# cvangysel/SERT

Hardware: AMD Instinct MI355X
Metric: training_pairs_per_sec (higher is better)
Workload: dtype f32; 1 GPU; C2 LSE: VectorSpaceLanguageModel (NCE z=10, Adam) V_w=100000 V_e=1000 d=128 window=10 batch=65536; global_batch=65536, per_gpu_batch=65536, parallelism=dp1, id_dtype=uint32, seed=0, instance_weights=1, dataset_instances=4194304, dataset_batches=64

## Files before the change

### include/sert_hip_debug.h

```cpp
#ifndef SERT_HIP_DEBUG_H
#define SERT_HIP_DEBUG_H

#include "sert_hip.h"

#ifdef __cplusplus
extern "C" {
#endif

int sert_debug_update_counts(sert_model* m, int64_t* out, int n);

int sert_debug_poison_scratch(sert_model* m);

int sert_debug_row_lists(const uint32_t* allbits, int world, int rank, int64_t num_batches, int64_t bit_words,
                         int64_t rows_per_rank, int64_t vocab, int64_t batch, int32_t* serve_cnt,
                         int32_t* fetch_cnt, int32_t* serve_rows, int32_t* fetch_rows, int32_t* union_rows,
                         int32_t* ptr, int32_t* ent, int64_t capacity, int64_t* sizes);

int sert_debug_word_index_sum(const void* ids, int id_bytes, int64_t num_batches, int B, int n, int vocab, int row_groups,
                              int dense_heavy, int64_t batch, const float* src, int d, float divisor, float* grad_out,
                              int64_t* stats);

int sert_bench_gemm(int device, int ta, int tb, int epi, int M, int N, int K, int splits,
                    int iters, double* avg_us);

int sert_debug_gemm(int device, int ta, int tb, int epi, int M, int N, int K, const float* A, const float* B,
                    const float* bias, float* C);

int sert_debug_gemm_splitk(int device, int M, int N, int K, int splits, const float* A, const float* B, float* out);

int sert_debug_gemm_longk(int device, int tb, int M, int N, int K, int splits, const float* A, const float* B, float* C);

enum { SERT_MEMBENCH_COPY = 0, SERT_MEMBENCH_READ = 1, SERT_MEMBENCH_GATHER = 2, SERT_MEMBENCH_OPTIMIZER = 3 };
int sert_bench_memory(int device, int kind, size_t bytes, size_t table_bytes, int row_bytes,
                      int window, size_t gap_bytes, int blocks, int iters, double* avg_us);

#ifdef __cplusplus
}
#endif
#endif
```

### sert_amd/_capi.py

```python
import ctypes
import os

import numpy as np

_HERE = os.path.dirname(os.path.abspath(__file__))
LIB_PATH = os.environ.get('SERT_LIB') or os.path.join(_HERE, 'libsert_hip.so')

KIND_LOGLINEAR, KIND_VECTORSPACE, KIND_VECTORSPACE_SOFTMAX = 0, 1, 2
SPLIT_TRAIN, SPLIT_VALIDATE = 0, 1

T_RW, T_RE, T_W, T_B = 0, 1, 2, 3
T_STATE0_RW, T_STATE0_RE, T_STATE0_W, T_STATE0_B = 4, 5, 6, 7
T_STATE1_RW, T_STATE1_RE, T_STATE1_W, T_STATE1_B = 8, 9, 10, 11
T_GRAD_RW, T_GRAD_RE, T_GRAD_W, T_GRAD_B = 12, 13, 14, 15
T_ACT_H, T_ACT_T, T_ACT_DA, T_ACT_DH, T_ACT_ROWLOSS = 16, 17, 18, 19, 20

COMM_ID_BYTES = 128

EXPORTS = [
    'sert_create', 'sert_destroy', 'sert_last_error', 'sert_device_info', 'sert_device_count',
    'sert_set_tensor', 'sert_get_tensor', 'sert_tensor_size', 'sert_set_step', 'sert_get_step',
    'sert_set_eval_draws', 'sert_get_eval_draws', 'sert_negatives_of_step',
    'sert_upload_dataset', 'sert_train_batch', 'sert_hint_next_batch', 'sert_train_batches',
    'sert_eval_batch', 'sert_eval_batches',
    'sert_predict_project', 'sert_predict_tokens', 'sert_score_topk',
    'sert_scorer_create', 'sert_scorer_destroy', 'sert_scorer_topk', 'sert_scorer_scores',
    'sert_host_alloc', 'sert_host_free',
    'sert_comm_unique_id', 'sert_comm_init', 'sert_comm_init_host', 'sert_comm_destroy', 'sert_comm_stats',
    'sert_synchronize', 'sert_timing_enable', 'sert_timing_reset', 'sert_timing_count',
    'sert_timing_name', 'sert_timing_avg_us', 'sert_timing_launches', 'sert_bench_gemm', 'sert_debug_gemm', 'sert_debug_gemm_splitk', 'sert_debug_gemm_longk', 'sert_bench_memory', 'sert_debug_row_lists', 'sert_debug_word_index_sum',
    'sert_debug_update_counts', 'sert_debug_poison_scratch',
    'sert_profile_range_push', 'sert_profile_range_pop',
]


_F32P, _I64P = ctypes.POINTER(ctypes.c_float), ctypes.POINTER(ctypes.c_int64)
ALLTOALL_FN = ctypes.CFUNCTYPE(ctypes.c_int, ctypes.c_void_p, _F32P, _I64P, _I64P, _F32P, _I64P, _I64P)


class SertConfig(ctypes.Structure):
    _fields_ = [
        ('struct_size', ctypes.c_uint32),
        ('kind', ctypes.c_int32),
        ('batch_size', ctypes.c_int32),
        ('global_batch_size', ctypes.c_int32),
        ('window_size', ctypes.c_int32),
        ('vocab_size', ctypes.c_int32),
        ('num_entities', ctypes.c_int32),
        ('word_dim', ctypes.c_int32),
        ('entity_dim', ctypes.c_int32),
        ('num_negatives', ctypes.c_int32),
        ('id_bytes', ctypes.c_int32),
        ('device', ctypes.c_int32),
        ('keep_grads', ctypes.c_int32),
        ('deterministic', ctypes.c_int32),
        ('inference_only', ctypes.c_int32),
        ('lambda_', ctypes.c_float),
        ('lr', ctypes.c_float),
        ('beta1', ctypes.c_float),
        ('beta2', ctypes.c_float),
        ('eps', ctypes.c_float),
        ('seed', ctypes.c_uint64),
    ]


class SertError(RuntimeError):
    pass


_lib = None


def load():
    global _lib
    if _lib is not None:
        return _lib
    if not os.path.exists(LIB_PATH):
        raise SertError(
            'libsert_hip.so not found at %s; build it with '
            '`python -m sert_amd._build` (hipcc --offload-arch=gfx950). '
            'There is no CPU fallback.' % LIB_PATH)
    lib = ctypes.CDLL(LIB_PATH)
    vp, i32, i64, sz = ctypes.c_void_p, ctypes.c_int32, ctypes.c_int64, ctypes.c_size_t
    fp = ctypes.c_void_p
    lib.sert_create.argtypes = [ctypes.POINTER(SertConfig), ctypes.POINTER(vp)]
    lib.sert_destroy.argtypes = [vp]
    lib.sert_last_error.restype = ctypes.c_char_p
    lib.sert_device_info.argtypes = [ctypes.c_int, ctypes.c_char_p, sz]
    lib.sert_device_count.argtypes = []
    lib.sert_set_tensor.argtypes = [vp, ctypes.c_int, fp, sz]
    lib.sert_get_tensor.argtypes = [vp, ctypes.c_int, fp, sz]
    lib.sert_tensor_size.argtypes = [vp, ctypes.c_int]
    lib.sert_tensor_size.restype = sz
    lib.sert_set_step.argtypes = [vp, i64]
    lib.sert_get_step.argtypes = [vp]
    lib.sert_get_step.restype = i64
    lib.sert_set_eval_draws.argtypes = [vp, i64]
    lib.sert_get_eval_draws.argtypes = [vp]
    lib.sert_get_eval_draws.restype = i64
    lib.sert_negatives_of_step.argtypes = [vp, i64, ctypes.c_int, vp]
    lib.sert_upload_dataset.argtypes = [vp, ctypes.c_int, fp, fp, fp, fp, fp, fp, i64]
    lib.sert_train_batch.argtypes = [vp, i64, fp, ctypes.POINTER(ctypes.c_float)]
    lib.sert_train_batches.argtypes = [vp, fp, i64, fp]
    lib.sert_hint_next_batch.argtypes = [vp, i64]
    lib.sert_eval_batch.argtypes = [vp, ctypes.c_int, i64, fp, ctypes.POINTER(ctypes.c_float)]
    lib.sert_eval_batches.argtypes = [vp, ctypes.c_int, ctypes.c_void_p, i64, ctypes.c_void_p]
    lib.sert_predict_project.argtypes = [vp, fp, i64, fp]
    lib.sert_predict_tokens.argtypes = [vp, fp, i64, fp]
    lib.sert_score_topk.argtypes = [ctypes.c_int, fp, i64, i32, fp, i64, i32, fp, fp]
    lib.sert_scorer_create.argtypes = [ctypes.c_int, fp, i64, i32, ctypes.POINTER(vp)]
    lib.sert_scorer_destroy.argtypes = [vp]
    lib.sert_scorer_topk.argtypes = [vp, fp, i64, i32, fp, fp]
    lib.sert_scorer_scores.argtypes = [vp, fp, i64, fp]
    lib.sert_host_alloc.argtypes = [ctypes.POINTER(vp), sz]
# ... 159 lines not shown
        check(self._lib.sert_eval_batch(self._h, split, int(batch_index), _addr(negatives),
                                        ctypes.byref(loss)))
        return np.float32(loss.value)

    def eval_batches(self, split, batch_indices):
        idx = np.ascontiguousarray(batch_indices, dtype=np.int64)
        out = np.empty(idx.shape[0], dtype=np.float32)
        if idx.shape[0]:
            check(self._lib.sert_eval_batches(self._h, split, idx.ctypes.data, idx.shape[0], out.ctypes.data))
        return out

    def predict_project(self, avg):
        avg = np.ascontiguousarray(avg, dtype=np.float32)
        q = avg.shape[0]
        out = np.empty((q, self.cfg.entity_dim), dtype=np.float32)
        check(self._lib.sert_predict_project(self._h, avg.ctypes.data, q, out.ctypes.data))
        return out

    def predict_tokens(self, ids):
        ids = np.ascontiguousarray(ids)
        assert ids.dtype.itemsize == self.cfg.id_bytes
        rows = ids.shape[0]
        out = np.empty((rows, self.cfg.window_size, self.cfg.num_entities), dtype=np.float32)
        check(self._lib.sert_predict_tokens(self._h, ids.ctypes.data, rows, out.ctypes.data))
        return out

    def comm_init(self, unique_id, rank, world):
        assert len(unique_id) == COMM_ID_BYTES
        check(self._lib.sert_comm_init(self._h, unique_id, rank, world))

    def comm_init_host(self, rank, world, alltoall):
        def trampoline(_user, send, soff, scnt, recv, roff, rcnt):
            try:
                so = np.ctypeslib.as_array(soff, shape=(world,))
                sc = np.ctypeslib.as_array(scnt, shape=(world,))
                ro = np.ctypeslib.as_array(roff, shape=(world,))
                rc = np.ctypeslib.as_array(rcnt, shape=(world,))
                ns = int((so + sc).max()) if world else 0
                nr = int((ro + rc).max()) if world else 0
                sbuf = np.ctypeslib.as_array(send, shape=(max(ns, 1),))
                rbuf = np.ctypeslib.as_array(recv, shape=(max(nr, 1),))
                alltoall(sbuf, so, sc, rbuf, ro, rc)
                return 0
            except Exception:
                import traceback
                traceback.print_exc()
                return 1
        self._host_alltoall = ALLTOALL_FN(trampoline)
        check(self._lib.sert_comm_init_host(self._h, rank, world, self._host_alltoall, None))

    def comm_stats(self):
        v = (ctypes.c_double * 8)()
        check(self._lib.sert_comm_stats(self._h, v, 8))
        return {'world': int(v[0]), 'exchange': {0: 'none', 1: 'zero1', 2: 'rows'}[int(v[1])],
                'bytes_per_step': float(v[2]), 'zero1_bytes_per_step': float(v[3]),
                'transport': {0: 'none', 1: 'rccl', 2: 'host'}[int(v[4])], 'steps': int(v[5]),
                'rows_fetched_per_batch': float(v[6]), 'rows_served_per_batch': float(v[7])}

    def synchronize(self):
        check(self._lib.sert_synchronize(self._h))

    def timing_enable(self, on=True):
        check(self._lib.sert_timing_enable(self._h, int(on)))

    def timing_launches(self):
        n = self._lib.sert_timing_count(self._h)
        return {self._lib.sert_timing_name(self._h, i).decode():
                self._lib.sert_timing_launches(self._h, i) for i in range(n)}

    def timing_reset(self):
        check(self._lib.sert_timing_reset(self._h))

    def poison_scratch(self):
        self._lib.sert_debug_poison_scratch.argtypes = [ctypes.c_void_p]
        check(self._lib.sert_debug_poison_scratch(self._h))

    def update_counts(self):
        v = (ctypes.c_int64 * 10)()
        self._lib.sert_debug_update_counts.argtypes = [ctypes.c_void_p, ctypes.POINTER(ctypes.c_int64), ctypes.c_int]
        check(self._lib.sert_debug_update_counts(self._h, v, 10))
        names = ('dense', 'lazy', 'skip_32_1', 'skip_64_1', 'skip_32_3', 'skip_64_2', 'skip_64_3', 'skip_64_4', 'skip_full', 'skip_sparse')
        return dict(zip(names, (int(x) for x in v)))

    def timings(self):
        n = self._lib.sert_timing_count(self._h)
        return {self._lib.sert_timing_name(self._h, i).decode():
                self._lib.sert_timing_avg_us(self._h, i) for i in range(n)}


def comm_unique_id():
    buf = ctypes.create_string_buffer(COMM_ID_BYTES)
    check(load().sert_comm_unique_id(buf))
    return buf.raw


def score_topk(entities, projections, k, device=0):
    e = np.ascontiguousarray(entities, dtype=np.float32)
    p = np.ascontiguousarray(projections, dtype=np.float32)
    assert e.ndim == 2 and p.ndim == 2 and e.shape[1] == p.shape[1]
    q = p.shape[0]
    idx = np.empty((q, k), dtype=np.int32)
    val = np.empty((q, k), dtype=np.float32)
    check(load().sert_score_topk(device, e.ctypes.data, e.shape[0], e.shape[1], p.ctypes.data, q,
                                 k, idx.ctypes.data, val.ctypes.data))
    return idx, val


class PinnedBuffer(object):

    def __init__(self, dtype):
        self.dtype = np.dtype(dtype)
        self._ptr = ctypes.c_void_p()
        self._bytes = 0
        self._lib = load()

    def view(self, shape):
        if os.environ.get('SERT_NO_PINNED'):
            return np.empty(shape, dtype=self.dtype)
        need = int(np.prod(shape)) * self.dtype.itemsize
        if need > self._bytes:
            self.free()
            cap = max(need, 1 << 16)
            check(self._lib.sert_host_alloc(ctypes.byref(self._ptr), cap))
            self._bytes = cap
        raw = (ctypes.c_char * max(need, 1)).from_address(self._ptr.value)
        return np.frombuffer(raw, dtype=self.dtype, count=int(np.prod(shape))).reshape(shape)

    def holds(self, array):
        if not self._ptr.value or not isinstance(array, np.ndarray) or not array.flags['C_CONTIGUOUS']:
            return False
        addr = array.ctypes.data
        return self._ptr.value <= addr and addr + array.nbytes <= self._ptr.value + self._bytes

    def free(self):
        if self._ptr.value:
            self._lib.sert_host_free(self._ptr)
            self._ptr = ctypes.c_void_p()
            self._bytes = 0

    def __del__(self):
        try:
            self.free()
        except Exception:
            pass


class Scorer(object):

    MAX_HOST_SCORES = 1 << 26

    def __init__(self, entities, device=0):
        e = np.ascontiguousarray(entities, dtype=np.float32)
        assert e.ndim == 2
        self.num_entities, self.dim = e.shape
        self._lib = load()
        self._h = ctypes.c_void_p()
        check(self._lib.sert_scorer_create(device, e.ctypes.data, e.shape[0], e.shape[1],
                                           ctypes.byref(self._h)))
        self._pin_q, self._pin_idx, self._pin_val = PinnedBuffer(np.float32), PinnedBuffer(np.int32), PinnedBuffer(np.float32)

    def query_buffer(self, num_queries):
        return self._pin_q.view((num_queries, self.dim))

    def _stage(self, projections):
        p = np.asarray(projections, dtype=np.float32)
        if p.ndim == 1:
# ... 4 lines not shown
        staged = self._pin_q.view(p.shape)
        np.copyto(staged, p)
        return staged

    def topk(self, projections, k):
        p = self._stage(projections)
        q = p.shape[0]
        idx = self._pin_idx.view((q, k))
        val = self._pin_val.view((q, k))
        check(self._lib.sert_scorer_topk(self._h, p.ctypes.data, q, k, idx.ctypes.data,
                                         val.ctypes.data))
        return idx, val

    def scores(self, projections):
        p = np.ascontiguousarray(projections, dtype=np.float32)
        if p.ndim == 1:
            p = p.reshape(1, -1)
        assert p.shape[1] == self.dim
        out = np.empty((p.shape[0], self.num_entities), dtype=np.float32)
        check(self._lib.sert_scorer_scores(self._h, p.ctypes.data, p.shape[0], out.ctypes.data))
        return out

    def rank(self, projections, k=None):
        if k is not None and k <= min(self.num_entities, 1024):
            return self.topk(projections, k)
        p = np.asarray(projections, dtype=np.float32)
        if p.ndim == 1:
            p = p.reshape(1, -1)
        keep = self.num_entities if k is None else min(k, self.num_entities)
        step = max(1, self.MAX_HOST_SCORES // self.num_entities)
        idx = np.empty((p.shape[0], keep), dtype=np.int32)
        val = np.empty((p.shape[0], keep), dtype=np.float32)
        for lo in range(0, p.shape[0], step):
            sc = self.scores(p[lo:lo + step])
            order = np.argsort(-sc, axis=1, kind='stable')[:, :keep]
            idx[lo:lo + step] = order
            val[lo:lo + step] = np.take_along_axis(sc, order, axis=1)
        return idx, val

    def close(self):
        if getattr(self, '_h', None) is not None and self._h:
            self._lib.sert_scorer_destroy(self._h)
            self._h = None
        for b in (getattr(self, '_pin_q', None), getattr(self, '_pin_idx', None), getattr(self, '_pin_val', None)):
            if b is not None:
                b.free()

    def __del__(self):
        try:
            self.close()
        except Exception:
            pass


def bench_gemm(M, N, K, ta=0, tb=0, epi=0, splits=1, iters=20, device=0):
    us = ctypes.c_double()
    check(load().sert_bench_gemm(device, ta, tb, epi, M, N, K, splits, iters, ctypes.byref(us)))
    return us.value


MEMBENCH_COPY, MEMBENCH_READ, MEMBENCH_GATHER, MEMBENCH_OPTIMIZER = 0, 1, 2, 3
SEPARATE_ALLOCATIONS = ctypes.c_size_t(-1).value


def debug_word_index_sum(ids, vocab, src, batch=0, row_groups=1, dense_heavy=False, divisor=1.0, sort_level0=False):
    lib = load()
    ids = np.ascontiguousarray(ids)
    assert ids.ndim == 3 and ids.dtype in (np.uint8, np.uint16, np.uint32), (ids.shape, ids.dtype)
    src = np.ascontiguousarray(src, dtype=np.float32)
    nb, B, n = ids.shape
    assert src.shape[0] == B
    d = src.shape[1]
    out = np.empty((vocab, d), dtype=np.float32)
    stats = np.zeros(8, dtype=np.int64)
    lib.sert_debug_word_index_sum.argtypes = [ctypes.c_void_p, ctypes.c_int, ctypes.c_int64, ctypes.c_int, ctypes.c_int, ctypes.c_int,
                                              ctypes.c_int, ctypes.c_int, ctypes.c_int64, ctypes.c_void_p, ctypes.c_int, ctypes.c_float,
                                              ctypes.c_void_p, ctypes.c_void_p]
    check(lib.sert_debug_word_index_sum(_addr(ids), ids.dtype.itemsize, nb, B, n, int(vocab), int(row_groups), int(bool(dense_heavy)) | (2 if sort_level0 else 0),
                                        int(batch), _addr(src), d, float(divisor), _addr(out), _addr(stats)))
    keys = ('levels', 'items', 'partial_rows', 'final_items', 'dense_words', 'row_groups', 'level0_items', 'distinct_words')
    return out, dict(zip(keys, [int(x) for x in stats]))


def debug_gemm(A, B, ta=0, tb=0, epi=0, bias=None, device=0):
    lib = load()
    A = np.ascontiguousarray(A, dtype=np.float32)
    B = np.ascontiguousarray(B, dtype=np.float32)
    K, M = A.shape if ta else A.shape[::-1]
    N = B.shape[0] if tb else B.shape[1]
    assert (B.shape[1] if tb else B.shape[0]) == K, (A.shape, B.shape)
    C = np.empty((M, N), dtype=np.float32)
    if bias is not None:
        bias = np.ascontiguousarray(bias, dtype=np.float32)
    lib.sert_debug_gemm.argtypes = [ctypes.c_int] * 7 + [ctypes.c_void_p] * 4
    check(lib.sert_debug_gemm(device, int(ta), int(tb), int(epi), M, N, K, _addr(A), _addr(B),
                              _addr(bias) if bias is not None else None, _addr(C)))
    return C


def debug_gemm_splitk(A, B, splits, device=0):
    lib = load()
    A = np.ascontiguousarray(A, dtype=np.float32)
    B = np.ascontiguousarray(B, dtype=np.float32)
    K, M = A.shape
    N = B.shape[1]
    assert B.shape[0] == K
    out = np.empty(M * N + N, dtype=np.float32)
    lib.sert_debug_gemm_splitk.argtypes = [ctypes.c_int] * 5 + [ctypes.c_void_p] * 3
    check(lib.sert_debug_gemm_splitk(device, M, N, K, int(splits), _addr(A), _addr(B), _addr(out)))
    return out[:M * N].reshape(M, N), out[M * N:]


def debug_gemm_longk(A, B, splits, tb=0, device=0):
    lib = load()
    A = np.ascontiguousarray(A, dtype=np.float32)
    B = np.ascontiguousarray(B, dtype=np.float32)
    M, K = A.shape
    N = B.shape[0] if tb else B.shape[1]
    assert (B.shape[1] if tb else B.shape[0]) == K
    out = np.empty((M, N), dtype=np.float32)
    lib.sert_debug_gemm_longk.argtypes = [ctypes.c_int] * 6 + [ctypes.c_void_p] * 3
    check(lib.sert_debug_gemm_longk(device, int(tb), M, N, K, int(splits), _addr(A), _addr(B), _addr(out)))
    return out


def bench_memory(kind, nbytes, table_bytes=0, row_bytes=512, window=10, gap_bytes=0, blocks=0, iters=20, device=0):
    us = ctypes.c_double()
    check(load().sert_bench_memory(device, kind, nbytes, table_bytes, row_bytes, window, gap_bytes, blocks, iters,
                                   ctypes.byref(us)))
    return us.value


def debug_row_lists(allbits, rank, rows_per_rank, vocab, batch):
    allbits = np.ascontiguousarray(allbits, dtype=np.uint32)
    world, nb, bw = allbits.shape
    cap = int(vocab) + 2
    i32 = lambda n: np.zeros(n, dtype=np.int32)
    scnt, fcnt = i32(world), i32(world)
    srows, frows, urows, ptr, ent = (i32(cap * world) for _ in range(5))
    sizes = np.zeros(5, dtype=np.int64)
    check(load().sert_debug_row_lists(allbits.ctypes.data, world, rank, nb, bw, rows_per_rank, vocab, batch,
                                      scnt.ctypes.data, fcnt.ctypes.data, srows.ctypes.data, frows.ctypes.data,
                                      urows.ctypes.data, ptr.ctypes.data, ent.ctypes.data, cap * world, sizes.ctypes.data))
    ns, nf, nu, ne = (int(x) for x in sizes[:4])
    return dict(serve_cnt=scnt, fetch_cnt=fcnt, serve_rows=srows[:ns], fetch_rows=frows[:nf], union_rows=urows[:nu],
                ptr=ptr[:nu + 1], ent=ent[:ne], max_xfer_rows=int(sizes[4]))


class profile_range(object):

    def __init__(self, name):
        self.name = name.encode() if isinstance(name, str) else name

    def __enter__(self):
        check(load().sert_profile_range_push(self.name))
        return self

    def __exit__(self, *exc):
        check(load().sert_profile_range_pop())
```

### sert_amd/csrc/host/api_data_train.inc

```

int sert_upload_dataset(sert_model* m, int split, const void* x, const int32_t* y_int,
                        const int64_t* csr_indptr, const int32_t* csr_indices,
                        const float* csr_data, const float* w, int64_t N) {
    if (!m) SERT_FAIL("null model");
    invalidate_speculation(m);
    m->hint_next = -1;
    if (split != SERT_SPLIT_TRAIN && split != SERT_SPLIT_VALIDATE) SERT_FAIL("bad split");
    if (N < 0) SERT_FAIL("negative instance count");
    if (N > 0 && !x) SERT_FAIL("x is null");
    if (N > 0 && !y_int && !(csr_indptr && csr_indices && csr_data)) SERT_FAIL("no labels given");
    if (is_vs(m) && N > 0 && !y_int) SERT_FAIL("vectorspace requires int labels (models.py:933-934)");
    SERT_HIP(hipSetDevice(m->cfg.device));
    if (N > 0) {
        const size_t toks = (size_t)N * m->cfg.window_size;
        const uint32_t Vw = (uint32_t)m->cfg.vocab_size;
        bool ok = true;
        SERT_ID_DISPATCH(m->cfg.id_bytes, {
            const IdT* xi = (const IdT*)x;
            uint32_t mx = 0;
            for (size_t i = 0; i < toks; ++i) mx = std::max<uint32_t>(mx, (uint32_t)xi[i]);
            ok = mx < Vw;
        });
        if (!ok) SERT_FAIL("token id >= vocab_size in x");
        const int32_t Ve = m->cfg.num_entities;
        if (y_int) {
            for (int64_t i = 0; i < N; ++i)
                if (y_int[i] < 0 || y_int[i] >= Ve) SERT_FAIL("label out of range [0, num_entities) in y");
        } else {
            if (csr_indptr[0] != 0) SERT_FAIL("csr_indptr[0] != 0");
            for (int64_t r = 0; r < N; ++r)
                if (csr_indptr[r + 1] < csr_indptr[r]) SERT_FAIL("csr_indptr is not non-decreasing");
            const int64_t nnz = csr_indptr[N];
            for (int64_t i = 0; i < nnz; ++i)
                if (csr_indices[i] < 0 || csr_indices[i] >= Ve) SERT_FAIL("label column out of range [0, num_entities) in csr_indices");
        }
    }
    DataSplit& d = m->split[split];
    free_split(d);
    d.N = N;
    if (N == 0) return 0;
    hipStream_t s = m->stream;
    const size_t xbytes = (size_t)N * m->cfg.window_size * m->cfg.id_bytes;
    SERT_HIP(hipMalloc(&d.x, xbytes));
    SERT_HIP(hipMemcpyAsync(d.x, x, xbytes, hipMemcpyHostToDevice, s));
    if (y_int) {
        d.max_labels_per_row = 1;
        SERT_TRY(dmalloc(&d.y, (size_t)N));
        SERT_HIP(hipMemcpyAsync(d.y, y_int, N * sizeof(int32_t), hipMemcpyHostToDevice, s));
    } else {
        d.nnz = csr_indptr[N];
        for (int64_t r = 0; r < N; ++r)
            d.max_labels_per_row = std::max<int64_t>(d.max_labels_per_row, csr_indptr[r + 1] - csr_indptr[r]);
        SERT_TRY(dmalloc(&d.csr_indptr, (size_t)N + 1));
        SERT_TRY(dmalloc(&d.csr_indices, (size_t)std::max<int64_t>(1, d.nnz)));
        SERT_TRY(dmalloc(&d.csr_data, (size_t)std::max<int64_t>(1, d.nnz)));
        SERT_HIP(hipMemcpyAsync(d.csr_indptr, csr_indptr, (N + 1) * sizeof(int64_t), hipMemcpyHostToDevice, s));
        if (d.nnz) {
            SERT_HIP(hipMemcpyAsync(d.csr_indices, csr_indices, d.nnz * sizeof(int32_t), hipMemcpyHostToDevice, s));
            SERT_HIP(hipMemcpyAsync(d.csr_data, csr_data, d.nnz * sizeof(float), hipMemcpyHostToDevice, s));
        }
    }
    if (split == SERT_SPLIT_TRAIN) {
        SERT_TRY(dmalloc(&d.w, (size_t)N));
        if (w) {
            SERT_HIP(hipMemcpyAsync(d.w, w, N * sizeof(float), hipMemcpyHostToDevice, s));
        } else {
            std::vector<float> ones((size_t)N, 1.0f);
            SERT_HIP(hipMemcpyAsync(d.w, ones.data(), N * sizeof(float), hipMemcpyHostToDevice, s));
            SERT_HIP(hipStreamSynchronize(s));
        }
    }
    if (split == SERT_SPLIT_TRAIN && !m->cfg.inference_only && !is_vs(m))
        SERT_TRY(dmalloc(&d.labfix, (size_t)std::max<int64_t>(1, y_int ? N : d.nnz)));
    if (split == SERT_SPLIT_TRAIN && !m->cfg.inference_only) {
        const int B = m->cfg.batch_size, n = m->cfg.window_size;
        const int64_t nb = N / B;
        WordIndex wi;
        const bool row_is_pos = !is_vs(m);
        bool vs_heavy = false;
        if (is_vs(m) && m->cfg.word_dim % 4 == 0 && m->cfg.word_dim <= 512) {
            const int d4 = m->cfg.word_dim / 4;
            const bool lpi32 = d4 <= 32 || (d4 > 64 && 64 * cdiv(d4, 64) > 32 * cdiv(d4, 32));
            const bool bundle_on = variant_knob("SERT_SEG_BUNDLE") && atoi(variant_knob("SERT_SEG_BUNDLE")) != 0;
            vs_heavy = knob("SERT_DENSE_HEAVY") ? atoi(knob("SERT_DENSE_HEAVY")) != 0 : (lpi32 && !bundle_on);
        }
        const bool dense_heavy = !variant_knob("SERT_NO_DENSE_HEAVY") && (is_vs(m) ? vs_heavy : (m->cfg.num_entities % 4 == 0));
        int row_groups = 1;
        if (is_vs(m) && m->cfg.word_dim % 4 == 0)
            if (const char* e = variant_knob("SERT_SEG_GROUPS")) row_groups = std::min(std::max(1, atoi(e)), std::max(1, B / 64));
        const bool sort_level0 = is_vs(m) && row_groups == 1 && !(variant_knob("SERT_SEG_BUNDLE") && atoi(variant_knob("SERT_SEG_BUNDLE")) != 0) &&
                                 !variant_knob("SERT_SEG_NO_SORT");
        bool ids_ok = true;
        SERT_ID_DISPATCH(m->cfg.id_bytes,
                         ids_ok = build_word_index<IdT>((const IdT*)x, nb, B, n, m->cfg.vocab_size, row_is_pos, wi,
                                                        !is_vs(m), dense_heavy, row_groups, sort_level0));
        if (!ids_ok) SERT_FAIL("token id >= vocab_size in x");
        if (!is_vs(m) && !wi.slots.empty()) {
            const size_t V = (size_t)m->cfg.num_entities;
            SERT_TRY(dmalloc(&d.idx_uwords, std::max<size_t>(1, wi.uwords.size())));
            SERT_TRY(dmalloc(&d.idx_slots, wi.slots.size()));
            SERT_HIP(hipMemcpyAsync(d.idx_uwords, wi.uwords.data(), wi.uwords.size() * sizeof(int32_t), hipMemcpyHostToDevice, s));
            SERT_HIP(hipMemcpyAsync(d.idx_slots, wi.slots.data(), wi.slots.size() * sizeof(int32_t), hipMemcpyHostToDevice, s));
            SERT_TRY(dmalloc(&d.idx_rows_div, wi.rows_div.size()));
            SERT_HIP(hipMemcpyAsync(d.idx_rows_div, wi.rows_div.data(), wi.rows_div.size() * sizeof(int32_t), hipMemcpyHostToDevice, s));
            SERT_HIP(hipStreamSynchronize(s));
            if ((size_t)wi.max_distinct > m->zu_rows) {
                (void)hipFree(m->Zu); (void)hipFree(m->dZu);
                m->Zu = nullptr; m->dZu = nullptr;
                m->zu_rows = (size_t)wi.max_distinct;
                SERT_TRY(dmalloc(&m->Zu, m->zu_rows * V));
                SERT_TRY(dmalloc(&m->dZu, m->zu_rows * V));
            }
            if ((size_t)wi.max_part_rows + 1 > m->zpart_rows) {
                (void)hipFree(m->zpart);
                m->zpart = nullptr;
                m->zpart_rows = (size_t)wi.max_part_rows + 1;
                SERT_TRY(dmalloc(&m->zpart, m->zpart_rows * V));
            }
        }
        if (!wi.rows.empty()) {
            SERT_TRY(dmalloc(&d.idx_rows, wi.rows.size()));
            SERT_HIP(hipMemcpyAsync(d.idx_rows, wi.rows.data(), wi.rows.size() * sizeof(int32_t), hipMemcpyHostToDevice, s));
            SERT_HIP(hipMalloc((void**)&d.idx_items, std::max<size_t>(1, wi.items.size()) * sizeof(SegItem)));
            SERT_HIP(hipMemcpyAsync(d.idx_items, wi.items.data(), wi.items.size() * sizeof(SegItem), hipMemcpyHostToDevice, s));
            if (!wi.heavy.empty()) {
                SERT_HIP(hipMalloc((void**)&d.idx_heavy, wi.heavy.size() * sizeof(int32_t)));
                SERT_HIP(hipMemcpyAsync(d.idx_heavy, wi.heavy.data(), wi.heavy.size() * sizeof(int32_t), hipMemcpyHostToDevice, s));
            }
            const bool bundle = variant_knob("SERT_SEG_BUNDLE") && atoi(variant_knob("SERT_SEG_BUNDLE")) != 0;
            if (!wi.bundles.empty() && bundle && is_vs(m)) {
                SERT_TRY(dmalloc(&d.idx_bundles, wi.bundles.size()));
                SERT_HIP(hipMemcpyAsync(d.idx_bundles, wi.bundles.data(), wi.bundles.size() * sizeof(int32_t), hipMemcpyHostToDevice, s));
            }
            SERT_HIP(hipStreamSynchronize(s));
        }
        if (!wi.touched_bits.empty()) {
            SERT_TRY(dmalloc(&d.idx_touched_bits, wi.touched_bits.size()));
            SERT_HIP(hipMemcpyAsync(d.idx_touched_bits, wi.touched_bits.data(), wi.touched_bits.size() * sizeof(uint32_t),
                                    hipMemcpyHostToDevice, s));
            SERT_HIP(hipStreamSynchronize(s));
            d.bit_words = wi.bit_words;
        }
        if (is_dp(m)) SERT_TRY(xr_build_lists(m, wi.touched_bits, nb, wi.bit_words));
        if (wi.any_dense) {
            SERT_HIP(hipMalloc((void**)&d.idx_dense_counts, wi.dense_counts.size()));
            SERT_HIP(hipMemcpyAsync(d.idx_dense_counts, wi.dense_counts.data(), wi.dense_counts.size(), hipMemcpyHostToDevice, s));
            std::vector<int32_t> hw((size_t)nb * kHeavyMax, 0);
            for (int64_t b = 0; b < nb; ++b)
                for (int h = 0; h < wi.batches[(size_t)b].dense_cnt; ++h) hw[(size_t)b * kHeavyMax + h] = wi.batches[(size_t)b].dense_word[h];
            if (!wi.dense_tok_slot.empty() && variant_knob("SERT_GATHER_HOT") && atoi(variant_knob("SERT_GATHER_HOT")) != 0) {
                SERT_HIP(hipMalloc((void**)&d.idx_tok_slot, wi.dense_tok_slot.size()));
                SERT_HIP(hipMemcpyAsync(d.idx_tok_slot, wi.dense_tok_slot.data(), wi.dense_tok_slot.size(), hipMemcpyHostToDevice, s));
                d.dense_cnt_of.resize((size_t)nb);
                for (int64_t b = 0; b < nb; ++b) d.dense_cnt_of[(size_t)b] = wi.batches[(size_t)b].dense_cnt;
            }
            SERT_TRY(dmalloc(&d.idx_dense_words, hw.size()));
            SERT_HIP(hipMemcpyAsync(d.idx_dense_words, hw.data(), hw.size() * sizeof(int32_t), hipMemcpyHostToDevice, s));
            SERT_HIP(hipStreamSynchronize(s));
            if (!m->hpart)
                SERT_TRY(dmalloc(&m->hpart, (size_t)std::max(cdiv(B, heavy_rows_fused(B)), cdiv(B, kHeavyRowsPerBlock)) * kHeavyMax *
                                               (size_t)(is_vs(m) ? m->cfg.word_dim : m->cfg.num_entities)));
        } else {
            for (auto& bxx : wi.batches) bxx.dense_cnt = 0;
        }
        d.idx_batches = wi.batches;
        if ((size_t)wi.max_part_rows + 1 > m->wpart_rows) {
            (void)hipFree(m->wpart);
            m->wpart_rows = (size_t)wi.max_part_rows + 1;
            SERT_TRY(dmalloc(&m->wpart, m->wpart_rows * m->cfg.word_dim));
        }
    }
    SERT_HIP(hipStreamSynchronize(s));
    return 0;
}

int sert_train_batch(sert_model* m, int64_t batch_index, const int64_t* negatives, float* loss_out) {
    refresh_gemm_choice();
    if (!m) SERT_FAIL("null model");
    SERT_HIP(hipSetDevice(m->cfg.device));
    static const bool no_spin = variant_knob("SERT_NO_SPIN") != nullptr;
    const int64_t hint = m->hint_next;
    m->hint_next = -1;
    m->lazy_next = hint;
    auto prefetch_next = [&]() -> int {
        const DataSplit& ds = m->split[SERT_SPLIT_TRAIN];
        if (hint < 0 || m->timing.enabled || m->cfg.keep_grads) return 0;
        if ((hint + 1) * (int64_t)m->cfg.batch_size > ds.N) return 0;
        if (can_speculate_step(m)) {
            bool fused = false;
            SERT_TRY(step_forward_backward(m, ds, hint, nullptr, &fused));
            m->spec_fb_batch = hint;
            m->spec_fb_step = m->step;
        } else if (is_vs(m) && !is_fs(m)) {
            if (m->xr_on) SERT_TRY(xr_fetch_params(m, hint));
            SERT_TRY(vs_project(m, ds, hint));
            m->projected_batch = hint;
        } else if (m->xr_on) {
            SERT_TRY(xr_fetch_params(m, hint));
        }
        return 0;
    };
    if (m->timing.enabled || no_spin) {
        SERT_TRY(train_step_async(m, batch_index, negatives, m->d_loss));
        SERT_HIP(hipMemcpyAsync(m->h_loss, m->d_loss, 3 * sizeof(float), hipMemcpyDeviceToHost, m->stream));
        SERT_HIP(hipEventRecord(m->ev_loss, m->stream));
        SERT_TRY(prefetch_next());
        SERT_HIP(hipEventSynchronize(m->ev_loss));
        timing_collect(m);
        if (loss_out) *loss_out = m->h_loss[0];
        return 0;
    }
    SERT_TRY(train_step_async(m, batch_index, negatives, m->h_loss_dev, true));
    SERT_TRY(prefetch_next());
    const unsigned want = m->loss_seq;
    volatile unsigned* flag = reinterpret_cast<volatile unsigned*>(m->h_loss + 4);
    {
        const auto t_spin0 = std::chrono::steady_clock::now();
        double next_query_ms = 50.0;
        for (unsigned spins = 1; *flag != want; ++spins) {
            if ((spins & 0xfff) != 0) continue;
            const double waited_ms = std::chrono::duration<double, std::milli>(std::chrono::steady_clock::now() - t_spin0).count();
            if (waited_ms < next_query_ms) continue;
            next_query_ms = waited_ms + 50.0;
            const hipError_t q = hipStreamQuery(m->tail_pending ? m->tail_stream : m->stream);
// ... 213 lines not shown
```

### sert_amd/csrc/host/api_debug.inc

```

int sert_debug_poison_scratch(sert_model* m) {
    if (!m) SERT_FAIL("null argument");
    if (m->spec_fb_batch >= 0) SERT_FAIL("a run-ahead step is in flight (sert_hint_next_batch): its gradients live in the scratch");
    SERT_HIP(hipSetDevice(m->cfg.device));
    SERT_HIP(hipDeviceSynchronize());
    if (!m->gflat) return 0;
    std::vector<uint32_t> h(m->gflat_alloc, 0x7fc00000u);
    if (m->run_start) {
        const size_t V4 = round_up((size_t)m->cfg.num_entities, 4);
        for (size_t i = 0; i < V4; ++i) { h[m->gflat_count + i] = 0u; h[m->gflat_count + V4 + i] = 1u; }
    }
    SERT_HIP(hipMemcpy(m->gflat, h.data(), h.size() * sizeof(uint32_t), hipMemcpyHostToDevice));
    return 0;
}

int sert_debug_update_counts(sert_model* m, int64_t* out, int n) {
    if (!m || !out || n < 1 || n > 10) SERT_FAIL("bad argument");
    for (int i = 0; i < n; ++i) out[i] = m->upd_counts[i];
    return 0;
}

int sert_debug_row_lists(const uint32_t* allbits, int world, int rank, int64_t num_batches, int64_t bit_words,
                         int64_t rows_per_rank, int64_t vocab, int64_t batch, int32_t* serve_cnt, int32_t* fetch_cnt,
                         int32_t* serve_rows, int32_t* fetch_rows, int32_t* union_rows, int32_t* ptr, int32_t* ent,
                         int64_t capacity, int64_t* sizes) {
    if (!allbits || world < 1 || rank < 0 || rank >= world || batch < 0 || batch >= num_batches || !sizes)
        SERT_FAIL("bad argument");
    RowExchangeLists L;
    build_row_exchange(allbits, world, rank, num_batches, bit_words, rows_per_rank, vocab, L);
    const RowExchangeBatch& xb = L.batches[(size_t)batch];
    sizes[0] = xb.serve_total; sizes[1] = xb.fetch_total; sizes[2] = xb.nunion; sizes[3] = xb.nent; sizes[4] = L.max_xfer_rows;
    if (std::max<int64_t>(std::max(xb.serve_total, xb.fetch_total), std::max(xb.nunion + 1, xb.nent)) > capacity)
        SERT_FAIL("capacity too small");
    for (int q = 0; q < world; ++q) { serve_cnt[q] = xb.serve_cnt[(size_t)q]; fetch_cnt[q] = xb.fetch_cnt[(size_t)q]; }
    std::copy_n(L.serve_rows.begin() + xb.serve_off, xb.serve_total, serve_rows);
    std::copy_n(L.fetch_rows.begin() + xb.fetch_off, xb.fetch_total, fetch_rows);
    std::copy_n(L.union_rows.begin() + xb.union_off, xb.nunion, union_rows);
    std::copy_n(L.ptr.begin() + xb.ptr_off, xb.nunion + 1, ptr);
    std::copy_n(L.ent.begin() + xb.ent_off, xb.nent, ent);
    return 0;
}

int sert_debug_word_index_sum(const void* ids, int id_bytes, int64_t num_batches, int B, int n, int vocab, int row_groups,
                              int dense_heavy, int64_t batch, const float* src, int d, float divisor, float* grad_out,
                              int64_t* stats) {
    if (!ids || !src || !grad_out || !stats || num_batches <= 0 || B <= 0 || n <= 0 || vocab <= 0 || d <= 0 || batch < 0 ||
        batch >= num_batches || (id_bytes != 1 && id_bytes != 2 && id_bytes != 4))
        SERT_FAIL("bad argument");
    WordIndex wi;
    bool ok = true;
    SERT_ID_DISPATCH(id_bytes, ok = build_word_index<IdT>((const IdT*)ids, num_batches, B, n, vocab, false, wi,
                                                          false, (dense_heavy & 1) != 0, row_groups,
                                                          (dense_heavy & 2) != 0));
    if (!ok) SERT_FAIL("token id >= vocab");
    const BatchIndex& bx = wi.batches[(size_t)batch];
    if (((dense_heavy & 2) != 0 && row_groups <= 1 && bx.nlevels >= 1 && bx.item_cnt[0] > 0) != bx.slot_is_row) SERT_FAIL("slot_is_row not as asked");
    if (bx.slot_is_row) {
        const SegItem* l0 = wi.items.data() + bx.item_off[0];
        const int32_t* r0 = wi.rows.data() + bx.rows_off;
        for (int32_t k = 0; k < bx.item_cnt[0]; ++k) {
            if (l0[k].slot != r0[l0[k].begin]) SERT_FAIL("a level-0 item's slot is not its first row");
            if (k > 0 && l0[k].end - l0[k].begin > l0[k - 1].end - l0[k - 1].begin) SERT_FAIL("level 0 is not sorted by length");
        }
    }
    std::fill(grad_out, grad_out + (size_t)vocab * d, 0.f);
    std::vector<float> part((size_t)std::max<int64_t>(1, bx.part_rows) * d, 0.f);
    int64_t items_total = 0, finals = 0;
    for (int l = 0; l < bx.nlevels; ++l) {
        const SegItem* items = wi.items.data() + bx.item_off[l];
        const float* in = l == 0 ? src : part.data() + (size_t)bx.part_off[l - 1] * d;
        const int32_t* rows = l == 0 ? wi.rows.data() + bx.rows_off : nullptr;
        float* pout = part.data() + (size_t)bx.part_off[l] * d;
        std::vector<int32_t> order;
        if (l == 0 && bx.row_groups > 1) {
            for (int x = 0; x < 8; ++x)
                for (int k = 0; k < bx.xcd_cnt[x]; ++k) order.push_back(bx.xcd_off[x] + k);
            if ((int32_t)order.size() != bx.item_cnt[0]) SERT_FAIL("XCD lists do not cover level 0");
        } else {
            for (int32_t k = 0; k < bx.item_cnt[l]; ++k) order.push_back(k);
        }
        for (int32_t k : order) {
            const SegItem& it = items[k];
            if (it.end - it.begin > kSegChunk && l < kSegMaxLevels - 1) SERT_FAIL("an item longer than a chunk");
            ++items_total;
            float* dst = it.dst >= 0 ? grad_out + (size_t)it.dst * d : pout + (size_t)(-(it.dst + 1)) * d;
            if (it.dst >= 0) ++finals;
            for (int c = 0; c < d; ++c) {
                float a = 0.f;
                if (l == 0 && bx.slot_is_row && it.end - it.begin == 1) a += in[(size_t)it.slot * d + c];
                else
                for (int32_t e = it.begin; e < it.end; ++e) a += in[(size_t)(rows ? rows[e] : e) * d + c];
                dst[c] = it.dst >= 0 ? a / divisor : a;
            }
        }
    }
    for (int h = 0; h < bx.dense_cnt; ++h) {
        const uint8_t* dc = wi.dense_counts.data() + (size_t)(batch * B) * kHeavyMax;
        for (int c = 0; c < d; ++c) {
            float a = 0.f;
            for (int i = 0; i < B; ++i) a += (float)dc[(size_t)i * kHeavyMax + h] * src[(size_t)i * d + c];
            grad_out[(size_t)bx.dense_word[h] * d + c] = a / divisor;
        }
    }
    stats[0] = bx.nlevels; stats[1] = items_total; stats[2] = bx.part_rows; stats[3] = finals; stats[4] = bx.dense_cnt;
    stats[5] = bx.row_groups; stats[6] = bx.item_cnt[0]; stats[7] = bx.num_distinct;
    return 0;
}

int sert_profile_range_push(const char* name) {
    roctx_load();
    if (!name) SERT_FAIL("null range name");
    return g_roctx.push ? (g_roctx.push(name) < 0 ? 1 : 0) : 0;
}
int sert_profile_range_pop(void) {
    roctx_load();
    return g_roctx.pop ? (g_roctx.pop() < 0 ? 1 : 0) : 0;
}

int sert_synchronize(sert_model* m) {
    if (!m) SERT_FAIL("null model");
    SERT_HIP(hipSetDevice(m->cfg.device));
    SERT_HIP(hipStreamSynchronize(m->stream));
    SERT_HIP(hipStreamSynchronize(m->stream2));
    if (m->stream3) SERT_HIP(hipStreamSynchronize(m->stream3));
    if (m->stream4) SERT_HIP(hipStreamSynchronize(m->stream4));
    if (m->tail_stream) SERT_HIP(hipStreamSynchronize(m->tail_stream));
    if (m->comm_stream) SERT_HIP(hipStreamSynchronize(m->comm_stream));
    return 0;
}

int sert_timing_enable(sert_model* m, int on) {
    if (!m) SERT_FAIL("null model");
    if (on < 0 || on > 2) SERT_FAIL("timing mode: 0 = off, 1 = every group alone on one queue, 2 = in the step");
    SERT_HIP(hipSetDevice(m->cfg.device));
    if (m->instep.on && on != 2) {
        SERT_HIP(hipDeviceSynchronize());
        instep_harvest(m, true);
    }
    if (on == 2 && !m->instep.created) {
        for (int i = 0; i < InStep::kRing; ++i)
            for (int k = 0; k < 2; ++k) SERT_HIP(hipEventCreate(&m->instep.ev[i][k]));
        m->instep.created = true;
    }
    m->timing.enabled = on == 1;
    m->instep.on = on == 2;
    m->instep.cur_group = -1;
    return 0;
}
int sert_timing_reset(sert_model* m) {
    if (!m) SERT_FAIL("null model");
    for (int g = 0; g < TG_COUNT; ++g) { m->timing.total_us[g] = 0; m->timing.samples[g] = 0; m->timing.used[g] = false; }
    if (m->instep.created) {
        SERT_HIP(hipSetDevice(m->cfg.device));
        SERT_HIP(hipDeviceSynchronize());
        instep_harvest(m, true);
        for (int g = 0; g < TG_COUNT; ++g) { m->instep.total_us[g] = 0; m->instep.launches[g] = 0; }
        m->instep.steps = 0;
    }
    return 0;
}
int sert_timing_count(sert_model*) { return TG_COUNT; }
const char* sert_timing_name(sert_model*, int i) { return (i >= 0 && i < TG_COUNT) ? kTimingNames[i] : ""; }
double sert_timing_avg_us(sert_model* m, int i) {
    if (!m || i < 0 || i >= TG_COUNT) return 0.0;
    if (m->instep.steps > 0) {
        if (m->instep.head < m->instep.tail) {
            (void)hipSetDevice(m->cfg.device);
            (void)hipDeviceSynchronize();
            instep_harvest(m, true);
        }
        return m->instep.total_us[i] / (double)m->instep.steps;
    }
    if (m->timing.samples[i] == 0) return 0.0;
    return m->timing.total_us[i] / (double)m->timing.samples[i];
}
double sert_timing_launches(sert_model* m, int i) {
    if (!m || i < 0 || i >= TG_COUNT || m->instep.steps == 0) return 0.0;
    return (double)m->instep.launches[i] / (double)m->instep.steps;
}

int sert_bench_gemm(int device, int ta, int tb, int epi, int M, int N, int K, int splits, int iters,
                    double* avg_us) {
    refresh_gemm_choice();
    if (!avg_us || M <= 0 || N <= 0 || K <= 0 || iters <= 0) SERT_FAIL("bad argument");
    SERT_HIP(hipSetDevice(device));
    hipStream_t s;
    SERT_HIP(hipStreamCreateWithFlags(&s, hipStreamNonBlocking));
    if (splits < 1) splits = 1;
// ... 218 lines not shown
```

### sert_amd/csrc/host/api_model.inc

```

const char* sert_last_error(void) { return g_last_error.c_str(); }

int sert_device_count(void) {
    int n = 0;
    if (hipGetDeviceCount(&n) != hipSuccess) return -1;
    return n;
}

int sert_device_info(int device, char* buf, size_t buflen) {
    hipDeviceProp_t p;
    if (hipGetDeviceProperties(&p, device) != hipSuccess) {
        g_last_error = "hipGetDeviceProperties failed";
        return -1;
    }
    return snprintf(buf, buflen, "%s %s: %d CUs, %.0f MHz, %.1f GiB, LDS/block %zu KiB", p.name,
                    p.gcnArchName, p.multiProcessorCount, p.clockRate / 1000.0,
                    p.totalGlobalMem / (1024.0 * 1024.0 * 1024.0), p.sharedMemPerBlock / 1024);
}

static int create_resources(sert_model* m);
static int layout_gradients(sert_model* m);

static int shard_setup(sert_model* m) {
    if (m->cfg.inference_only) SERT_FAIL("model was created inference_only");
// ... 84 lines not shown
        SERT_HIP(hipEventCreateWithFlags(e, flags));
    }
    m->events_device_scope = device_scope;
    return 0;
}

int sert_create(const sert_config* cfg, sert_model** out) {
    if (!cfg || !out) SERT_FAIL("null argument");
    if (cfg->struct_size != sizeof(sert_config)) SERT_FAIL("sert_config size mismatch (ABI)");
    if (cfg->kind != SERT_KIND_LOGLINEAR && cfg->kind != SERT_KIND_VECTORSPACE &&
        cfg->kind != SERT_KIND_VECTORSPACE_SOFTMAX)
        SERT_FAIL("bad kind");
    if (cfg->batch_size <= 0 || cfg->window_size <= 0 || cfg->vocab_size <= 0 ||
        cfg->num_entities <= 0 || cfg->word_dim <= 0)
        SERT_FAIL("sizes must be positive");
    if (cfg->global_batch_size < cfg->batch_size) SERT_FAIL("global_batch_size < batch_size");
    if (cfg->id_bytes != 1 && cfg->id_bytes != 2 && cfg->id_bytes != 4) SERT_FAIL("id_bytes must be 1, 2 or 4");
    if (cfg->kind != SERT_KIND_LOGLINEAR) {
        if (cfg->entity_dim <= 0 || cfg->entity_dim > 512) SERT_FAIL("entity_dim must be in [1, 512]");
        if (cfg->num_negatives < 0) SERT_FAIL("num_negatives must be >= 0");
    }
    SERT_HIP(hipSetDevice(cfg->device));
    sert_model* m = new sert_model();
    m->cfg = *cfg;
    const int rc = create_resources(m);
    if (rc != 0) {
        const std::string why = g_last_error;
        sert_destroy(m);
        g_last_error = why;
        return rc;
    }
    *out = m;
    return 0;
}

static int layout_gradients(sert_model* m) {
    const bool vs = is_vs(m);
    const size_t V = m->cfg.num_entities;
    size_t off[5];
    size_t cur = 0;
    auto place = [&](int i) { off[i] = cur; cur += round_up(m->pt_pad[i], 4); };
    place(0);
    m->ar_split = cur;
    for (int i = 1; i < 4; ++i) if (m->pt_sharded[i]) place(i);
    m->rest_off = m->pt_sharded[0] ? cur : 0;
    for (int i = 1; i < 4; ++i) if (!m->pt_sharded[i]) place(i);
    off[4] = cur;
    m->gflat_count = off[4] + 4;
    m->gflat_alloc = m->gflat_count + (vs ? 2 * round_up(V, 4) : 0);
    if (m->gflat) { SERT_HIP(hipStreamSynchronize(m->stream)); (void)hipFree(m->gflat); m->gflat = nullptr; }
    SERT_TRY(dzalloc(&m->gflat, m->gflat_alloc, m->stream));
    if (vs) {
        m->run_start = (int32_t*)(m->gflat + m->gflat_count);
        m->run_end = m->run_start + round_up(V, 4);
    }
    m->g_rw = m->gflat + off[0];
    m->g_re = m->n_re ? m->gflat + off[1] : nullptr;
    m->g_w = m->gflat + off[2];
    m->g_b = m->gflat + off[3];
    m->g_loss = m->gflat + off[4];
    m->g_sq = m->g_loss + 1;
    return 0;
}

static int create_resources(sert_model* m) {
    const auto& c = m->cfg;
    SERT_HIP(hipStreamCreateWithFlags(&m->stream, hipStreamNonBlocking));
    SERT_HIP(hipStreamCreateWithFlags(&m->stream2, hipStreamNonBlocking));
    {
        const char* e3 = knob("SERT_STREAMS");
        const bool want3 = (e3 && atoi(e3) >= 3) || (variant_knob("SERT_DW_THIRD") && atoi(variant_knob("SERT_DW_THIRD")) != 0);
        const bool want4 = variant_knob("SERT_ADAM_SPLIT") && atoi(variant_knob("SERT_ADAM_SPLIT")) != 0;
        if (want3) SERT_HIP(hipStreamCreateWithFlags(&m->stream3, hipStreamNonBlocking));
        if (want4) SERT_HIP(hipStreamCreateWithFlags(&m->stream4, hipStreamNonBlocking));
        if (m->cfg.kind == SERT_KIND_VECTORSPACE && !m->cfg.inference_only && variant_knob("SERT_TAIL_QUEUE") && atoi(variant_knob("SERT_TAIL_QUEUE")) == 1) {
            SERT_HIP(hipStreamCreateWithFlags(&m->tail_stream, hipStreamNonBlocking));
            SERT_HIP(hipEventCreateWithFlags(&m->ev_tail_go, hipEventDisableTiming | hipEventDisableSystemFence));
            SERT_HIP(hipEventCreateWithFlags(&m->ev_tail_done, hipEventDisableTiming | hipEventDisableSystemFence));
        }
    }
    m->proj_fused = variant_knob("SERT_PROJ_FUSED") && atoi(variant_knob("SERT_PROJ_FUSED")) != 0;
    m->lazy_skip = !(knob("SERT_LAZY_SKIP") && atoi(knob("SERT_LAZY_SKIP")) == 0);
    m->lazy_max = knob("SERT_LAZY_MAX") ? (float)atof(knob("SERT_LAZY_MAX")) : 0.5f;
    {
        int cus = 0;
        if (hipDeviceGetAttribute(&cus, hipDeviceAttributeMultiprocessorCount, m->cfg.device) != hipSuccess || cus <= 0) cus = 256;
        m->num_cus = cus;
    }
    const char* fence_env = knob("SERT_EVENT_FENCE");
    SERT_TRY(create_intra_events(m, !(fence_env && !strcmp(fence_env, "system"))));
    SERT_HIP(hipEventCreateWithFlags(&m->ev_loss, hipEventDisableTiming));
    const size_t B = c.batch_size, n = c.window_size, dw = c.word_dim, V = c.num_entities;
    const bool vs = is_vs(m);
    const size_t de = vs ? c.entity_dim : 0;
    m->n_rw = (size_t)c.vocab_size * dw;
    m->n_re = vs ? V * de : 0;
    m->n_w = vs ? dw * de : dw * V;
    m->n_b = vs ? de : V;
    hipStream_t s = m->stream;
    {
        const size_t n[4] = {m->n_rw, m->n_re, m->n_w, m->n_b};
        for (int i = 0; i < 4; ++i) {
            m->pt_pad[i] = n[i];
            m->pt_big[i] = n[i] > 0 && (i == 0 || (i < 3 && n[i] > ((size_t)1 << 22)));
            m->pt_sharded[i] = false;
        }
    }
    SERT_TRY(dzalloc(&m->rw, m->n_rw, s));  SERT_TRY(dzalloc(&m->re, m->n_re, s));
    SERT_TRY(dzalloc(&m->W, m->n_w, s));    SERT_TRY(dzalloc(&m->b, m->n_b, s));
    if (!c.inference_only) {
        SERT_TRY(dzalloc(&m->s0_rw, m->n_rw, s)); SERT_TRY(dzalloc(&m->s0_re, m->n_re, s));
        SERT_TRY(dzalloc(&m->s0_w, m->n_w, s));   SERT_TRY(dzalloc(&m->s0_b, m->n_b, s));
        SERT_TRY(dzalloc(&m->s1_rw, m->n_rw, s)); SERT_TRY(dzalloc(&m->s1_re, m->n_re, s));
        SERT_TRY(dzalloc(&m->s1_w, m->n_w, s));   SERT_TRY(dzalloc(&m->s1_b, m->n_b, s));
        static const bool no_lazy = variant_knob("SERT_NO_LAZY") != nullptr;
        if (!no_lazy && c.word_dim % 4 == 0) {
            SERT_TRY(dzalloc(&m->rw_last[0], (size_t)c.vocab_size, s));
            SERT_TRY(dzalloc(&m->rw_last[1], (size_t)c.vocab_size, s));
            m->rw_pred_stride = (unsigned)round_up((size_t)c.vocab_size, 64);
            SERT_TRY(dzalloc(&m->rw_pred, (size_t)kLazyK * m->rw_pred_stride, s));
        }
        SERT_TRY(layout_gradients(m));
        SERT_TRY(dzalloc(&m->rowloss, B, s));
        size_t part = 0;
        if (vs) {
            SERT_TRY(dzalloc(&m->H, B * dw, s));  SERT_TRY(dzalloc(&m->T, B * de, s));
            if (c.kind == SERT_KIND_VECTORSPACE && !c.inference_only) SERT_TRY(dzalloc(&m->T_alt, B * de, s));
            SERT_TRY(dzalloc(&m->DA, B * de, s)); SERT_TRY(dzalloc(&m->DH, B * dw, s));
            SERT_TRY(dzalloc(&m->neg, std::max<size_t>(4, B * c.num_negatives), s));
            SERT_TRY(dzalloc(&m->neg_alt, std::max<size_t>(4, B * c.num_negatives), s));
            SERT_TRY(dzalloc(&m->neg_stage, std::max<size_t>(4, B * c.num_negatives), s));
            part = (size_t)1024 * (dw * de + de);
            if (c.kind == SERT_KIND_VECTORSPACE_SOFTMAX) {
                {
                    const char* em = variant_knob("SERT_FS_TILE_MB");
                    const size_t cap = (size_t)(em && atoi(em) > 0 ? atoi(em) : 1700) << 20;
                    size_t tile = B;
                    if (B * V * sizeof(float) > cap) tile = std::max<size_t>(256, (cap / (V * sizeof(float))) / 256 * 256);
                    const char* er = knob("SERT_FS_TILE_ROWS");
                    if (er && atoi(er) > 0) tile = (size_t)atoi(er);
                    m->fs_tile = (int)std::min<size_t>(B, tile);
                }
                SERT_TRY(dzalloc(&m->Z, (size_t)m->fs_tile * V, s));
                SERT_TRY(dzalloc(&m->DH2, B * de, s));
                const size_t tiles = (size_t)cdiv(de, GN) * cdiv(V, GM);
                const size_t sp = std::max<size_t>(1, cdiv(1024, tiles)) + 1;
                part = std::max(part, sp * V * de);
            }
            const size_t total = B * (c.num_negatives + 1);
            {
                const bool force_sort = knob("SERT_EGRAD_SORT") && atoi(knob("SERT_EGRAD_SORT")) != 0;
                m->egrad_force_sort = force_sort;
                m->egrad_ranges = variant_knob("SERT_EGRAD_RANGES") && atoi(variant_knob("SERT_EGRAD_RANGES")) != 0;
                const size_t c1 = c.num_negatives + 1;
                if (!force_sort && c.kind == SERT_KIND_VECTORSPACE && V <= 2048 && de % 4 == 0 && de <= 128 &&
                    total < ((size_t)1 << 27) && c1 <= (size_t)kElSubPairs) {
                    m->eg_er_shift = 4;
                    m->eg_ranges = cdiv(V, 16);
                    m->eg_sub_rows = (int)std::min<size_t>(256, kElSubPairs / c1);
                    while (m->eg_sub_rows > 32 && (size_t)B < (size_t)64 * m->eg_sub_rows) m->eg_sub_rows /= 2;
                    m->eg_num_sub = cdiv(B, m->eg_sub_rows);
                    m->eg_subs_per_group = (int)std::max<size_t>(1, (((size_t)2 << 20) / (de * sizeof(float))) / m->eg_sub_rows);
                    static const int want_groups = variant_knob("SERT_EG_GROUPS") ? std::max(1, atoi(variant_knob("SERT_EG_GROUPS"))) : 16;
                    m->eg_subs_per_group = std::max(1, std::min(m->eg_subs_per_group, m->eg_num_sub / want_groups));
                    m->eg_groups = cdiv(m->eg_num_sub, m->eg_subs_per_group);
                }
                if (m->eg_groups > 0) {
                    SERT_TRY(dzalloc(&m->epart, (size_t)m->eg_groups * V * de, s));
                    SERT_TRY(dzalloc(&m->eg_entries, total, s));
                    SERT_TRY(dzalloc(&m->eg_offs, (size_t)m->eg_num_sub * (m->eg_ranges + 1), s));
                }
            }
            SERT_TRY(dzalloc(&m->cand, total, s));        SERT_TRY(dzalloc(&m->cand_sorted, total + 1, s));
            SERT_TRY(dzalloc(&m->cand_early, total, s));
            SERT_TRY(dzalloc(&m->pair_sorted, total, s));
            SERT_TRY(dzalloc(&m->coef, total, s));
            const size_t chunks = (total + kEChunk - 1) / kEChunk;
            SERT_TRY(dzalloc(&m->ehead, chunks * de, s)); SERT_TRY(dzalloc(&m->etail, chunks * de, s));
            m->sort_bits = 1;
            while ((1ll << m->sort_bits) < (long long)V) ++m->sort_bits;
            const size_t tiles = (total + kSortTile - 1) / kSortTile;
            SERT_TRY(dzalloc(&m->sort_hist, (size_t)kSortMaxBins * tiles, s));
            SERT_TRY(dzalloc(&m->sort_bin_total, (size_t)kSortMaxBins, s));
            if (m->sort_bits > kSortMaxBits) {
                SERT_TRY(dzalloc(&m->sort_k_tmp, total, s));
                SERT_TRY(dzalloc(&m->sort_v_tmp, total, s));
            }
        } else {
#define SERT_LL_ATTR(NT)                                                                                  \
    SERT_HIP(hipFuncSetAttribute((const void*)ll_fused_row<true, NT>, hipFuncAttributeMaxDynamicSharedMemorySize, 150 * 1024)); \
    SERT_HIP(hipFuncSetAttribute((const void*)ll_fused_row<false, NT>, hipFuncAttributeMaxDynamicSharedMemorySize, 150 * 1024))
            SERT_LL_ATTR(512);
            SERT_HIP(hipFuncSetAttribute((const void*)ll_row_from_table<512>, hipFuncAttributeMaxDynamicSharedMemorySize, 150 * 1024));
#undef SERT_LL_ATTR
            SERT_TRY(dzalloc(&m->G, B * n * dw, s));  SERT_TRY(dzalloc(&m->Z, B * n * V, s));
            SERT_TRY(dzalloc(&m->J, B * V, s));       SERT_TRY(dzalloc(&m->DG, B * n * dw, s));
            const size_t nseg = cdiv(V, kLlSeg);
            SERT_TRY(dzalloc(&m->ll_tokstat, B * n * nseg, s)); SERT_TRY(dzalloc(&m->ll_lse, B * n, s));
            SERT_TRY(dzalloc(&m->ll_jstat, B * nseg, s));       SERT_TRY(dzalloc(&m->ll_rowinfo, B, s));
            SERT_TRY(dzalloc(&m->ll_rpart, B * n * nseg, s));   SERT_TRY(dzalloc(&m->ll_r, B * n, s));
            SERT_TRY(dzalloc(&m->ll_rsum, B * n, s));
            const size_t tiles = (size_t)cdiv(V, GN) * cdiv(dw, GM);
            const size_t splits = std::max<size_t>(1, cdiv(1024, tiles)) + 1;
            part = splits * (dw * V + V);
        }
        m->part_count = part;
        SERT_TRY(dzalloc(&m->part, part, s));
        SERT_TRY(dzalloc(&m->red_loss, std::max<size_t>((size_t)kOptBlocks, (B + 15) / 16), s));
        SERT_TRY(dzalloc(&m->red_sq, (size_t)8 * kOptBlocks, s));
        SERT_TRY(dzalloc(&m->re_sq, (size_t)4 * kOptBlocks, s));
        SERT_TRY(dzalloc(&m->sq_scratch, (size_t)8 * kOptBlocks, s));
        SERT_TRY(dzalloc(&m->d_loss, (size_t)4, s));
        if (vs) {
            SERT_TRY(dzalloc(&m->tail_blk, (size_t)4 * (cdiv((int64_t)(m->n_w + m->n_b), 64) + 1), s));
        }
    }
    SERT_HIP(hipHostMalloc((void**)&m->h_loss, 8 * sizeof(float), hipHostMallocMapped | hipHostMallocCoherent));
    memset(m->h_loss, 0, 8 * sizeof(float));
    SERT_HIP(hipHostGetDevicePointer((void**)&m->h_loss_dev, m->h_loss, 0));
    {
        const char* e = knob("SERT_STREAMS");
        const int v = e ? atoi(e) : 0;
        if (v >= 1 && v <= 3) m->nstreams = v;
    }
    for (int g = 0; g < TG_COUNT; ++g)
        for (int k = 0; k < 2; ++k) SERT_HIP(hipEventCreate(&m->timing.ev[g][k]));
    m->timing.created = true;
    SERT_HIP(hipStreamSynchronize(s));
    return 0;
}

static void free_split(DataSplit& d) {
    (void)hipFree(d.x); (void)hipFree(d.y); (void)hipFree(d.csr_indptr);
    (void)hipFree(d.csr_indices); (void)hipFree(d.csr_data); (void)hipFree(d.w); (void)hipFree(d.labfix);
    (void)hipFree(d.idx_rows); (void)hipFree(d.idx_items);
    (void)hipFree(d.idx_heavy); d.idx_heavy = nullptr;
    (void)hipFree(d.idx_bundles); d.idx_bundles = nullptr;
    (void)hipFree(d.idx_uwords); (void)hipFree(d.idx_slots); (void)hipFree(d.idx_rows_div);
    (void)hipFree(d.idx_touched_bits);
    (void)hipFree(d.idx_dense_counts); (void)hipFree(d.idx_dense_words); (void)hipFree(d.idx_tok_slot);
    d.idx_uwords = nullptr; d.idx_slots = nullptr; d.idx_rows_div = nullptr;
    d = DataSplit();
}

int sert_destroy(sert_model* m) {
    if (!m) return 0;
    (void)hipSetDevice(m->cfg.device);
    if (m->stream) (void)hipStreamSynchronize(m->stream);
    if (m->stream2) (void)hipStreamSynchronize(m->stream2);
    if (m->stream3) (void)hipStreamSynchronize(m->stream3);
    if (m->stream4) (void)hipStreamSynchronize(m->stream4);
    if (m->tail_stream) (void)hipStreamSynchronize(m->tail_stream);
    if (m->comm_stream) (void)hipStreamSynchronize(m->comm_stream);
    if (m->comm && g_rccl.CommDestroy) g_rccl.CommDestroy(m->comm);
    if (m->ev_rest_ready) (void)hipEventDestroy(m->ev_rest_ready);
    if (m->ev_ar_done) (void)hipEventDestroy(m->ev_ar_done);
    if (m->ev_ag_done) (void)hipEventDestroy(m->ev_ag_done);
    for (int i = 0; i < 4; ++i) {
        if (m->ev_grad_ready[i]) (void)hipEventDestroy(m->ev_grad_ready[i]);
        for (int c = 0; c < sert_model::kMaxArChunks; ++c) {
            if (m->ev_rs_done[i][c]) (void)hipEventDestroy(m->ev_rs_done[i][c]);
            if (m->ev_opt_done[i][c]) (void)hipEventDestroy(m->ev_opt_done[i][c]);
        }
    }
    (void)hipFree(m->sq_scratch);
    (void)hipFree(m->tail_blk);
    (void)hipFree(m->rw_last[0]); (void)hipFree(m->rw_last[1]); (void)hipFree(m->rw_pred);
    xr_free_lists(m);
    if (m->ev_params_ready) (void)hipEventDestroy(m->ev_params_ready);
    if (m->ev_word_updated) (void)hipEventDestroy(m->ev_word_updated);
    if (m->comm_stream) (void)hipStreamDestroy(m->comm_stream);
    float* bufs[] = {m->rw, m->re, m->W, m->b, m->s0_rw, m->s0_re, m->s0_w, m->s0_b, m->s1_rw,
                     m->s1_re, m->s1_w, m->s1_b, m->gflat, m->H, m->T, m->T_alt, m->DA, m->DH, m->rowloss,
                     m->G, m->Z, m->J, m->DG, m->DH2, m->part, m->skbuf, m->wpart, m->hpart, m->red_loss, m->red_sq, m->re_sq, m->d_loss,
                     m->d_losses};
    for (float* p : bufs) (void)hipFree(p);
    (void)hipFree(m->ll_tokstat); (void)hipFree(m->ll_lse); (void)hipFree(m->ll_jstat);
    (void)hipFree(m->ll_rowinfo); (void)hipFree(m->ll_rpart); (void)hipFree(m->ll_r); (void)hipFree(m->ll_rsum);
    (void)hipFree(m->Zu); (void)hipFree(m->dZu); (void)hipFree(m->zpart);
    (void)hipFree(m->neg); (void)hipFree(m->neg_alt); (void)hipFree(m->neg_stage);
    (void)hipFree(m->pred_a); (void)hipFree(m->pred_b); (void)hipFree(m->pred_ids);
    (void)hipFree(m->cand); (void)hipFree(m->cand_sorted); (void)hipFree(m->cand_early);
    (void)hipFree(m->pair_sorted); (void)hipFree(m->coef); (void)hipFree(m->ehead);
    (void)hipFree(m->etail); (void)hipFree(m->epart); (void)hipFree(m->eg_entries); (void)hipFree(m->eg_offs); (void)hipFree(m->sort_hist); (void)hipFree(m->sort_bin_total);
    (void)hipFree(m->sort_k_tmp); (void)hipFree(m->sort_v_tmp);
    if (m->h_loss) (void)hipHostFree(m->h_loss);
    if (m->host_send) (void)hipHostFree(m->host_send);
    if (m->host_recv) (void)hipHostFree(m->host_recv);
    free_split(m->split[0]); free_split(m->split[1]);
    if (m->timing.created)
        for (int g = 0; g < TG_COUNT; ++g)
            for (int k = 0; k < 2; ++k) (void)hipEventDestroy(m->timing.ev[g][k]);
    if (m->instep.created)
        for (int i = 0; i < InStep::kRing; ++i)
            for (int k = 0; k < 2; ++k) (void)hipEventDestroy(m->instep.ev[i][k]);
    if (m->ev_fork) (void)hipEventDestroy(m->ev_fork);
    if (m->ev_join) (void)hipEventDestroy(m->ev_join);
    if (m->stream2) (void)hipStreamDestroy(m->stream2);
    if (m->ev_join3) (void)hipEventDestroy(m->ev_join3);
    for (hipEvent_t e : {m->ev_step_done, m->ev_neg, m->ev_opt_fork, m->ev_small, m->ev_re, m->ev_dense, m->ev_loss})
        if (e) (void)hipEventDestroy(e);
    if (m->stream3) (void)hipStreamDestroy(m->stream3);
    if (m->stream4) (void)hipStreamDestroy(m->stream4);
    if (m->ev_tail_go) (void)hipEventDestroy(m->ev_tail_go);
    if (m->ev_tail_done) (void)hipEventDestroy(m->ev_tail_done);
    if (m->tail_stream) (void)hipStreamDestroy(m->tail_stream);
    for (hipEvent_t e : {m->ev_word_opt, m->ev_early})
        if (e) (void)hipEventDestroy(e);
    if (m->stream) (void)hipStreamDestroy(m->stream);
    delete m;
    return 0;
}

size_t sert_tensor_size(sert_model* m, int which) {
    if (!m) return 0;
    return tensor_ref(m, which).count;
}

int sert_set_tensor(sert_model* m, int which, const float* host, size_t count) {
    if (m) invalidate_speculation(m);
    if (!m || !host) SERT_FAIL("null argument");
    SERT_HIP(hipSetDevice(m->cfg.device));
// ... 71 lines not shown
```

### sert_amd/csrc/host/lazy_segsum.inc

```

static void optimizer_args(const sert_model* m, int64_t t, AdamArgs* aa, AdadeltaArgs* da);
static LazyArgs lazy_args(sert_model* m, int64_t t_prev, int update) {
    LazyArgs lz;
    lz.last_in = m->rw_stale ? m->rw_last[m->rw_last_cur] : nullptr;
    lz.last_out = m->rw_last[m->rw_last_cur ^ 1];
    lz.next_bits = nullptr;
    lz.t_prev = (int)t_prev;
    lz.write_all = 1;
    lz.update = update;
    for (int k = 0; k <= kLazyK; ++k) {
        AdamArgs aa; AdadeltaArgs da;
        optimizer_args(m, std::max<int64_t>(1, t_prev + 1 - k), &aa, &da);
        lz.a_of[k] = aa.a_t;
    }
    return lz;
}
static int ensure_rw_current(sert_model* m, int64_t batch, int64_t t_applied) {
    if (!m->rw_stale) return 0;
    if (batch >= 0 && batch == m->rw_ready_batch) return 0;
    if (t_applied < 0) t_applied = m->step;
    AdamArgs aa; AdadeltaArgs da;
    optimizer_args(m, std::max<int64_t>(1, t_applied), &aa, &da);
    const LazyArgs lz = lazy_args(m, t_applied, 0);
    const int64_t max_nb = m->n_rw >= ((size_t)1 << 24) ? 2 * kOptBlocks : kOptBlocks;
    const int nb = (int)std::min<int64_t>(max_nb, cdiv(cdiv(m->n_rw, 4), 256));
    if (is_vs(m))
        hipLaunchKernelGGL((dense_update_lazy<true>), dim3(nb), dim3(256), 0, m->stream, m->rw, (const float*)m->g_rw, m->s0_rw, m->s1_rw,
                           m->n_rw, aa, da, m->sq_scratch, (const uint32_t*)nullptr, (unsigned)m->cfg.word_dim, lz);
    else
        hipLaunchKernelGGL((dense_update_lazy<false>), dim3(nb), dim3(256), 0, m->stream, m->rw, (const float*)m->g_rw, m->s0_rw, m->s1_rw,
                           m->n_rw, aa, da, m->sq_scratch, (const uint32_t*)nullptr, (unsigned)m->cfg.word_dim, lz);
    m->rw_last_cur ^= 1;
    m->rw_stale = false;
    m->rw_ready_batch = -1;
    return 0;
}

static int settle_tail(sert_model* m) {
    if (m->tail_pending) {
        SERT_HIP(hipStreamWaitEvent(m->stream, m->ev_tail_done, 0));
        m->tail_pending = false;
    }
    return 0;
}
static int settle_entity_update(sert_model* m) {
    SERT_TRY(settle_tail(m));
    if (m->re_pending) {
        SERT_HIP(hipStreamWaitEvent(m->stream, m->ev_re, 0));
        m->re_pending = false;
    }
    return 0;
}

struct TensorRef {
    float* ptr;
    size_t count;
};
static TensorRef tensor_ref(sert_model* m, int which) {
    const size_t B = m->cfg.batch_size;
    switch (which) {
        case SERT_T_RW: return {m->rw, m->n_rw};
        case SERT_T_RE: return {m->re, m->n_re};
        case SERT_T_W: return {m->W, m->n_w};
        case SERT_T_B: return {m->b, m->n_b};
        case SERT_T_STATE0_RW: return {m->s0_rw, m->n_rw};
        case SERT_T_STATE0_RE: return {m->s0_re, m->n_re};
        case SERT_T_STATE0_W: return {m->s0_w, m->n_w};
        case SERT_T_STATE0_B: return {m->s0_b, m->n_b};
        case SERT_T_STATE1_RW: return {m->s1_rw, m->n_rw};
        case SERT_T_STATE1_RE: return {m->s1_re, m->n_re};
        case SERT_T_STATE1_W: return {m->s1_w, m->n_w};
        case SERT_T_STATE1_B: return {m->s1_b, m->n_b};
        case SERT_T_GRAD_RW: return {m->g_rw, m->n_rw};
        case SERT_T_GRAD_RE: return {m->g_re, m->n_re};
        case SERT_T_GRAD_W: return {m->g_w, m->n_w};
        case SERT_T_GRAD_B: return {m->g_b, m->n_b};
        case SERT_T_ACT_H: return {m->H, m->H ? B * m->cfg.word_dim : 0};
        case SERT_T_ACT_T: return {m->T, m->T ? B * m->cfg.entity_dim : 0};
        case SERT_T_ACT_DA: return {m->DA, m->DA ? B * m->cfg.entity_dim : 0};
        case SERT_T_ACT_DH: return {m->DH, m->DH ? B * m->cfg.word_dim : 0};
        case SERT_T_ACT_ROWLOSS: return {m->rowloss, B};
        default: return {nullptr, 0};
    }
}

#define SERT_ID_DISPATCH(id_bytes, ...)                                  \
    do {                                                                 \
        if ((id_bytes) == 1) { typedef uint8_t IdT; __VA_ARGS__; }       \
        else if ((id_bytes) == 2) { typedef uint16_t IdT; __VA_ARGS__; } \
        else { typedef uint32_t IdT; __VA_ARGS__; }                      \
    } while (0)


static int word_grad_segsum(sert_model* m, const DataSplit& ds, int64_t batch_index,
                            const float* src, float divisor) {
    const int d = m->cfg.word_dim;
    if ((size_t)batch_index >= ds.idx_batches.size()) SERT_FAIL("batch has no word index");
    const BatchIndex& bx = ds.idx_batches[(size_t)batch_index];
    unsigned char* touched = nullptr;
    static const bool no_fused_upper = variant_knob("SERT_SEG_NO_FUSED_UPPER") != nullptr;
    const bool fused_upper = !no_fused_upper && bx.fused_upper_ok && ds.idx_heavy && d % 4 == 0 &&
                             bx.nlevels == 3 && bx.item_cnt[1] > 0;
    bool heavy_fused = false, heavy_combined = false;
    PlusJob hjob = PlusJob();
    if (bx.dense_cnt > 0 && is_vs(m) && d % 4 == 0) {
        const int B = m->cfg.batch_size, d4 = d / 4;
        static const bool no_fuse = variant_knob("SERT_HEAVY_NO_FUSE") != nullptr;
        const bool lpi32 = d4 <= 32 || (d4 > 64 && 64 * cdiv(d4, 64) > 32 * cdiv(d4, 32));
        const bool bundled = bx.bundle_cnt > 0 && ds.idx_bundles;
        heavy_fused = !no_fuse && lpi32 && bx.nlevels >= 1 && bx.item_cnt[0] > 0 && bx.row_groups == 1 && !bundled;
        const uint4* cnt = ds.idx_dense_counts + (size_t)batch_index * B;
        if (heavy_fused) {
            hjob.kind = 1; hjob.rpb = heavy_rows_fused(B); hjob.extra = cdiv(B, hjob.rpb); hjob.src = src; hjob.cnt16 = cnt; hjob.part = m->hpart;
            hjob.words = (const int32_t*)ds.idx_dense_words + (size_t)batch_index * kHeavyMax;
            hjob.nheavy = bx.dense_cnt; hjob.nblocks = hjob.extra; hjob.B = B;
        } else {
        const int nblk = cdiv(B, kHeavyRowsPerBlock);
        const size_t lds = (size_t)4 * kHeavyMax * 32 * sizeof(float4);
        hipLaunchKernelGGL(segsum_heavy, dim3(nblk * cdiv(d4, 32)), dim3(1024), lds, m->stream, src, cnt, B, d, m->hpart);
        hipLaunchKernelGGL(segsum_heavy_combine, dim3(bx.dense_cnt, cdiv(d4, 32)), dim3(256), 0, m->stream,
                           (const float*)m->hpart, nblk, d, (const int32_t*)ds.idx_dense_words + (size_t)batch_index * kHeavyMax,
                           bx.dense_cnt, m->g_rw, divisor);
        }
    }
    auto heavy_combine_job = [&]() { PlusJob j = hjob; j.kind = 2; j.extra = bx.dense_cnt; j.src = m->hpart; return j; };
    for (int l = 0; l < bx.nlevels; ++l) {
        const int nitems = bx.item_cnt[l];
        if (nitems == 0) continue;
        if (fused_upper && l == 1) {
            const int nb_normal = cdiv(nitems, 32);
            hipLaunchKernelGGL(segsum_upper_fused, dim3(nb_normal + bx.heavy_cnt, cdiv(d / 4, 32)), dim3(1024), 0, m->stream,
                               m->wpart + (size_t)bx.part_off[0] * d, ds.idx_items + bx.item_off[1], nitems, nb_normal,
                               ds.idx_heavy + bx.heavy_off, m->g_rw, d, divisor);
            break;
        }
        const float* in = (l == 0) ? src : m->wpart + (size_t)bx.part_off[l - 1] * d;
        const int32_t* rows = (l == 0) ? ds.idx_rows + bx.rows_off : nullptr;
        const int4* items = ds.idx_items + bx.item_off[l];
        float* pout = m->wpart + (size_t)bx.part_off[l] * d;
        if (heavy_fused && l <= 1) {
            PlusJob j = l == 0 ? hjob : heavy_combine_job();
            j.slot_is_row = (l == 0 && bx.slot_is_row) ? 1 : 0;
            int ni = nitems;
            static const int ko = variant_knob("SERT_KO_PLUS") ? atoi(variant_knob("SERT_KO_PLUS")) : 0;
            if (ko == 1 && l == 0) j.extra = 0;
            if (ko == 2 && l == 0) ni = 0;
            hipLaunchKernelGGL(segsum_rows_plus, dim3(j.extra + cdiv(ni, 8), cdiv(d / 4, 32)), dim3(256), 0, m->stream, in, rows, items,
                               ni, m->g_rw, pout, d, divisor, j);
            if (l == 1) heavy_combined = true;
            continue;
        }
#ifdef SERT_VARIANTS
        if (l == 0 && d % 4 == 0 && bx.bundle_cnt > 0 && ds.idx_bundles && bx.row_groups == 1) {
            hipLaunchKernelGGL(segsum_rows_bundled, dim3(cdiv(bx.bundle_cnt, 8), cdiv(d / 4, 32)), dim3(256), 0, m->stream, in, rows,
                               items, (const int32_t*)ds.idx_bundles + bx.bundle_off, (int)bx.bundle_cnt, m->g_rw, pout, d, divisor);
            continue;
        }
#endif
        if (d % 4 == 0) {
            const int ch = d / 4;
            const bool seg32y = ch > 64 && ch * (64 * cdiv(ch, 64)) > ch * (32 * cdiv(ch, 32));
            XcdLists xl = XcdLists();
            xl.slot_is_row = (l == 0 && bx.slot_is_row) ? 1 : 0;
            int longest = 0;
            if (l == 0 && bx.row_groups > 1) {
                xl.on = 1;
                for (int x = 0; x < 8; ++x) { xl.off[x] = bx.xcd_off[x]; xl.cnt[x] = bx.xcd_cnt[x]; longest = std::max(longest, bx.xcd_cnt[x]); }
            }
            const int ipb = (d / 4 <= 32 || seg32y) ? 8 : 4;
            const int gx = xl.on ? 8 * cdiv(longest, ipb) : cdiv(nitems, ipb);
            if (d / 4 <= 32)
                hipLaunchKernelGGL((segsum_rows<32>), dim3(gx), dim3(256), 0, m->stream,
                                   in, rows, items, nitems, m->g_rw, pout, d, divisor, touched, 1, nullptr, nullptr, DenseSlots(), xl);
            else if (seg32y)
                hipLaunchKernelGGL((segsum_rows<32>), dim3(gx, cdiv(d / 4, 32)), dim3(256), 0, m->stream,
                                   in, rows, items, nitems, m->g_rw, pout, d, divisor, touched, 1, nullptr, nullptr, DenseSlots(), xl);
            else
                hipLaunchKernelGGL((segsum_rows<64>), dim3(gx, cdiv(d / 4, 64)), dim3(256), 0, m->stream,
                                   in, rows, items, nitems, m->g_rw, pout, d, divisor, touched, 1, nullptr, nullptr, DenseSlots(), xl);
        } else {
            hipLaunchKernelGGL((segsum_rows_scalar<false>), dim3(cdiv(nitems, 4), cdiv(d, 64)), dim3(256), 0, m->stream, in,
// ... 168 lines not shown
```

### sert_amd/csrc/host/optimizer_and_loss.inc

```

static int reduce_rowloss(sert_model* m, hipStream_t st) {
    const int B = m->cfg.batch_size;
    int nb = std::min(kOptBlocks, cdiv(B, 256));
    m->loss_from_rows = false;
    if (is_vs(m) && !is_fs(m) && m->nce_loss_partials > 0) nb = m->nce_loss_partials;
    else if (!is_dp(m) && B <= 8192) {
        m->loss_from_rows = true;
        nb = B;
    } else hipLaunchKernelGGL(sum_partial, dim3(nb), dim3(256), 0, st, m->rowloss, (size_t)B, m->red_loss);
    if (is_dp(m))
        hipLaunchKernelGGL(partials_to_scalar, dim3(1), dim3(256), 0, st, m->red_loss, nb, m->g_loss);
    m->n_loss_partials = nb;
    return 0;
}

static void launch_stream_opt(sert_model* m, hipStream_t st, float* p, float* g, float* s0, float* s1, size_t count,
                              int nb, const AdamArgs& aa, const AdadeltaArgs& da, float* sq,
                              const uint32_t* bits, unsigned row_len, int rows_mode = kRowsAll, float* sq_new = nullptr) {
    const bool keep = m->cfg.keep_grads != 0;
    if (is_vs(m)) {
        if (keep) hipLaunchKernelGGL((adam_l2<true>), dim3(nb), dim3(256), 0, st, p, g, s0, s1, count, aa, sq, bits, row_len, rows_mode, sq_new);
        else      hipLaunchKernelGGL((adam_l2<false>), dim3(nb), dim3(256), 0, st, p, g, s0, s1, count, aa, sq, bits, row_len, rows_mode, sq_new);
    } else {
        if (keep) hipLaunchKernelGGL((adadelta_l2<true>), dim3(nb), dim3(256), 0, st, p, g, s0, s1, count, da, sq, bits, row_len, rows_mode);
        else      hipLaunchKernelGGL((adadelta_l2<false>), dim3(nb), dim3(256), 0, st, p, g, s0, s1, count, da, sq, bits, row_len, rows_mode);
    }
}

static void optimizer_args(const sert_model* m, int64_t t, AdamArgs* aa, AdadeltaArgs* da) {
    const auto& c = m->cfg;
    const float l2k = c.lambda_ > 0.f ? c.lambda_ / (float)c.global_batch_size : 0.f;
    *aa = AdamArgs{l2k, 0.f, c.beta1, c.beta2, c.eps};
    *da = AdadeltaArgs{l2k, c.lr, c.beta1, c.eps};
    if (is_vs(m)) {
        const float tf = (float)t;
        aa->a_t = c.lr * sqrtf(1.0f - powf(c.beta2, tf)) / (1.0f - powf(c.beta1, tf));
    }
}

static bool adam_split_enabled() {
    static const bool on = variant_knob("SERT_ADAM_SPLIT") && atoi(variant_knob("SERT_ADAM_SPLIT")) != 0;
    return on;
}
static int issue_untouched_rows_update(sert_model* m, const uint32_t* bits) {
    m->early_issued = false;
    m->early_sq = 0;
    const bool split = adam_split_enabled();
    if (!split || !bits || !m->use_touched || is_dp(m) || m->timing.enabled || m->nstreams < 2) return 0;
    AdamArgs aa; AdadeltaArgs da;
    optimizer_args(m, m->step + 1, &aa, &da);
    SERT_HIP(hipStreamWaitEvent(m->stream4, m->ev_word_opt, 0));
    const int nb = (int)std::min<int64_t>(kOptBlocks, cdiv(cdiv(m->n_rw, 4), 256));
    launch_stream_opt(m, m->stream4, m->rw, m->g_rw, m->s0_rw, m->s1_rw, m->n_rw, nb, aa, da, m->red_sq, bits,
                      (unsigned)m->cfg.word_dim, kRowsUntouched);
    SERT_HIP(hipEventRecord(m->ev_early, m->stream4));
    m->early_issued = true;
    m->early_sq = nb;
    return 0;
}

static int launch_lazy_word_update(sert_model* m, const ParamTensor& t, const uint32_t* tf, const uint32_t* next_bits, const int nb,
                                   const AdamArgs& aa, const AdadeltaArgs& da, float* sq) {
    const auto& c = m->cfg;
    LazyArgs lz = lazy_args(m, m->step - 1, 1);
    int nb_skip = 0;
    lz.next_bits = next_bits;
    lz.write_all = (next_bits == nullptr || m->step % kLazyK == 0) ? 1 : 0;
    const unsigned d4 = (unsigned)c.word_dim / 4;
    if (m->lazy_skip && m->rw_pred && d4 <= 256) {
        const int64_t u = m->step;
        const bool sparse = next_bits && m->rw_pred_ok && u < m->rw_pred_T;
        lz.write_all = sparse ? 0 : 1;
        if (!sparse) m->rw_pred_T = u + kLazyK;
        SkipArgs sk;
        sk.pred = m->rw_pred;
        sk.stride = m->rw_pred_stride;
        sk.npred = next_bits ? (int)(m->rw_pred_T - 1 - u) : 0;
        for (int j = 0; j < kLazyK; ++j) {
            AdamArgs a2; AdadeltaArgs d2;
            optimizer_args(m, u + 1 + j, &a2, &d2);
            sk.a_fut[j] = a2.a_t;
        }
        m->rw_pred_ok = next_bits != nullptr;
        const unsigned nrows = (unsigned)c.vocab_size;
        static const int skip_blocks_knob = variant_knob("SERT_SKIP_BLOCKS") ? atoi(variant_knob("SERT_SKIP_BLOCKS")) : 0;
        const int nb_dense = nb;
        const int nb = std::max(1, std::min<int>(skip_blocks_knob > 0 ? std::min(skip_blocks_knob, 4 * kOptBlocks) : skip_grid(nb_dense, t.n),
                                                 (int)cdiv(nrows, 8u)));
        nb_skip = nb;
#define SERT_SKIP_LAUNCH(ADAM, LPR, CPL)                                                                                   \
    hipLaunchKernelGGL((dense_update_skip<ADAM, LPR, CPL>), dim3(nb), dim3(256), 0, m->stream, t.p, (const float*)t.g, t.s0, \
           t.s1, nrows, aa, da, sq, tf, (unsigned)c.word_dim, lz, sk)
        static const int skip_32x3_knob = variant_knob("SERT_SKIP_32X3") ? atoi(variant_knob("SERT_SKIP_32X3")) : -1;
        const bool skip_32x3 = skip_32x3_knob >= 0 ? skip_32x3_knob != 0 : t.n < ((size_t)1 << 26);
#define SERT_SKIP_SHAPE(ADAM)                                                                   \
    do {                                                                                        \
        if (d4 <= 32) { SERT_SKIP_LAUNCH(ADAM, 32, 1); ++m->upd_counts[2]; }                    \
        else if (d4 <= 64) { SERT_SKIP_LAUNCH(ADAM, 64, 1); ++m->upd_counts[3]; }               \
        else if (d4 <= 96 && skip_32x3) { SERT_SKIP_LAUNCH(ADAM, 32, 3); ++m->upd_counts[4]; }  \
        else if (d4 <= 128) { SERT_SKIP_LAUNCH(ADAM, 64, 2); ++m->upd_counts[5]; }              \
        else if (d4 <= 192) { SERT_SKIP_LAUNCH(ADAM, 64, 3); ++m->upd_counts[6]; }              \
        else { SERT_SKIP_LAUNCH(ADAM, 64, 4); ++m->upd_counts[7]; }                             \
        ++m->upd_counts[sparse ? 9 : 8];                                                        \
    } while (0)
        if (is_vs(m)) SERT_SKIP_SHAPE(true);
        else SERT_SKIP_SHAPE(false);
#undef SERT_SKIP_SHAPE
#undef SERT_SKIP_LAUNCH
    } else {
    ++m->upd_counts[1];
    if (is_vs(m))
        hipLaunchKernelGGL((dense_update_lazy<true>), dim3(nb), dim3(256), 0, m->stream, t.p, (const float*)t.g, t.s0, t.s1, t.n,
                           aa, da, sq, tf, (unsigned)c.word_dim, lz);
    else
        hipLaunchKernelGGL((dense_update_lazy<false>), dim3(nb), dim3(256), 0, m->stream, t.p, (const float*)t.g, t.s0, t.s1, t.n,
                           aa, da, sq, tf, (unsigned)c.word_dim, lz);
    }
    m->rw_last_cur ^= 1;
    m->rw_stale = !lz.write_all;
    m->rw_ready_batch = lz.write_all ? -1 : m->lazy_next;
    return nb_skip > 0 ? nb_skip : nb;
}

static int optimizer_and_loss(sert_model* m, float* loss_dst, bool publish = false,
                              const uint32_t* bits = nullptr, const uint32_t* next_bits = nullptr) {
    const int n_loss_partials = m->n_loss_partials;
    const auto& c = m->cfg;
    const float l2k = c.lambda_ > 0.f ? c.lambda_ / (float)c.global_batch_size : 0.f;
    m->step += 1;
    AdamArgs aa; AdadeltaArgs da;
    optimizer_args(m, m->step, &aa, &da);
    int n_sq = m->early_issued ? m->early_sq : 0;
    const bool exchanged = m->comm && !m->timing.enabled;
    const bool side_small = !is_dp(m) && !m->timing.enabled && m->nstreams >= 2 && (is_vs(m) || m->ll_dw_side);
    hipStream_t ss = side_small ? m->stream2 : m->stream;
    if (side_small && m->lazy_join && fork_late_mode(m)) {
    } else if (side_small && m->lazy_join) {
        SERT_HIP(hipStreamWaitEvent(ss, m->ev_dense, 0));
    } else if (side_small) {
        SERT_HIP(hipEventRecord(m->ev_opt_fork, m->stream));
        SERT_HIP(hipStreamWaitEvent(ss, m->ev_opt_fork, 0));
    }
    bool any_ag = false;
    const int tail_splits = m->tail_splits;
    m->tail_splits = 0;
    static const bool no_defer = knob("SERT_RE_DEFER") && atoi(knob("SERT_RE_DEFER")) == 0;
    const bool defer_re = !no_defer && m->side_heavy && side_small && tail_splits > 0 && m->pt_big[1] && is_vs(m) && !c.keep_grads;
    const bool defer_small = !no_defer && !defer_re && side_small && tail_splits > 0 && !m->pt_big[1] && is_vs(m) && !is_fs(m) &&
                             !c.keep_grads && m->lazy_join && fork_late_mode(m) && m->n_re > 0;
    const int re_cur = (int)(m->step & 1), re_nxt = re_cur ^ 1;
    const size_t re_cap = (size_t)2 * kOptBlocks;
    bool small_needs_join = !defer_small;
    int re_sq_lo = 0, re_nb = 0;
    for (int i = 0; i < 4; ++i) {
        if (!m->pt_big[i]) continue;
        const ParamTensor t = param_tensor(m, i);
        if (t.n == 0) continue;
        const int tg = i == 0 ? TG_OPT_WORD : TG_OPTIMIZER;
        if (i == 1 && defer_re) {
            const int64_t max_nb = t.n >= ((size_t)1 << 24) ? 2 * kOptBlocks : kOptBlocks;
            re_nb = (int)std::min<int64_t>(max_nb, cdiv(cdiv(t.n, 4), 256));
            re_sq_lo = n_sq;
            n_sq += re_nb;
            continue;
        }
        if (!(is_dp(m) && m->pt_sharded[i])) {
            ScopedTimer tm(m, tg);
            const int64_t max_nb = t.n >= ((size_t)1 << 24) ? 2 * kOptBlocks : kOptBlocks;
            const int nb = (int)std::min<int64_t>(max_nb, cdiv(cdiv(t.n, 4), 256));
            const uint32_t* tf = (i == 0 && m->use_touched) ? bits : nullptr;
            const float lazy_max = (next_bits && m->lazy_skip) ? m->lazy_max : std::min(m->lazy_max, 0.35f);
            static const bool lazy_small = variant_knob("SERT_LAZY_SMALL_TABLES") != nullptr;
            if (i == 0 && tf && !m->early_issued && m->rw_last[0] && !c.keep_grads && c.word_dim % 4 == 0 &&
                m->cur_touched_frac <= lazy_max && (t.n >= ((size_t)1 << 22) || lazy_small)) {
                n_sq += launch_lazy_word_update(m, t, tf, next_bits, nb, aa, da, m->red_sq + n_sq);
                continue;
            }
            if (i == 0) m->rw_pred_ok = false;
            if (i == 0) ++m->upd_counts[0];
            if (i == 0) SERT_TRY(ensure_rw_current(m, -1, m->step - 1));
            const bool on_side = side_small && ((i == 1 && m->side_heavy) || (i >= 2 && m->ll_dw_side));
            launch_stream_opt(m, on_side ? ss : m->stream, t.p, t.g, t.s0, t.s1, t.n, nb, aa, da,
                              m->red_sq + n_sq, tf,
                              i == 0 ? (unsigned)c.word_dim : 1u,
                              (i == 0 && tf && m->early_issued) ? kRowsTouched : kRowsAll);
            n_sq += nb;
            continue;
        }
        const size_t sc = m->pt_sc[i];
        const int nch = m->ar_chunks;
        const bool by_rows = (i == 0) && m->xr_on;
        {
            ScopedTimer tm(m, tg);
            for (int ch = 0; ch < nch; ++ch) {
                if (exchanged && m->rs_issued[i]) SERT_HIP(hipStreamWaitEvent(m->stream, m->ev_rs_done[i][by_rows ? 0 : ch], 0));
                const size_t off = piece_off(m, i, ch);
                const int nb = (int)std::min<int64_t>(std::max(1, kOptBlocks / nch), cdiv(cdiv(sc, 4), 256));
                const uint32_t* ub = by_rows ? m->xr_ubits + (size_t)m->xr_batch * (size_t)m->xr->owned_bit_words : nullptr;
                launch_stream_opt(m, m->stream, t.p + off, t.g + off, t.s0 + (size_t)ch * sc, t.s1 + (size_t)ch * sc, sc,
                                  nb, aa, da, m->sq_scratch, ub, by_rows ? (unsigned)c.word_dim : 1u);
                if (by_rows) {
                    if (m->ev_word_updated) SERT_HIP(hipEventRecord(m->ev_word_updated, m->stream));
                    m->rw_full = false;
                    m->xr_fetched_batch = -1;
                    continue;
                }
                m->comm_bytes_moved += 8.0 * (double)sc * (double)(m->world - 1);
                if (exchanged) {
                    SERT_HIP(hipEventRecord(m->ev_opt_done[i][ch], m->stream));
                    SERT_HIP(hipStreamWaitEvent(m->comm_stream, m->ev_opt_done[i][ch], 0));
                    SERT_NCCL(g_rccl.AllGather(t.p + off, t.p + (size_t)ch * slab_elems(m, i), sc,  7,
                                               m->comm, m->comm_stream));
                    any_ag = true;
                }
            }
        }
        m->rs_issued[i] = false;
        if (by_rows) {
        } else if (m->host_ar) {
            ScopedTimer tm(m, TG_ALLGATHER);
            for (int ch = 0; ch < nch; ++ch) SERT_TRY(host_allgather(m, t.p + (size_t)ch * slab_elems(m, i), sc, m->stream));
        } else if (m->comm && m->timing.enabled) {
            ScopedTimer tm(m, TG_ALLGATHER);
            for (int ch = 0; ch < nch; ++ch)
                SERT_NCCL(g_rccl.AllGather(t.p + piece_off(m, i, ch), t.p + (size_t)ch * slab_elems(m, i), sc, 7, m->comm,
                                           m->stream));
        }
    }
    if (exchanged) SERT_HIP(hipStreamWaitEvent(m->stream, m->ev_ar_done, 0));
    if (side_small && egrad_writes_every_row(m) && c.kind == SERT_KIND_VECTORSPACE && !is_fs(m) && c.num_negatives > 0 && !c.keep_grads &&
        m->neg_alt_step != m->step) {
        const int64_t count = (int64_t)c.batch_size * c.num_negatives;
        hipLaunchKernelGGL(vs_sample_negatives, dim3(grid_for((count + 3) / 4)), dim3(256), 0, ss, m->neg_alt, count,
                           (int64_t)m->rank * count, (uint32_t)c.num_entities, c.seed, (uint64_t)m->step * 2);
        m->neg_alt_step = m->step;
    }
    const bool split_small = side_small && m->lazy_join && fork_late_mode(m);
    auto small_tensors = [&](hipStream_t ss, unsigned mask) {
        ScopedTimer t(m, TG_OPTIMIZER);
        SmallTensors st;
        int k = 0, blocks = 0;
        for (int i = 1; i < 4; ++i) {
            const ParamTensor t2 = param_tensor(m, i);
            if (m->pt_big[i] || t2.n == 0 || !((mask >> i) & 1u)) continue;
            st.p[k] = t2.p; st.g[k] = t2.g; st.s0[k] = t2.s0; st.s1[k] = t2.s1; st.count[k] = t2.n;
            const bool parts = (i == 1) && m->re_in_parts;
            st.gparts[k] = parts ? m->epart : nullptr;
            st.ngroups[k] = parts ? m->eg_groups : 0;
            st.gstride[k] = parts ? (unsigned long long)m->n_re : 0ull;
            st.l2k[k] = t2.l2 ? l2k : 0.f;
            st.first_block[k] = blocks;
            blocks += (int)std::min<int64_t>(512, cdiv(t2.n, 256));
            ++k;
        }
        for (int i = k; i < 3; ++i) { st.p[i] = st.g[i] = st.s0[i] = st.s1[i] = nullptr; st.count[i] = 0; st.l2k[i] = 0.f; st.gparts[i] = nullptr; st.ngroups[i] = 0; st.gstride[i] = 0; }
        for (int i = k; i <= 3; ++i) st.first_block[i] = blocks;
        float* sq = m->red_sq + n_sq;
        float* sq_new = nullptr;
        if (defer_small && mask == 0x2u && blocks > 0) {
            re_sq_lo = n_sq;
// ... 278 lines not shown
```

### sert_amd/csrc/host/step_vectorspace.inc

```

static int reduce_rowloss(sert_model* m, hipStream_t st);

static int vs_negatives(sert_model* m, const int64_t* negatives, uint64_t stream_pos, hipStream_t st) {
    const auto& c = m->cfg;
    const int64_t count = (int64_t)c.batch_size * c.num_negatives;
    if (count == 0) return 0;
    if (negatives) {
        const int64_t Ve = c.num_entities;
        for (int64_t i = 0; i < count; ++i)
            if (negatives[i] < 0 || negatives[i] >= Ve) SERT_FAIL("negative sample out of range [0, num_entities)");
        SERT_HIP(hipMemcpyAsync(m->neg_stage, negatives, count * sizeof(int64_t),
                                hipMemcpyHostToDevice, st));
        hipLaunchKernelGGL(convert_i64_to_i32, dim3(grid_for(count)), dim3(256), 0, st,
                           m->neg_stage, m->neg, count);
    } else {
        const int64_t global_offset = (int64_t)m->rank * count;
        hipLaunchKernelGGL(vs_sample_negatives, dim3(grid_for((count + 3) / 4)), dim3(256), 0,
                           st, m->neg, count, global_offset, (uint32_t)c.num_entities,
                           c.seed, stream_pos);
    }
    return 0;
}

static int vs_project(sert_model* m, const DataSplit& ds, int64_t batch_index) {
// ... 269 lines not shown
        const int chunks = cdiv(total, kEChunk);
        dim3 cgrid(cdiv(chunks, 16)), fgrid(cdiv(V, 4)), blk(256);
#define SERT_EG_ARGS m->cand_sorted, m->pair_sorted, m->coef, m->T, total, c.num_negatives + 1, de, \
                     m->g_re, m->ehead, m->etail, m->run_start, m->run_end
        {
            ScopedTimer t(m, TG_EGRAD, st);
            if (de % 4 == 0) {
                const int nch = cdiv(de / 4, 16);
                if (nch <= 1)      hipLaunchKernelGGL((egrad_chunk_reduce<4, 1>), cgrid, blk, 0, st, SERT_EG_ARGS);
                else if (nch <= 2) hipLaunchKernelGGL((egrad_chunk_reduce<4, 2>), cgrid, blk, 0, st, SERT_EG_ARGS);
                else if (nch <= 5) hipLaunchKernelGGL((egrad_chunk_reduce<4, 5>), cgrid, blk, 0, st, SERT_EG_ARGS);
                else               hipLaunchKernelGGL((egrad_chunk_reduce<4, 8>), cgrid, blk, 0, st, SERT_EG_ARGS);
            } else {
                hipLaunchKernelGGL((egrad_chunk_reduce<1, 4>), cgrid, blk, 0, st, SERT_EG_ARGS);
            }
        }
        {
            ScopedTimer t(m, TG_EFIX, st);
            const bool few = V < 256 && de <= 512;
            if (de % 4 == 0) {
                if (few) {
                    hipLaunchKernelGGL((egrad_fixup_wg<4>), dim3(V), blk, 0, st, m->run_start, m->run_end, V, de,
                                       m->ehead, m->etail, m->g_re);
                } else {
                    hipLaunchKernelGGL((egrad_fixup<4>), fgrid, blk, 0, st, m->run_start, m->run_end, V, de,
                                       m->ehead, m->etail, m->g_re);
                }
            } else if (few) {
                hipLaunchKernelGGL((egrad_fixup_wg<1>), dim3(V), blk, 0, st, m->run_start, m->run_end, V, de,
                                   m->ehead, m->etail, m->g_re);
            } else {
                hipLaunchKernelGGL((egrad_fixup<1>), fgrid, blk, 0, st, m->run_start, m->run_end, V, de,
                                   m->ehead, m->etail, m->g_re);
            }
        }
#undef SERT_EG_ARGS
        }
        return 0;
    };
    bool dense_bound = false;
    auto dh_gemm = [&]() -> int {
        {
            ScopedTimer t(m, TG_GEMM_DX);
#ifdef SERT_VARIANTS
            const bool strip = gemm_strip_ok(B, dw, de, de, de, true, m->DA, m->W);
#else
            const bool strip = false;
#endif
            dense_bound = m->lazy_join && ext_events() && !strip && !fork_nce;
            if (dense_bound) set_stop_event(fork_late ? m->ev_fork : m->ev_dense);
#ifdef SERT_VARIANTS
            if (fused_bwd) {
                static const bool attr_set = hipFuncSetAttribute((const void*)vs_bwd_fused, hipFuncAttributeMaxDynamicSharedMemorySize,
                                                                 (int)vs_bwd_fused_lds_bytes()) == hipSuccess;
                if (!attr_set) { set_stop_event(nullptr); SERT_FAIL("cannot reserve the LDS of vs_bwd_fused"); }
                BwdFusedArgs fa;
                fa.DA = m->DA; fa.H = m->H; fa.W = m->W; fa.DH = m->DH; fa.part = m->part; fa.B = B;
                fa.stride = (size_t)FB_D * FB_D + FB_D;
                SERT_LAUNCH(vs_bwd_fused, dim3(fused_grid), dim3(FB_THREADS), vs_bwd_fused_lds_bytes(), m->stream, fa);
            } else
            if (strip)
                launch_gemm_strip<true, EPI_STORE>(m->stream, m->DA, m->W, m->DH, nullptr, B, dw, de, de, de, dw);
            else
#endif
                launch_gemm<false, true, EPI_STORE>(m->stream, m->DA, m->W, m->DH, nullptr, B, dw, de, de,
                                                    de, dw);
            set_stop_event(nullptr);
        }
        if (m->lazy_join && !dense_bound && !fork_nce) SERT_HIP(hipEventRecord(fork_late ? m->ev_fork : m->ev_dense, m->stream));
        if (fork_late && !fork_nce && !is_dp(m) && !m->timing.enabled && m->epart && c.kind == SERT_KIND_VECTORSPACE &&
            c.num_negatives > 0 && m->neg_alt_step != m->step + 1) {
            const int64_t count = (int64_t)c.batch_size * c.num_negatives;
            hipLaunchKernelGGL(vs_sample_negatives, dim3(grid_for((count + 3) / 4)), dim3(256), 0, m->stream2, m->neg_alt, count,
                               (int64_t)m->rank * count, (uint32_t)c.num_entities, c.seed, (uint64_t)(m->step + 1) * 2);
            m->neg_alt_step = m->step + 1;
        }
        if (fork_late && !fork_nce) SERT_HIP(hipStreamWaitEvent(m->stream2, m->ev_fork, 0));
        if (fork_late && dw_third_queue(m)) SERT_HIP(hipStreamWaitEvent(m->stream3, m->ev_fork, 0));
        return 0;
    };
    auto word_table_sum = [&]() -> int {
        {
            ScopedTimer t(m, TG_SCATTER);
            SERT_TRY(word_grad_segsum(m, ds, batch_index, m->DH, (float)n));
        }
        return allreduce_word_grad(m);
    };
    auto dense_grad = [&]() -> int {
        hipStream_t sd = (m->timing.enabled || m->nstreams < 3) ? m->stream : m->stream3;
        static const bool dw_side = variant_knob("SERT_DW_SIDE") && atoi(variant_knob("SERT_DW_SIDE")) != 0;
        if ((dw_side || side_heavy) && m->lazy_join) sd = m->stream2;
        if (m->dp_late_join || m->dw_side_first) sd = m->stream2;
        if (fork_late && m->lazy_join && dw_third_queue(m)) sd = m->stream3;
        if (sd != m->stream && sd != m->stream2 && !fork_late) SERT_HIP(hipStreamWaitEvent(sd, m->ev_fork, 0));
        static const int user_splits = [] { const char* e = variant_knob("SERT_DW_SPLITS"); const int v = e ? atoi(e) : 0; return v > 0 ? v : 0; }();
        int auto_splits = std::max(1, std::min(std::min(512, cdiv(1024, cdiv(dw, GM) * cdiv(de, GN))), B / 64));
        const int x3_splits = std::max(1, std::min(256 / ((dw <= 128 && de <= 128) ? 1 : cdiv(de, 160)), B / 64));
        if (gemm_x3_enabled() && x3_shape_ok(true, false, m->H, m->DA, dw, de, B, dw, de, x3_splits))
            auto_splits = x3_splits;
        const int want_splits = user_splits ? user_splits : auto_splits;
        int splits = std::min(want_splits, cdiv(B, GK));
        int kper = (int)round_up(cdiv(B, splits), GK);
        splits = cdiv(B, kper);
        const size_t mn = (size_t)dw * de;
        const size_t stride = mn + de;
        if (fused_bwd) {
            splits = fused_grid;
            if (sd != m->stream) SERT_FAIL("internal: the fused backward needs dW's combine on the main stream");
        } else
#ifdef SERT_VARIANTS
        if (gemm_strip_ok(B, de, dw, dw, de, false, m->H, m->DA) && dw % 32 == 0 && de % 4 == 0) {
            ScopedTimer t(m, TG_GEMM_DW);
            static const int want_wgs = variant_knob("SERT_STRIP_DW_WGS") ? atoi(variant_knob("SERT_STRIP_DW_WGS")) : 512;
            const int strips = cdiv(B, SG_ROWS);
            const int spw = std::max(1, cdiv(strips, std::min(want_wgs, 1024)));
            splits = cdiv(strips, spw);
            hipLaunchKernelGGL(gemm_strip_tn, dim3(splits), dim3(256), 0, sd, (const float*)m->H, (const float*)m->DA, B,
                               dw, de, dw, de, spw, m->part, stride);
        } else
#endif
        {
            ScopedTimer t(m, TG_GEMM_DW);
            launch_gemm<true, false, EPI_STORE, true>(sd, m->H, m->DA, m->part, nullptr, dw, de,
                                                      B, dw, de, de, splits, kper, stride);
        }
        static const bool no_tail = variant_knob("SERT_NO_TAIL") != nullptr;
        m->tail_splits = 0;
        if (!no_tail && !is_dp(m) && (sd == m->stream || ((side_heavy || m->dw_side_first) && sd == m->stream2)) &&
            m->cfg.kind == SERT_KIND_VECTORSPACE && !m->pt_big[2] &&
            mn + de < ((size_t)1 << 31)) {
            m->tail_splits = splits;
            m->tail_stride = stride;
            m->tail_part = m->part;
            static const bool combine_side_off = !(variant_knob("SERT_COMBINE_SIDE") && atoi(variant_knob("SERT_COMBINE_SIDE")) == 1);
            if (!combine_side_off && m->dw_side_first && sd == m->stream2 && splits > 1 && !c.keep_grads) {
                ScopedTimer t(m, TG_SPLITK, sd);
                const size_t count = stride;
                hipLaunchKernelGGL((reduce_partials_g<16>), dim3((unsigned)((count + 63) / 64)), dim3(1024), 0, sd, (const float*)m->part, splits, stride,
                                   count, m->g_w, mn, m->g_b, (const int32_t*)nullptr, 0);
                m->tail_splits = 1;
                m->tail_part = m->g_w;
                if (m->g_b != m->g_w + mn) SERT_FAIL("internal: g_W and g_b are not adjacent");
            }
        } else {
            ScopedTimer t(m, TG_SPLITK);
            launch_reduce_partials(sd, m->part,
                               splits, stride, stride, m->g_w, mn, m->g_b);
        }
        SERT_TRY(reduce_rowloss(m, sd));
        static const bool ko_tail_early = variant_knob("SERT_KO_TAIL_EARLY") != nullptr;
        m->tail_early = false;
        if (ko_tail_early && m->tail_splits > 0 && m->dw_side_first && sd == m->stream2 && !c.keep_grads && !m->timing.enabled) {
            AdamArgs aa2; AdadeltaArgs da2;
            optimizer_args(m, m->step + 1, &aa2, &da2);
            TailArgs ta;
            ta.part = m->tail_part ? m->tail_part : m->part; ta.splits = m->tail_splits; ta.stride = m->tail_stride;
            ta.W = m->W; ta.b = m->b; ta.s0_w = m->s0_w; ta.s1_w = m->s1_w; ta.s0_b = m->s0_b; ta.s1_b = m->s1_b;
            ta.g_w = m->g_w; ta.g_b = m->g_b;
            ta.n_w = (unsigned)m->n_w; ta.n_b = (unsigned)m->n_b;
            ta.aa = aa2;
            ta.loss_partials = m->red_loss; ta.n_loss = 0;
            ta.sq_partials = m->red_sq; ta.n_sq = 0;
            ta.sq_alt = nullptr; ta.sq_alt_lo = 0; ta.sq_alt_hi = 0;
            ta.inv_batch = 1.f; ta.reg_scale = 0.f;
            ta.out = m->d_loss; ta.host_flag = nullptr; ta.seq = 0u;
            ta.blk = m->tail_blk;
            if (++m->tail_launch_seq == 0) ++m->tail_launch_seq;
// ... 97 lines not shown
```

### sert_amd/csrc/kernels_opt.h

```cpp
#pragma once
#include "common.h"

namespace sert {

#ifndef SERT_OPT_BLOCKS
#define SERT_OPT_BLOCKS 2048
#endif
constexpr int kOptBlocks = SERT_OPT_BLOCKS;

struct AdamArgs {
    float l2k;
    float a_t;
    float b1, b2, eps;
};

__device__ __forceinline__ float sq_acc(float acc, float x) { return __builtin_fmaf(x, x, acc); }

__device__ __forceinline__ void adam_elem(float& p, float& g, float& m, float& v, const AdamArgs& a,
                                          float omb1, float omb2, float& ss, float& ss_new) {
#pragma clang fp contract(off)
    const float pv = p;
    const float l2 = a.l2k * pv;
    const float gv = g + l2;
    ss = sq_acc(ss, pv);
    const float m1 = a.b1 * m, m2 = omb1 * gv;
    const float mv = m1 + m2;
    const float v1 = a.b2 * v, v2 = (omb2 * gv) * gv;
    const float vv = v1 + v2;
    m = mv;
    v = vv;
#ifndef SERT_OPT_IEEE_DIV
    const float num = a.a_t * mv, den = __builtin_amdgcn_sqrtf(vv) + a.eps;
    const float quo = num * __builtin_amdgcn_rcpf(den);
    const float pn = pv - quo;
#else
    const float num = a.a_t * mv, den = sqrtf(vv) + a.eps;
    const float pn = pv - num / den;
#endif
    p = pn;
    ss_new = sq_acc(ss_new, pn);
    g = gv;
}

enum { kRowsAll = 0, kRowsTouched = 1, kRowsUntouched = 2 };
__device__ __forceinline__ bool row_bit(const uint32_t* __restrict__ bits, unsigned row) {
    return (bits[row >> 5] >> (row & 31)) & 1u;
}

template <bool STORE_G>
__global__ __launch_bounds__(256) void adam_l2(float* __restrict__ p, float* __restrict__ g,
                                               float* __restrict__ m, float* __restrict__ v,
                                               size_t count, AdamArgs a,
                                               float* __restrict__ sumsq_partial,
                                               const uint32_t* __restrict__ bits = nullptr,
                                               unsigned row_len = 1, int rows_mode = kRowsAll,
                                               float* __restrict__ sumsq_new_partial = nullptr) {
    __shared__ float red[4];
    float ss = 0.f, ssn = 0.f;
    const float omb1 = 1.0f - a.b1, omb2 = 1.0f - a.b2;
    const size_t n4 = count >> 2;
    float4* p4 = reinterpret_cast<float4*>(p);
    float4* g4 = reinterpret_cast<float4*>(g);
    float4* m4 = reinterpret_cast<float4*>(m);
    float4* v4 = reinterpret_cast<float4*>(v);
    const size_t per = (n4 + gridDim.x - 1) / gridDim.x;
    const size_t lo = (size_t)blockIdx.x * per;
    const size_t hi = lo + per < n4 ? lo + per : n4;
    for (size_t i = lo + threadIdx.x; i < hi; i += blockDim.x) {
        const bool hit = !bits || row_bit(bits, ((unsigned)i << 2) / row_len);
        if (rows_mode != kRowsAll && hit != (rows_mode == kRowsTouched)) continue;
#ifndef SERT_ADAM_NO_NT
        typedef float nt_f4 __attribute__((ext_vector_type(4)));
        float4 pp = p4[i];
        const nt_f4 mr = __builtin_nontemporal_load(reinterpret_cast<const nt_f4*>(m) + i);
        const nt_f4 vr = __builtin_nontemporal_load(reinterpret_cast<const nt_f4*>(v) + i);
        float4 mm = make_float4(mr.x, mr.y, mr.z, mr.w), vv = make_float4(vr.x, vr.y, vr.z, vr.w);
#else
        float4 pp = p4[i], mm = m4[i], vv = v4[i];
#endif
        float4 gg = make_float4(0.f, 0.f, 0.f, 0.f);
        if (hit) gg = g4[i];
        adam_elem(pp.x, gg.x, mm.x, vv.x, a, omb1, omb2, ss, ssn);
        adam_elem(pp.y, gg.y, mm.y, vv.y, a, omb1, omb2, ss, ssn);
        adam_elem(pp.z, gg.z, mm.z, vv.z, a, omb1, omb2, ss, ssn);
// ... 150 lines not shown
                                                         const uint32_t* __restrict__ bits, unsigned row_len, const LazyArgs lz) {
    __shared__ float red[4];
    float ss = 0.f;
    const float omb1 = 1.0f - a.b1, omb2 = 1.0f - a.b2, omr = 1.0f - da.rho;
    const size_t n4 = count >> 2;
    float4* p4 = reinterpret_cast<float4*>(p);
    const float4* g4 = reinterpret_cast<const float4*>(g);
    typedef float nt_f4 __attribute__((ext_vector_type(4)));
    const size_t per = (n4 + gridDim.x - 1) / gridDim.x;
    const size_t lo = (size_t)blockIdx.x * per;
    const size_t hi = lo + per < n4 ? lo + per : n4;
    for (size_t i = lo + threadIdx.x; i < hi; i += blockDim.x) {
        const unsigned e0 = (unsigned)i << 2;
        const unsigned row = e0 / row_len;
        const bool first_piece = e0 - row * row_len == 0u;
        const int last = lz.last_in ? lz.last_in[row] : lz.t_prev;
        const int lag = lz.t_prev - last;
        const bool hit = lz.update && row_bit(bits, row);
        const bool need = lz.update ? (hit || lz.write_all || (lz.next_bits && row_bit(lz.next_bits, row))) : (lag > 0);
        if (first_piece) lz.last_out[row] = lz.update ? (need ? lz.t_prev + 1 : last) : lz.t_prev;
        if (!lz.update && lag == 0) continue;
        float4 pp = p4[i];
        const nt_f4 mr = __builtin_nontemporal_load(reinterpret_cast<const nt_f4*>(s0) + i);
        const nt_f4 vr = __builtin_nontemporal_load(reinterpret_cast<const nt_f4*>(s1) + i);
        float4 mm = make_float4(mr.x, mr.y, mr.z, mr.w), vv = make_float4(vr.x, vr.y, vr.z, vr.w);
        for (int k = lag; k >= 1; --k) {
            float z0 = 0.f, z1 = 0.f, z2 = 0.f, z3 = 0.f, sd = 0.f, sn = 0.f;
            if (ADAM) {
                AdamArgs ak = a;
                ak.a_t = lazy_step_size(lz, k);
                adam_elem(pp.x, z0, mm.x, vv.x, ak, omb1, omb2, sd, sn);
                adam_elem(pp.y, z1, mm.y, vv.y, ak, omb1, omb2, sd, sn);
                adam_elem(pp.z, z2, mm.z, vv.z, ak, omb1, omb2, sd, sn);
                adam_elem(pp.w, z3, mm.w, vv.w, ak, omb1, omb2, sd, sn);
            } else {
                adadelta_elem(pp.x, z0, mm.x, vv.x, da, omr, sd);
                adadelta_elem(pp.y, z1, mm.y, vv.y, da, omr, sd);
                adadelta_elem(pp.z, z2, mm.z, vv.z, da, omr, sd);
                adadelta_elem(pp.w, z3, mm.w, vv.w, da, omr, sd);
            }
        }
        if (lz.update && !need) {
            ss = sq_acc(ss, pp.x);
            ss = sq_acc(ss, pp.y);
            ss = sq_acc(ss, pp.z);
            ss = sq_acc(ss, pp.w);
            continue;
        }
        if (lz.update) {
            float4 gg = make_float4(0.f, 0.f, 0.f, 0.f);
            if (hit) gg = g4[i];
            float sn = 0.f;
            if (ADAM) {
                AdamArgs ak = a;
                ak.a_t = lz.a_of[0];
                adam_elem(pp.x, gg.x, mm.x, vv.x, ak, omb1, omb2, ss, sn);
                adam_elem(pp.y, gg.y, mm.y, vv.y, ak, omb1, omb2, ss, sn);
                adam_elem(pp.z, gg.z, mm.z, vv.z, ak, omb1, omb2, ss, sn);
                adam_elem(pp.w, gg.w, mm.w, vv.w, ak, omb1, omb2, ss, sn);
            } else {
                adadelta_elem(pp.x, gg.x, mm.x, vv.x, da, omr, ss);
                adadelta_elem(pp.y, gg.y, mm.y, vv.y, da, omr, ss);
                adadelta_elem(pp.z, gg.z, mm.z, vv.z, da, omr, ss);
                adadelta_elem(pp.w, gg.w, mm.w, vv.w, da, omr, ss);
            }
        }
        p4[i] = pp;
        { nt_f4 t; t.x = mm.x; t.y = mm.y; t.z = mm.z; t.w = mm.w; __builtin_nontemporal_store(t, reinterpret_cast<nt_f4*>(s0) + i); }
        { nt_f4 t; t.x = vv.x; t.y = vv.y; t.z = vv.z; t.w = vv.w; __builtin_nontemporal_store(t, reinterpret_cast<nt_f4*>(s1) + i); }
    }
    if (lz.update) {
        const float tot = block_sum_256(ss, red);
        if (threadIdx.x == 0) sumsq_partial[blockIdx.x] = tot;
    }
}

#ifndef SERT_SKIP_PF
#define SERT_SKIP_PF 1
#endif
constexpr bool kSkipPrefetchAdam = SERT_SKIP_PF != 0;
#ifndef SERT_SKIP_WAVES
#define SERT_SKIP_WAVES(CPL) 1
#endif
struct SkipArgs {
    float* pred;
    unsigned stride;
    int npred;
    float a_fut[kLazyK];
};

template <int LPR>
__device__ __forceinline__ float lane_group_sum(float v, int lane) {
    v = row16_sum(v);
    const float lo = read_lane(v, 0) + read_lane(v, 16), hi = read_lane(v, 32) + read_lane(v, 48);
    if (LPR == 64) return lo + hi;
    return lane < 32 ? lo : hi;
}

template <bool ADAM, int LPR, int CPL>
__global__ __launch_bounds__(256, SERT_SKIP_WAVES(CPL)) void dense_update_skip(float* __restrict__ p, const float* __restrict__ g,
                                                         float* __restrict__ s0, float* __restrict__ s1, unsigned nrows,
                                                         AdamArgs a, AdadeltaArgs da, float* __restrict__ sumsq_partial,
                                                         const uint32_t* __restrict__ bits, unsigned row_len, const LazyArgs lz,
                                                         const SkipArgs sk) {
    constexpr int GPB = 256 / LPR;
    constexpr bool kSkipPrefetch = kSkipPrefetchAdam && ADAM;
    __shared__ float red[GPB];
    const int lane = threadIdx.x & 63, l = threadIdx.x & (LPR - 1), grp = threadIdx.x / LPR;
    const float omb1 = 1.0f - a.b1, omb2 = 1.0f - a.b2, omr = 1.0f - da.rho;
    const unsigned d4 = row_len >> 2;
    const unsigned per = (nrows + gridDim.x - 1) / gridDim.x;
    const unsigned lo = blockIdx.x * per;
    const unsigned hi = lo + per < nrows ? lo + per : nrows;
    const int slot_now = (lz.t_prev + 1) % kLazyK;
    typedef float nt_f4 __attribute__((ext_vector_type(4)));
    float4* p4 = reinterpret_cast<float4*>(p);
    const float4* g4 = reinterpret_cast<const float4*>(g);
    float acc = 0.f;
    const unsigned cnt = hi > lo + grp ? (hi - lo - grp + GPB - 1) / GPB : 0u;
    const unsigned cnt_w = (unsigned)__builtin_amdgcn_readfirstlane((int)cnt);
    for (unsigned j0 = 0; j0 < cnt_w; j0 += LPR) {
        const unsigned jm = j0 + l;
        const unsigned row_m = lo + grp + jm * GPB;
        int flags_m = 0, last_m = lz.t_prev;
        float pred_m = 0.f;
        if (jm < cnt) {
            last_m = lz.last_in ? lz.last_in[row_m] : lz.t_prev;
            const bool hit_m = row_bit(bits, row_m);
            const bool need_m = hit_m || lz.write_all || (lz.next_bits && row_bit(lz.next_bits, row_m));
            lz.last_out[row_m] = need_m ? lz.t_prev + 1 : last_m;
            if (!need_m) pred_m = sk.pred[(size_t)slot_now * sk.stride + row_m];
            flags_m = 1 | (hit_m ? 2 : 0) | (need_m ? 4 : 0);
        }
        const unsigned trips = cnt_w - j0 < (unsigned)LPR ? cnt_w - j0 : (unsigned)LPR;
        struct RowRegs { float4 p[CPL], m[CPL], v[CPL], g[CPL]; };
        auto fetch = [&](unsigned jj, RowRegs& r) {
            const int flags = __shfl(flags_m, (int)jj, LPR);
            const bool hit = flags & 2, proc = (flags & 5) == 5;
            const unsigned row = lo + grp + (j0 + jj) * GPB;
#pragma unroll
            for (int c = 0; c < CPL; ++c) {
                r.p[c] = r.m[c] = r.v[c] = r.g[c] = make_float4(0.f, 0.f, 0.f, 0.f);
                if (proc && (unsigned)(l + c * LPR) < d4) {
                    const size_t i = (size_t)row * d4 + l + c * LPR;
                    r.p[c] = p4[i];
                    const nt_f4 mr = __builtin_nontemporal_load(reinterpret_cast<const nt_f4*>(s0) + i);
                    const nt_f4 vr = __builtin_nontemporal_load(reinterpret_cast<const nt_f4*>(s1) + i);
                    r.m[c] = make_float4(mr.x, mr.y, mr.z, mr.w);
                    r.v[c] = make_float4(vr.x, vr.y, vr.z, vr.w);
                    if (hit) r.g[c] = g4[i];
                }
            }
        };
        RowRegs nxt;
        if (kSkipPrefetch && trips > 0) fetch(0, nxt);
        for (unsigned jj = 0; jj < trips; ++jj) {
            const int flags = __shfl(flags_m, (int)jj, LPR);
            const int last = __shfl(last_m, (int)jj, LPR);
            const float predv = __shfl(pred_m, (int)jj, LPR);
            const bool valid = flags & 1, proc = (flags & 5) == 5;
            RowRegs cur;
            if (kSkipPrefetch) {
                cur = nxt;
                if (jj + 1 < trips) fetch(jj + 1, nxt);
            }
            if (!__any(proc)) {
                if (valid) acc += predv;
                continue;
            }
            if (!kSkipPrefetch) fetch(jj, cur);
            const unsigned row = lo + grp + (j0 + jj) * GPB;
            const int lag = proc ? lz.t_prev - last : 0;
            bool on[CPL];
#pragma unroll
            for (int c = 0; c < CPL; ++c) on[c] = proc && (unsigned)(l + c * LPR) < d4;
            float4 (&pp)[CPL] = cur.p;
            float4 (&mm)[CPL] = cur.m;
            float4 (&vv)[CPL] = cur.v;
            auto advance = [&](float at, float& s) {
                float sn = 0.f;
#pragma unroll
                for (int c = 0; c < CPL; ++c) {
                    if (!on[c]) continue;
                    float z0 = 0.f, z1 = 0.f, z2 = 0.f, z3 = 0.f;
                    if (ADAM) {
                        AdamArgs ak = a;
                        ak.a_t = at;
                        adam_elem(pp[c].x, z0, mm[c].x, vv[c].x, ak, omb1, omb2, s, sn);
                        adam_elem(pp[c].y, z1, mm[c].y, vv[c].y, ak, omb1, omb2, s, sn);
                        adam_elem(pp[c].z, z2, mm[c].z, vv[c].z, ak, omb1, omb2, s, sn);
                        adam_elem(pp[c].w, z3, mm[c].w, vv[c].w, ak, omb1, omb2, s, sn);
                    } else {
                        adadelta_elem(pp[c].x, z0, mm[c].x, vv[c].x, da, omr, s);
                        adadelta_elem(pp[c].y, z1, mm[c].y, vv[c].y, da, omr, s);
                        adadelta_elem(pp[c].z, z2, mm[c].z, vv[c].z, da, omr, s);
                        adadelta_elem(pp[c].w, z3, mm[c].w, vv[c].w, da, omr, s);
                    }
                }
            };
            for (int k = kLazyK; k >= 1; --k) {
                if (k <= lag) { float sd = 0.f; advance(lazy_step_size(lz, k), sd); }
            }
            float s = 0.f;
            {
                float sn = 0.f;
#pragma unroll
                for (int c = 0; c < CPL; ++c) {
                    if (!on[c]) continue;
                    const size_t i = (size_t)row * d4 + l + c * LPR;
                    float4 gg = cur.g[c];
                    if (ADAM) {
                        AdamArgs ak = a;
                        ak.a_t = lz.a_of[0];
                        adam_elem(pp[c].x, gg.x, mm[c].x, vv[c].x, ak, omb1, omb2, s, sn);
                        adam_elem(pp[c].y, gg.y, mm[c].y, vv[c].y, ak, omb1, omb2, s, sn);
                        adam_elem(pp[c].z, gg.z, mm[c].z, vv[c].z, ak, omb1, omb2, s, sn);
                        adam_elem(pp[c].w, gg.w, mm[c].w, vv[c].w, ak, omb1, omb2, s, sn);
                    } else {
                        adadelta_elem(pp[c].x, gg.x, mm[c].x, vv[c].x, da, omr, s);
                        adadelta_elem(pp[c].y, gg.y, mm[c].y, vv[c].y, da, omr, s);
                        adadelta_elem(pp[c].z, gg.z, mm[c].z, vv[c].z, da, omr, s);
                        adadelta_elem(pp[c].w, gg.w, mm[c].w, vv[c].w, da, omr, s);
                    }
                    p4[i] = pp[c];
                    { nt_f4 t; t.x = mm[c].x; t.y = mm[c].y; t.z = mm[c].z; t.w = mm[c].w; __builtin_nontemporal_store(t, reinterpret_cast<nt_f4*>(s0) + i); }
                    { nt_f4 t; t.x = vv[c].x; t.y = vv[c].y; t.z = vv[c].z; t.w = vv[c].w; __builtin_nontemporal_store(t, reinterpret_cast<nt_f4*>(s1) + i); }
                }
            }
            const float rowsum = lane_group_sum<LPR>(s, lane);
            if (valid) acc += proc ? rowsum : predv;
            for (int q = 1; q <= sk.npred; ++q) {
                float s2 = 0.f;
                if (q < sk.npred) {
                    advance(sk.a_fut[q - 1], s2);
                } else {
#pragma unroll
                    for (int c = 0; c < CPL; ++c) {
                        if (!on[c]) continue;
                        s2 = sq_acc(s2, pp[c].x); s2 = sq_acc(s2, pp[c].y); s2 = sq_acc(s2, pp[c].z); s2 = sq_acc(s2, pp[c].w);
                    }
                }
                const float r = lane_group_sum<LPR>(s2, lane);
                if (proc && l == 0) sk.pred[(size_t)((lz.t_prev + 1 + q) % kLazyK) * sk.stride + row] = r;
            }
        }
    }
    if (l == 0) red[grp] = acc;
    __syncthreads();
    if (threadIdx.x == 0) {
        float t = red[0];
#pragma unroll
        for (int i = 1; i < GPB; ++i) t += red[i];
        sumsq_partial[blockIdx.x] = t;
// ... 256 lines not shown
```

### sert_amd/csrc/model.h

```cpp
#pragma once
#include <vector>
#include <string>
#include "common.h"
#include "word_index.h"
#include "kernels_xchg.h"
#include "../../include/sert_hip.h"
#include "../../include/sert_hip_debug.h"

namespace sert {

struct DataSplit {
    int64_t N = 0;
    void* x = nullptr;
    int32_t* y = nullptr;
    int64_t* csr_indptr = nullptr;
    int32_t* csr_indices = nullptr;
    float* csr_data = nullptr;
    int64_t nnz = 0;
    int64_t max_labels_per_row = 0;
    float* w = nullptr;
    float* labfix = nullptr;
    int32_t* idx_rows = nullptr;
    int4* idx_items = nullptr;
    int4* idx_heavy = nullptr;
    int32_t* idx_bundles = nullptr;
    int32_t* idx_uwords = nullptr;
    int32_t* idx_slots = nullptr;
    int32_t* idx_rows_div = nullptr;
    uint32_t* idx_touched_bits = nullptr;
    uint4* idx_dense_counts = nullptr;
    int32_t* idx_dense_words = nullptr;
    uint8_t* idx_tok_slot = nullptr;
    std::vector<int32_t> dense_cnt_of;
    int64_t bit_words = 0;
    std::vector<BatchIndex> idx_batches;
};

enum TimingGroup {
    TG_GATHER = 0,
    TG_GEMM_FWD,
    TG_LOSS,
    TG_SORT,
    TG_EGRAD,
    TG_EFIX,
    TG_GEMM_DW,
    TG_SPLITK,
    TG_GEMM_DX,
    TG_SCATTER,
    TG_ALLREDUCE,
    TG_REDUCE_SCATTER,
    TG_ALLGATHER,
    TG_OPT_WORD,
    TG_OPTIMIZER,
    TG_FINALIZE,
    TG_COUNT
};

struct Timing {
    bool enabled = false;
    hipEvent_t ev[TG_COUNT][2] = {};
    bool created = false;
    bool used[TG_COUNT] = {};
    double total_us[TG_COUNT] = {};
    int64_t samples[TG_COUNT] = {};
};

struct InStep {
    static constexpr int kRing = 1024;
    bool on = false;
    bool created = false;
    hipEvent_t ev[kRing][2] = {};
    int group[kRing] = {};
    int64_t head = 0, tail = 0;
    int cur_group = -1;
    double total_us[TG_COUNT] = {};
    int64_t launches[TG_COUNT] = {};
    int64_t steps = 0;
};

}

struct sert_model {
    sert_config cfg;
    hipStream_t stream = nullptr;
    hipStream_t stream2 = nullptr;
    hipEvent_t ev_fork = nullptr, ev_join = nullptr, ev_join3 = nullptr;
    hipStream_t stream3 = nullptr;
    hipEvent_t ev_step_done = nullptr, ev_neg = nullptr, ev_opt_fork = nullptr, ev_small = nullptr;
    hipEvent_t ev_loss = nullptr;
    hipEvent_t ev_dense = nullptr;
    bool step_done_pending = false;
    bool re_in_parts = false;
    bool fork_bound = false;
    bool egrad_ranges = false;
    bool egrad_force_sort = false;
    bool events_device_scope = false;
    bool lazy_join = false;
    int num_cus = 256;
    bool proj_fused = false;
    bool ll_dw_side = false;
    bool dw_side_first = false;
    bool dp_late_join = false;
    bool side_heavy = false;
    hipEvent_t ev_re = nullptr;
    bool re_pending = false;
    bool tail_early = false, w_early_pending = false;
    hipStream_t tail_stream = nullptr;
    hipEvent_t ev_tail_go = nullptr, ev_tail_done = nullptr;
    bool tail_pending = false;
    int tail_queue_min_batch = 0;
    bool w_pending = false;
    float* re_sq = nullptr;
    int64_t re_sq_for[2] = {-1, -1};
    int n_loss_partials = 0;
    bool loss_from_rows = false;
    int nce_loss_partials = 0;
    int nstreams = 2;
    int64_t hint_next = -1;
    bool neg_side_ready = false;
    bool sort_early = false;
    bool bucket_early = false;
    int32_t* rw_last[2] = {nullptr, nullptr};
    int rw_last_cur = 0;
    bool rw_stale = false;
    int64_t rw_ready_batch = -1;
    int64_t lazy_next = -1;
    float cur_touched_frac = 1.f;
    float* rw_pred = nullptr;
    unsigned rw_pred_stride = 0;
    bool rw_pred_ok = false;
    int64_t rw_pred_T = 0;
    bool lazy_skip = true;
    float lazy_max = 0.5f;
    int64_t upd_counts[10] = {0, 0, 0, 0, 0, 0, 0, 0, 0, 0};
    int64_t projected_batch = -1;
    int64_t spec_fb_batch = -1;
    int64_t spec_fb_step = -1;
    unsigned loss_seq = 0;
    float* h_loss_dev = nullptr;

    size_t n_rw = 0, n_re = 0, n_w = 0, n_b = 0;

    float *rw = nullptr, *re = nullptr, *W = nullptr, *b = nullptr;
    float *s0_rw = nullptr, *s0_re = nullptr, *s0_w = nullptr, *s0_b = nullptr;
    float *s1_rw = nullptr, *s1_re = nullptr, *s1_w = nullptr, *s1_b = nullptr;

    float* gflat = nullptr;
    size_t gflat_count = 0;
    float *g_re = nullptr, *g_rw = nullptr, *g_w = nullptr, *g_b = nullptr, *g_loss = nullptr;
    size_t gflat_alloc = 0;
    int32_t *run_start = nullptr, *run_end = nullptr;

    float *H = nullptr, *T = nullptr, *DA = nullptr, *DH = nullptr, *rowloss = nullptr;
    float* T_alt = nullptr;
    float* DH2 = nullptr;
    int fs_tile = 0;
    int32_t* neg = nullptr;
    int32_t* neg_alt = nullptr;
    int64_t neg_alt_step = -1;
    int64_t* neg_stage = nullptr;
    int32_t *cand = nullptr, *cand_sorted = nullptr, *pair_sorted = nullptr;
    int32_t* cand_early = nullptr;
    float* coef = nullptr;
    float *ehead = nullptr, *etail = nullptr;
    float* epart = nullptr;
    int32_t *eg_entries = nullptr, *eg_offs = nullptr;
    int eg_sub_rows = 0, eg_num_sub = 0, eg_subs_per_group = 0, eg_groups = 0, eg_ranges = 0, eg_er_shift = 0;
    int32_t *sort_hist = nullptr, *sort_bin_total = nullptr;
    int32_t *sort_k_tmp = nullptr, *sort_v_tmp = nullptr;
    int sort_bits = 1;
    float *G = nullptr;
    float *Z = nullptr;
    float *J = nullptr;
    float *DG = nullptr;

    float* wpart = nullptr;
    float* hpart = nullptr;
    size_t wpart_rows = 0;
    float* part = nullptr;
    size_t part_count = 0;
    float2* ll_tokstat = nullptr; float* ll_lse = nullptr; float2* ll_jstat = nullptr;
    float4* ll_rowinfo = nullptr; float* ll_rpart = nullptr; float* ll_r = nullptr;
    bool use_touched = false;
    hipStream_t stream4 = nullptr;
    hipEvent_t ev_word_opt = nullptr;
    hipEvent_t ev_early = nullptr;
    bool early_issued = false;
    int early_sq = 0;

    float* Zu = nullptr;
    float* dZu = nullptr;
    size_t zu_rows = 0;
    float* zpart = nullptr;
    size_t zpart_rows = 0;
    bool ll_dedup = false;
    float* ll_rsum = nullptr;
    int ll_U = 0;
    float* skbuf = nullptr;
    size_t skbuf_count = 0;
    const float* tail_part = nullptr;
    unsigned long long* tail_blk = nullptr;
    unsigned tail_launch_seq = 0;
    int tail_splits = 0;
    size_t tail_stride = 0;
    float* red_loss = nullptr;
    float* red_sq = nullptr;
    float* d_loss = nullptr;
    float* h_loss = nullptr;
    float* d_losses = nullptr;
    int64_t d_losses_cap = 0;

    float *pred_a = nullptr, *pred_b = nullptr;
    void* pred_ids = nullptr;
    size_t pred_a_cap = 0, pred_b_cap = 0, pred_ids_cap = 0;

    sert::DataSplit split[2];
// ... 73 lines not shown
```

### sert_amd/csrc/sert_hip.hip

```cpp
#include <dlfcn.h>
#include <math.h>
#include <string.h>

#include <algorithm>
#include <chrono>
#include <functional>
#include <string>
#include <vector>

#include "common.h"
#include "gemm.h"
#include "gemm_x3.h"
#ifdef SERT_VARIANTS
#include "variants/gemm_bwd_fused.h"
#include "variants/gemm_big.h"
#include "variants/gemm_x3_bres.h"
#include "variants/score_filter_ring.h"
#include "variants/gemm_strip.h"
#include "variants/gemm_stream.h"
#include "variants/gemm_direct.h"
#endif
#include "kernels_score_bf16.h"
#include "kernels_egrad.h"
#include "kernels_ll.h"
// ... 119 lines not shown
};
struct Rccl {
    void* lib = nullptr;
    int (*GetUniqueId)(void*) = nullptr;
    int (*CommInitRank)(void**, int,  UniqueId, int) = nullptr;
    int (*CommDestroy)(void*) = nullptr;
    int (*AllReduce)(const void*, void*, size_t, int, int, void*, hipStream_t) = nullptr;
    int (*ReduceScatter)(const void*, void*, size_t, int, int, void*, hipStream_t) = nullptr;
    int (*AllGather)(const void*, void*, size_t, int, void*, hipStream_t) = nullptr;
    int (*Send)(const void*, size_t, int, int, void*, hipStream_t) = nullptr;
    int (*Recv)(void*, size_t, int, int, void*, hipStream_t) = nullptr;
    int (*GroupStart)() = nullptr;
    int (*GroupEnd)() = nullptr;
    const char* (*GetErrorString)(int) = nullptr;
};
static Rccl g_rccl;

static int rccl_load() {
    if (g_rccl.lib) return 0;
    const char* names[] = {"librccl.so.1", "librccl.so", "/opt/rocm/lib/librccl.so.1",
                           "/opt/rocm/lib/librccl.so"};
    void* lib = nullptr;
    for (const char* n : names) {
        lib = dlopen(n, RTLD_NOW | RTLD_GLOBAL);
        if (lib) break;
    }
    if (!lib) SERT_FAIL(std::string("cannot dlopen librccl: ") + dlerror());
    g_rccl.GetUniqueId = (decltype(g_rccl.GetUniqueId))dlsym(lib, "ncclGetUniqueId");
    g_rccl.CommInitRank = (decltype(g_rccl.CommInitRank))dlsym(lib, "ncclCommInitRank");
    g_rccl.CommDestroy = (decltype(g_rccl.CommDestroy))dlsym(lib, "ncclCommDestroy");
    g_rccl.AllReduce = (decltype(g_rccl.AllReduce))dlsym(lib, "ncclAllReduce");
    g_rccl.ReduceScatter = (decltype(g_rccl.ReduceScatter))dlsym(lib, "ncclReduceScatter");
    g_rccl.AllGather = (decltype(g_rccl.AllGather))dlsym(lib, "ncclAllGather");
    g_rccl.Send = (decltype(g_rccl.Send))dlsym(lib, "ncclSend");
    g_rccl.Recv = (decltype(g_rccl.Recv))dlsym(lib, "ncclRecv");
    g_rccl.GroupStart = (decltype(g_rccl.GroupStart))dlsym(lib, "ncclGroupStart");
    g_rccl.GroupEnd = (decltype(g_rccl.GroupEnd))dlsym(lib, "ncclGroupEnd");
    g_rccl.GetErrorString = (decltype(g_rccl.GetErrorString))dlsym(lib, "ncclGetErrorString");
    if (!g_rccl.GetUniqueId || !g_rccl.CommInitRank || !g_rccl.CommDestroy || !g_rccl.AllReduce ||
        !g_rccl.ReduceScatter || !g_rccl.AllGather || !g_rccl.Send || !g_rccl.Recv || !g_rccl.GroupStart ||
        !g_rccl.GroupEnd)
        SERT_FAIL("librccl is missing ncclGetUniqueId/ncclCommInitRank/ncclCommDestroy/ncclAllReduce/"
                  "ncclReduceScatter/ncclAllGather/ncclSend/ncclRecv/ncclGroupStart/ncclGroupEnd");
    g_rccl.lib = lib;
    return 0;
}
#define SERT_NCCL(expr)                                                                       \
    do {                                                                                      \
        int _r = (expr);                                                                      \
        if (_r != 0)                                                                          \
            SERT_FAIL(std::string(#expr) + ": " +                                             \
                      (g_rccl.GetErrorString ? g_rccl.GetErrorString(_r) : "rccl error"));    \
    } while (0)

template <typename T>
static int dmalloc(T** p, size_t count) {
    *p = nullptr;
    if (count == 0) return 0;
    SERT_HIP(hipMalloc((void**)p, count * sizeof(T)));
    return 0;
}
template <typename T>
static int dzalloc(T** p, size_t count, hipStream_t s) {
    SERT_TRY(dmalloc(p, count));
    if (count) SERT_HIP(hipMemsetAsync(*p, 0, count * sizeof(T), s));
    return 0;
}
static inline int grid_for(int64_t work_items, int block = 256, int cap = 256 * 8) {
    int64_t g = (work_items + block - 1) / block;
    if (g < 1) g = 1;
    if (g > cap) g = cap;
    return (int)g;
}
static inline size_t round_up(size_t a, size_t b) { return (a + b - 1) / b * b; }

static bool is_vs(const sert_model* m) { return m->cfg.kind != SERT_KIND_LOGLINEAR; }
static bool is_fs(const sert_model* m) { return m->cfg.kind == SERT_KIND_VECTORSPACE_SOFTMAX; }
static void discard_run_ahead(sert_model* m) {
    if (m->spec_fb_batch >= 0 && m->stream2 && m->ev_join) {
        (void)hipEventRecord(m->ev_join, m->stream2);
        (void)hipStreamWaitEvent(m->stream, m->ev_join, 0);
    }
    m->spec_fb_batch = -1;
}
static int ensure_rw_current(sert_model* m, int64_t batch, int64_t t_applied = -1);
static bool egrad_writes_every_row(const sert_model* m);
static int settle_tail(sert_model* m);
static void invalidate_speculation(sert_model* m) {
    discard_run_ahead(m);
    (void)settle_tail(m);
    (void)ensure_rw_current(m, -1);
    if (m->re_pending) {
        (void)hipStreamWaitEvent(m->stream, m->ev_re, 0);
        m->re_pending = false;
    }
    m->re_sq_for[0] = m->re_sq_for[1] = -1;
    m->projected_batch = -1;
    m->neg_alt_step = -1;
    m->rw_pred_ok = false;
}

#include "host/lazy_segsum.inc"

#include "host/data_parallel.inc"

#include "host/step_vectorspace.inc"

#include "host/step_softmax_loglinear.inc"

#include "host/optimizer_and_loss.inc"

}

using namespace sert;

extern "C" {

#include "host/api_model.inc"

#include "host/api_data_train.inc"

#include "host/api_scorer.inc"

#include "host/api_comm.inc"

#include "host/api_debug.inc"

}


#ifdef SR_TIMELINE
extern "C" int sert_debug_read(void* out, size_t bytes) {
    (void)hipDeviceSynchronize();
    return (int)hipMemcpyFromSymbol(out, HIP_SYMBOL(sert::sr_dbg), bytes, 0, hipMemcpyDeviceToHost);
}
#endif
```

### sert_amd/csrc/word_index.h

```cpp
#pragma once
#include <stdint.h>
#include <algorithm>
#include <vector>

namespace sert {

constexpr int kSegChunk = 64;
constexpr int kHeavyMax = 16;
constexpr int kHeavyMinCount = 4096;
constexpr int kHeavyRowsPerBlock = 256;
constexpr int kSegMaxLevels = 6;
constexpr int kBundleItems = 8;
constexpr int kFusedMaxChunks = 32;

struct SegItem {
    int32_t begin;
    int32_t end;
    int32_t dst;
    int32_t slot;
};

struct BatchIndex {
    int64_t rows_off = 0;
    int nlevels = 0;
    int64_t item_off[kSegMaxLevels] = {};
    int32_t item_cnt[kSegMaxLevels] = {};
    int64_t part_off[kSegMaxLevels] = {};
    int64_t part_rows = 0;
    int64_t uw_off = 0;
    int32_t num_distinct = 0;
    int64_t heavy_off = 0;
    int32_t heavy_cnt = 0;
    bool fused_upper_ok = false;
    int32_t dense_cnt = 0;
    int32_t dense_word[kHeavyMax] = {};
    int32_t dense_slot[kHeavyMax] = {};
    int32_t row_groups = 1;
    int32_t xcd_off[8] = {};
    int32_t xcd_cnt[8] = {};
    int64_t bundle_off = 0;
    int32_t bundle_cnt = 0;
    bool slot_is_row = false;
};

struct WordIndex {
    std::vector<int32_t> rows;
    std::vector<SegItem> items;
    std::vector<BatchIndex> batches;
    std::vector<int32_t> heavy;
    std::vector<int32_t> bundles;
    int64_t max_part_rows = 0;
    std::vector<int32_t> uwords;
    std::vector<int32_t> slots;
    std::vector<int32_t> rows_div;
    int32_t max_distinct = 0;
    std::vector<uint32_t> touched_bits;
    int64_t bit_words = 0;
    std::vector<uint8_t> dense_counts;
    bool any_dense = false;
    std::vector<uint8_t> dense_tok_slot;
};

template <typename IdT>
bool build_word_index(const IdT* ids, int64_t num_batches, int B, int n, int vocab,
                      bool row_is_pos, WordIndex& out, bool want_slots = false, bool dense_heavy = false,
                      int row_groups = 1, bool sort_level0 = false) {
    const int64_t T = (int64_t)B * n;
    if (want_slots || row_is_pos || row_groups < 1) row_groups = 1;
    const int rows_per_group = (B + row_groups - 1) / row_groups;
    const bool flag_only = want_slots;
    dense_heavy = dense_heavy && (want_slots || !row_is_pos) && n <= 255;
    std::vector<int8_t> heavy_slot;
    if (dense_heavy) {
        heavy_slot.assign((size_t)vocab, (int8_t)-1);
        out.dense_counts.assign((size_t)(num_batches * B) * kHeavyMax, (uint8_t)0);
        if (!want_slots) out.dense_tok_slot.assign((size_t)(num_batches * T), (uint8_t)255);
    }
    out.rows.resize((size_t)(num_batches * T));
    out.batches.resize((size_t)num_batches);
    if (want_slots) out.slots.resize((size_t)(num_batches * T));
    std::vector<int32_t> slot_of((size_t)(want_slots ? vocab : 0), 0);
    std::vector<int32_t> count((size_t)vocab + 1, 0);
    std::vector<int32_t> touched;
    touched.reserve((size_t)std::min<int64_t>(T, vocab));
    std::vector<int32_t> start;
    out.bit_words = ((((int64_t)vocab + 31) / 32) + 3) / 4 * 4;
    out.touched_bits.assign((size_t)(num_batches * out.bit_words), 0u);
    for (int64_t bi = 0; bi < num_batches; ++bi) {
        const IdT* x = ids + bi * T;
        BatchIndex& bx = out.batches[(size_t)bi];
        bx.rows_off = bi * T;
        touched.clear();
        for (int64_t p = 0; p < T; ++p) {
            const int64_t wid64 = (int64_t)x[p];
            if (wid64 >= vocab) return false;
            const int32_t wid = (int32_t)wid64;
            if (count[wid]++ == 0) touched.push_back(wid);
        }
        std::sort(touched.begin(), touched.end());
        {
            uint32_t* bits = out.touched_bits.data() + bi * out.bit_words;
            for (int32_t wid : touched) bits[wid >> 5] |= 1u << (wid & 31);
        }
        bx.dense_cnt = 0;
        if (dense_heavy) {
            std::vector<std::pair<int32_t, int32_t>> cand;
            for (int32_t wid : touched)
                if (count[wid] > kHeavyMinCount) cand.push_back({count[wid], wid});
            std::sort(cand.begin(), cand.end(), [](const std::pair<int32_t, int32_t>& a, const std::pair<int32_t, int32_t>& b) {
                return a.first != b.first ? a.first > b.first : a.second < b.second;
            });
            if ((int)cand.size() > kHeavyMax) cand.resize(kHeavyMax);
            int64_t held = 0;
            for (const auto& c : cand) held += c.first;
            if (!cand.empty() && held * 8 >= T) {
                for (size_t h = 0; h < cand.size(); ++h) {
                    bx.dense_word[h] = cand[h].second;
                    bx.dense_slot[h] = (int32_t)(std::lower_bound(touched.begin(), touched.end(), cand[h].second) - touched.begin());
                    heavy_slot[(size_t)cand[h].second] = (int8_t)h;
                }
                bx.dense_cnt = (int32_t)cand.size();
                uint8_t* dc = out.dense_counts.data() + (size_t)(bi * B) * kHeavyMax;
                uint8_t* ts = out.dense_tok_slot.empty() ? nullptr : out.dense_tok_slot.data() + (size_t)(bi * T);
                for (int64_t p = 0; p < T; ++p) {
                    const int8_t h = heavy_slot[(size_t)x[p]];
                    if (h >= 0) {
                        ++dc[(size_t)(p / n) * kHeavyMax + h];
                        if (ts) ts[p] = (uint8_t)h;
                    }
                }
                out.any_dense = true;
            }
        }
        bx.uw_off = (int64_t)out.uwords.size();
        bx.num_distinct = (int32_t)touched.size();
        out.max_distinct = std::max(out.max_distinct, bx.num_distinct);
        if (want_slots) {
            out.uwords.insert(out.uwords.end(), touched.begin(), touched.end());
            for (size_t t = 0; t < touched.size(); ++t) slot_of[(size_t)touched[t]] = (int32_t)t;
            int32_t* sl = out.slots.data() + bi * T;
            for (int64_t p = 0; p < T; ++p) sl[p] = slot_of[(size_t)x[p]];
        }
        start.resize(touched.size() + 1);
        int32_t acc = 0;
        for (size_t t = 0; t < touched.size(); ++t) {
            start[t] = acc;
            const int32_t c = count[touched[t]];
            count[touched[t]] = acc;
            acc += c;
        }
        start[touched.size()] = acc;
// ... 41 lines not shown
                    pbase[t] = nparts;
                    segs.push_back({nparts, nparts + nitems_of[t], touched[t], (int32_t)t, false});
                    nparts += nitems_of[t];
                }
            std::vector<int32_t> gbase((size_t)row_groups, 0);
            int32_t acc_e = 0;
            for (int g = 0; g < row_groups; ++g) {
                gbase[(size_t)g] = acc_e;
                std::copy(grows[(size_t)g].begin(), grows[(size_t)g].end(), rows + acc_e);
                acc_e += (int32_t)grows[(size_t)g].size();
            }
            bx.item_off[0] = (int64_t)out.items.size();
            bx.part_off[0] = 0;
            std::vector<int32_t> cursor(touched.size(), 0);
            std::vector<std::vector<int32_t>> first_part((size_t)row_groups);
            for (int g = 0; g < row_groups; ++g) {
                first_part[(size_t)g].resize(gsegs[(size_t)g].size());
                for (size_t k = 0; k < gsegs[(size_t)g].size(); ++k) {
                    const GSeg& sg = gsegs[(size_t)g][k];
                    first_part[(size_t)g][k] = cursor[(size_t)sg.t];
                    cursor[(size_t)sg.t] += (sg.end - sg.begin + kSegChunk - 1) / kSegChunk;
                }
            }
            for (int x = 0; x < 8; ++x) {
                bx.xcd_off[x] = (int32_t)((int64_t)out.items.size() - bx.item_off[0]);
                for (int g = x; g < row_groups; g += 8)
                    for (size_t k = 0; k < gsegs[(size_t)g].size(); ++k) {
                        const GSeg& sg = gsegs[(size_t)g][k];
                        int32_t q = 0;
                        for (int32_t b = sg.begin; b < sg.end; b += kSegChunk, ++q) {
                            const int32_t e2 = std::min(sg.end, b + kSegChunk);
                            const int32_t dst = pbase[(size_t)sg.t] < 0 ? touched[(size_t)sg.t]
                                                                       : -(pbase[(size_t)sg.t] + first_part[(size_t)g][k] + q + 1);
                            out.items.push_back({gbase[(size_t)g] + b, gbase[(size_t)g] + e2, dst, (int32_t)sg.t});
                        }
                    }
                bx.xcd_cnt[x] = (int32_t)((int64_t)out.items.size() - bx.item_off[0]) - bx.xcd_off[x];
            }
            bx.item_cnt[0] = (int32_t)((int64_t)out.items.size() - bx.item_off[0]);
            bx.row_groups = row_groups;
            part_base = nparts;
            level = 1;
        } else {
        for (size_t t = 0; t < touched.size(); ++t) {
            const bool dense = bx.dense_cnt > 0 && heavy_slot[(size_t)touched[t]] >= 0;
            if (dense && !flag_only) continue;
            segs.push_back({start[t], start[t + 1], touched[t], (int32_t)t, dense});
        }
        for (int h = 0; h < bx.dense_cnt; ++h) heavy_slot[(size_t)bx.dense_word[h]] = (int8_t)-1;
        }
        while (!segs.empty() && level < kSegMaxLevels) {
            bx.item_off[level] = (int64_t)out.items.size();
            bx.part_off[level] = part_base;
            std::vector<Seg> next;
            int32_t nparts = 0;
            for (const Seg& s : segs) {
                const int32_t len = s.end - s.begin;
                if (len <= kSegChunk || level == kSegMaxLevels - 1) {
                    out.items.push_back({s.begin, s.end, s.word, s.slot});
                } else {
                    const int32_t first = nparts;
                    for (int32_t b = s.begin; b < s.end; b += kSegChunk) {
                        const int32_t e = std::min(s.end, b + kSegChunk);
                        out.items.push_back({b, e, -(nparts + 1), s.dense ? -1 : 0});
                        ++nparts;
                    }
                    next.push_back({first, nparts, s.word, s.slot, s.dense});
                }
            }
            bx.item_cnt[level] = (int32_t)((int64_t)out.items.size() - bx.item_off[level]);
            part_base += nparts;
            segs.swap(next);
            ++level;
        }
        bx.nlevels = level;
        bx.part_rows = part_base;
        bx.slot_is_row = false;
        if (sort_level0 && !want_slots && !row_is_pos && bx.row_groups == 1 && level >= 1 && bx.item_cnt[0] > 0) {
            SegItem* l0 = out.items.data() + bx.item_off[0];
            for (int32_t k = 0; k < bx.item_cnt[0]; ++k) l0[k].slot = rows[l0[k].begin];
            std::stable_sort(l0, l0 + bx.item_cnt[0], [](const SegItem& a, const SegItem& b) { return a.end - a.begin > b.end - b.begin; });
            bx.slot_is_row = true;
        }
        bx.heavy_off = (int64_t)out.heavy.size() / 4;
        bx.heavy_cnt = 0;
        bx.fused_upper_ok = false;
        if (level == 3) {
            const SegItem* l1 = out.items.data() + bx.item_off[1];
            const SegItem* l2 = out.items.data() + bx.item_off[2];
            bool ok = true;
            int32_t i1 = 0;
            for (int32_t j = 0; j < bx.item_cnt[2] && ok; ++j) {
                const SegItem& parent = l2[j];
                while (i1 < bx.item_cnt[1] && l1[i1].dst >= 0) ++i1;
                const int32_t first = i1;
                int32_t n = 0;
                while (i1 < bx.item_cnt[1] && l1[i1].dst < 0 && -(l1[i1].dst + 1) < parent.end) {
                    ok = ok && (-(l1[i1].dst + 1) == parent.begin + n);
                    ++i1; ++n;
                }
                ok = ok && parent.dst >= 0 && n == parent.end - parent.begin && n >= 1 && n <= kFusedMaxChunks;
                out.heavy.push_back(first); out.heavy.push_back(n); out.heavy.push_back(parent.dst); out.heavy.push_back(0);
            }
            bx.heavy_cnt = bx.item_cnt[2];
            bx.fused_upper_ok = ok;
        }
        if (part_base > out.max_part_rows) out.max_part_rows = part_base;
        bx.bundle_off = (int64_t)out.bundles.size();
        bx.bundle_cnt = 0;
        if (bx.row_groups == 1 && bx.nlevels >= 1 && bx.item_cnt[0] > 0) {
            const SegItem* l0 = out.items.data() + bx.item_off[0];
            bool consecutive = true;
            for (int32_t k = 1; k < bx.item_cnt[0] && consecutive; ++k) consecutive = l0[k].begin == l0[k - 1].end;
            if (consecutive) {
                int32_t in_bundle = 0, entries = 0;
                for (int32_t k = 0; k < bx.item_cnt[0]; ++k) {
                    const int32_t len = l0[k].end - l0[k].begin;
                    if (in_bundle == 0 || in_bundle == kBundleItems || entries + len > kSegChunk) {
                        out.bundles.push_back(k);
                        ++bx.bundle_cnt;
                        in_bundle = 0;
                        entries = 0;
                    }
                    ++in_bundle;
                    entries += len;
                }
                out.bundles.push_back(bx.item_cnt[0]);
            }
        }
    }
    return true;
}

}
```

Baseline: 294.9 million pairs/s.

## Fuse final word-gradient reduction into the lazy Adam update via per-word recipes

Builds a per-batch recipe table on the host that records, for each touched word, how its gradient is formed: a single source row, a list of entries, a partial sum, or a heavy-word block sum. A bit-prefix index maps touched bits to recipe slots. The segmented-sum pass now only writes level-0 chunk partials and heavy partials. The Adam update kernel then forms each word's final gradient on the fly instead of reading a materialised gradient row, which aims to skip writing and rereading the full word-gradient rows. Where fusion is not applied, a deferred completion path runs the remaining segsum work, at the cost of more host bookkeeping and a larger, more branchy optimizer kernel.

```diff
diff --git a/include/sert_hip_debug.h b/include/sert_hip_debug.h
--- a/include/sert_hip_debug.h
+++ b/include/sert_hip_debug.h
@@ -8,6 +8,9 @@
 #endif
 
 int sert_debug_update_counts(sert_model* m, int64_t* out, int n);
+int sert_debug_fused_word_grad(sert_model* m, int64_t* out);
+int sert_debug_word_recipe_sum(const void* ids, int id_bytes, int64_t num_batches, int B, int n, int vocab, int dense_heavy,
+                               int64_t batch, const float* src, int d, float divisor, float* grad_out, int64_t* stats);
 
 int sert_debug_poison_scratch(sert_model* m);
 
diff --git a/sert_amd/_capi.py b/sert_amd/_capi.py
--- a/sert_amd/_capi.py
+++ b/sert_amd/_capi.py
@@ -29,7 +29,7 @@
     'sert_comm_unique_id', 'sert_comm_init', 'sert_comm_init_host', 'sert_comm_destroy', 'sert_comm_stats',
     'sert_synchronize', 'sert_timing_enable', 'sert_timing_reset', 'sert_timing_count',
     'sert_timing_name', 'sert_timing_avg_us', 'sert_timing_launches', 'sert_bench_gemm', 'sert_debug_gemm', 'sert_debug_gemm_splitk', 'sert_debug_gemm_longk', 'sert_bench_memory', 'sert_debug_row_lists', 'sert_debug_word_index_sum',
-    'sert_debug_update_counts', 'sert_debug_poison_scratch',
+    'sert_debug_update_counts', 'sert_debug_poison_scratch', 'sert_debug_fused_word_grad', 'sert_debug_word_recipe_sum',
     'sert_profile_range_push', 'sert_profile_range_pop',
 ]
 
@@ -355,6 +355,12 @@
         names = ('dense', 'lazy', 'skip_32_1', 'skip_64_1', 'skip_32_3', 'skip_64_2', 'skip_64_3', 'skip_64_4', 'skip_full', 'skip_sparse')
         return dict(zip(names, (int(x) for x in v)))
 
+    def fused_word_grad_counts(self):
+        v = (ctypes.c_int64 * 2)()
+        self._lib.sert_debug_fused_word_grad.argtypes = [ctypes.c_void_p, ctypes.POINTER(ctypes.c_int64)]
+        check(self._lib.sert_debug_fused_word_grad(self._h, v))
+        return int(v[0]), int(v[1])
+
     def timings(self):
         n = self._lib.sert_timing_count(self._h)
         return {self._lib.sert_timing_name(self._h, i).decode():
@@ -525,6 +531,25 @@
     return out, dict(zip(keys, [int(x) for x in stats]))
 
 
+def debug_word_recipe_sum(ids, vocab, src, batch=0, dense_heavy=False, divisor=1.0):
+    lib = load()
+    ids = np.ascontiguousarray(ids)
+    assert ids.ndim == 3 and ids.dtype in (np.uint8, np.uint16, np.uint32), (ids.shape, ids.dtype)
+    src = np.ascontiguousarray(src, dtype=np.float32)
+    nb, B, n = ids.shape
+    assert src.shape[0] == B
+    d = src.shape[1]
+    out = np.empty((vocab, d), dtype=np.float32)
+    stats = np.zeros(8, dtype=np.int64)
+    lib.sert_debug_word_recipe_sum.argtypes = [ctypes.c_void_p, ctypes.c_int, ctypes.c_int64, ctypes.c_int, ctypes.c_int, ctypes.c_int,
+                                               ctypes.c_int, ctypes.c_int64, ctypes.c_void_p, ctypes.c_int, ctypes.c_float,
+                                               ctypes.c_void_p, ctypes.c_void_p]
+    check(lib.sert_debug_word_recipe_sum(_addr(ids), ids.dtype.itemsize, nb, B, n, int(vocab), int(bool(dense_heavy)), int(batch),
+                                         _addr(src), d, float(divisor), _addr(out), _addr(stats)))
+    keys = ('recipe_ok', 'chunk_items', 'touched_rows', 'entries', 'rows', 'partials', 'heavy')
+    return out, dict(zip(keys, [int(x) for x in stats[:7]]))
+
+
 def debug_gemm(A, B, ta=0, tb=0, epi=0, bias=None, device=0):
     lib = load()
     A = np.ascontiguousarray(A, dtype=np.float32)
diff --git a/sert_amd/csrc/host/api_data_train.inc b/sert_amd/csrc/host/api_data_train.inc
--- a/sert_amd/csrc/host/api_data_train.inc
+++ b/sert_amd/csrc/host/api_data_train.inc
@@ -90,10 +90,13 @@
             if (const char* e = variant_knob("SERT_SEG_GROUPS")) row_groups = std::min(std::max(1, atoi(e)), std::max(1, B / 64));
         const bool sort_level0 = is_vs(m) && row_groups == 1 && !(variant_knob("SERT_SEG_BUNDLE") && atoi(variant_knob("SERT_SEG_BUNDLE")) != 0) &&
                                  !variant_knob("SERT_SEG_NO_SORT");
+        const bool want_recipe = is_vs(m) && !is_fs(m) && m->fused_wg && m->cfg.word_dim % 4 == 0 && m->cfg.word_dim / 4 <= 32 &&
+                                 row_groups == 1 && !(variant_knob("SERT_SEG_BUNDLE") && atoi(variant_knob("SERT_SEG_BUNDLE")) != 0);
         bool ids_ok = true;
         SERT_ID_DISPATCH(m->cfg.id_bytes,
                          ids_ok = build_word_index<IdT>((const IdT*)x, nb, B, n, m->cfg.vocab_size, row_is_pos, wi,
-                                                        !is_vs(m), dense_heavy, row_groups, sort_level0));
+                                                        !is_vs(m), dense_heavy, row_groups, sort_level0,
+                                                        want_recipe));
         if (!ids_ok) SERT_FAIL("token id >= vocab_size in x");
         if (!is_vs(m) && !wi.slots.empty()) {
             const size_t V = (size_t)m->cfg.num_entities;
@@ -140,6 +143,13 @@
                                     hipMemcpyHostToDevice, s));
             SERT_HIP(hipStreamSynchronize(s));
             d.bit_words = wi.bit_words;
+        }
+        if (!wi.recipe.empty() && !wi.bit_prefix.empty()) {
+            SERT_HIP(hipMalloc((void**)&d.idx_recipe, wi.recipe.size() * sizeof(int32_t)));
+            SERT_HIP(hipMemcpyAsync(d.idx_recipe, wi.recipe.data(), wi.recipe.size() * sizeof(int32_t), hipMemcpyHostToDevice, s));
+            SERT_TRY(dmalloc(&d.idx_bit_prefix, wi.bit_prefix.size()));
+            SERT_HIP(hipMemcpyAsync(d.idx_bit_prefix, wi.bit_prefix.data(), wi.bit_prefix.size() * sizeof(int32_t), hipMemcpyHostToDevice, s));
+            SERT_HIP(hipStreamSynchronize(s));
         }
         if (is_dp(m)) SERT_TRY(xr_build_lists(m, wi.touched_bits, nb, wi.bit_words));
         if (wi.any_dense) {
diff --git a/sert_amd/csrc/host/api_debug.inc b/sert_amd/csrc/host/api_debug.inc
--- a/sert_amd/csrc/host/api_debug.inc
+++ b/sert_amd/csrc/host/api_debug.inc
@@ -104,6 +104,90 @@
     }
     stats[0] = bx.nlevels; stats[1] = items_total; stats[2] = bx.part_rows; stats[3] = finals; stats[4] = bx.dense_cnt;
     stats[5] = bx.row_groups; stats[6] = bx.item_cnt[0]; stats[7] = bx.num_distinct;
+    return 0;
+}
+
+int sert_debug_word_recipe_sum(const void* ids, int id_bytes, int64_t num_batches, int B, int n, int vocab, int dense_heavy,
+                               int64_t batch, const float* src, int d, float divisor, float* grad_out, int64_t* stats) {
+    if (!ids || !src || !grad_out || !stats || num_batches <= 0 || B <= 0 || n <= 0 || vocab <= 0 || d <= 0 || batch < 0 ||
+        batch >= num_batches || (id_bytes != 1 && id_bytes != 2 && id_bytes != 4))
+        SERT_FAIL("bad argument");
+    WordIndex wi;
+    bool ok = true;
+    SERT_ID_DISPATCH(id_bytes, ok = build_word_index<IdT>((const IdT*)ids, num_batches, B, n, vocab, false, wi,
+                                                          false, dense_heavy != 0, 1, true,
+                                                          true));
+    if (!ok) SERT_FAIL("token id >= vocab");
+    const BatchIndex& bx = wi.batches[(size_t)batch];
+    std::fill(grad_out, grad_out + (size_t)vocab * d, 0.f);
+    for (int i = 0; i < 8; ++i) stats[i] = 0;
+    stats[0] = bx.recipe_ok ? 1 : 0;
+    stats[1] = bx.l0_chunk_cnt;
+    if (!bx.recipe_ok) return 0;
+    const SegItem* l0 = wi.items.data() + bx.item_off[0];
+    const int32_t* rows = wi.rows.data() + bx.rows_off;
+    for (int32_t k = 0; k < (bx.nlevels >= 1 ? bx.item_cnt[0] : 0); ++k)
+        if ((l0[k].dst < 0) != (k < bx.l0_chunk_cnt)) SERT_FAIL("level 0's chunk items do not stand first");
+    std::vector<float> part((size_t)std::max<int64_t>(1, bx.part_rows) * d, 0.f);
+    for (int32_t k = 0; k < bx.l0_chunk_cnt; ++k) {
+        const SegItem& it = l0[k];
+        for (int c = 0; c < d; ++c) {
+            float a = 0.f;
+            if (it.end - it.begin == 1) a += src[(size_t)it.slot * d + c];
+            else
+            for (int32_t e = it.begin; e < it.end; ++e) a += src[(size_t)rows[e] * d + c];
+            part[(size_t)(-(it.dst + 1)) * d + c] = a;
+        }
+    }
+    const int rpb = heavy_rows_fused(B), nblocks = (B + rpb - 1) / rpb;
+    std::vector<float> hpart((size_t)nblocks * kHeavyMax * d, 0.f);
+    const uint8_t* dc = wi.dense_counts.empty() ? nullptr : wi.dense_counts.data() + (size_t)(batch * B) * kHeavyMax;
+    for (int h = 0; h < bx.dense_cnt; ++h)
+        for (int b = 0; b < nblocks; ++b)
+            for (int c = 0; c < d; ++c) {
+                float a = 0.f;
+                for (int i = b * rpb; i < std::min(B, (b + 1) * rpb); ++i) a += (float)dc[(size_t)i * kHeavyMax + h] * src[(size_t)i * d + c];
+                hpart[((size_t)b * kHeavyMax + h) * d + c] = a;
+            }
+    const uint32_t* bits = wi.touched_bits.data() + batch * wi.bit_words;
+    const int32_t* pre = wi.bit_prefix.data() + batch * wi.bit_words;
+    const int32_t* rc = wi.recipe.data() + 2 * bx.recipe_off;
+    for (int64_t r = 0; r < vocab; ++r) {
+        const uint32_t w = bits[r >> 5];
+        if (!((w >> (r & 31)) & 1u)) continue;
+        ++stats[2];
+        const int32_t idx = pre[r >> 5] + __builtin_popcount(w & ((1u << (r & 31)) - 1u));
+        const int32_t x = rc[2 * idx], y = rc[2 * idx + 1], kind = y >> 24, len = y & 0xffffff;
+        if (kind < 0 || kind > 3) SERT_FAIL("bad recipe kind");
+        ++stats[3 + kind];
+        for (int c = 0; c < d; ++c) {
+            float a = 0.f;
+            if (kind == kRecipeHeavy) {
+                if (bx.dense_word[x] != r) SERT_FAIL("a heavy descriptor names another word");
+                float g8[8];
+                for (int g = 0; g < 8; ++g) {
+                    g8[g] = 0.f;
+                    for (int b = g; b < nblocks; b += 8) g8[g] += hpart[((size_t)b * kHeavyMax + x) * d + c];
+                }
+                a = g8[0];
+                for (int g = 1; g < 8; ++g) a += g8[g];
+            } else if (kind == kRecipeRow) {
+                a += src[(size_t)x * d + c];
+            } else if (kind == kRecipeEntries) {
+                for (int32_t e = x; e < x + len; ++e) a += src[(size_t)rows[e] * d + c];
+            } else {
+                for (int32_t e = x; e < x + len; ++e) a += part[(size_t)e * d + c];
+            }
+            grad_out[(size_t)r * d + c] = a / divisor;
+        }
+    }
+    return 0;
+}
+
+int sert_debug_fused_word_grad(sert_model* m, int64_t* out) {
+    if (!m || !out) SERT_FAIL("bad argument");
+    out[0] = m->wg_fused_count;
+    out[1] = m->wg_completed_count;
     return 0;
 }
 
diff --git a/sert_amd/csrc/host/api_model.inc b/sert_amd/csrc/host/api_model.inc
--- a/sert_amd/csrc/host/api_model.inc
+++ b/sert_amd/csrc/host/api_model.inc
@@ -190,6 +190,7 @@
     m->proj_fused = variant_knob("SERT_PROJ_FUSED") && atoi(variant_knob("SERT_PROJ_FUSED")) != 0;
     m->lazy_skip = !(knob("SERT_LAZY_SKIP") && atoi(knob("SERT_LAZY_SKIP")) == 0);
     m->lazy_max = knob("SERT_LAZY_MAX") ? (float)atof(knob("SERT_LAZY_MAX")) : 0.5f;
+    m->fused_wg = !(knob("SERT_FUSED_WORD_GRAD") && atoi(knob("SERT_FUSED_WORD_GRAD")) == 0);
     {
         int cus = 0;
         if (hipDeviceGetAttribute(&cus, hipDeviceAttributeMultiprocessorCount, m->cfg.device) != hipSuccess || cus <= 0) cus = 256;
@@ -346,6 +347,8 @@
     (void)hipFree(d.idx_bundles); d.idx_bundles = nullptr;
     (void)hipFree(d.idx_uwords); (void)hipFree(d.idx_slots); (void)hipFree(d.idx_rows_div);
     (void)hipFree(d.idx_touched_bits);
+    (void)hipFree(d.idx_recipe); d.idx_recipe = nullptr;
+    (void)hipFree(d.idx_bit_prefix); d.idx_bit_prefix = nullptr;
     (void)hipFree(d.idx_dense_counts); (void)hipFree(d.idx_dense_words); (void)hipFree(d.idx_tok_slot);
     d.idx_uwords = nullptr; d.idx_slots = nullptr; d.idx_rows_div = nullptr;
     d = DataSplit();
diff --git a/sert_amd/csrc/host/lazy_segsum.inc b/sert_amd/csrc/host/lazy_segsum.inc
--- a/sert_amd/csrc/host/lazy_segsum.inc
+++ b/sert_amd/csrc/host/lazy_segsum.inc
@@ -92,11 +92,88 @@
     } while (0)
 
 
+static bool adam_split_enabled();
+static inline bool is_dp(const sert_model* m);
+static bool heavy_stream_fused(const sert_model* m, const DataSplit& ds, const BatchIndex& bx) {
+    const int d4 = m->cfg.word_dim / 4;
+    static const bool no_fuse = variant_knob("SERT_HEAVY_NO_FUSE") != nullptr;
+    const bool lpi32 = d4 <= 32 || (d4 > 64 && 64 * cdiv(d4, 64) > 32 * cdiv(d4, 32));
+    const bool bundled = bx.bundle_cnt > 0 && ds.idx_bundles;
+    return !no_fuse && lpi32 && bx.nlevels >= 1 && bx.item_cnt[0] > 0 && bx.row_groups == 1 && !bundled;
+}
+static PlusJob heavy_stream_job(sert_model* m, const DataSplit& ds, int64_t batch_index, const BatchIndex& bx, const float* src) {
+    const int B = m->cfg.batch_size;
+    PlusJob j = PlusJob();
+    j.kind = 1; j.rpb = heavy_rows_fused(B); j.extra = cdiv(B, j.rpb); j.src = src; j.cnt16 = ds.idx_dense_counts + (size_t)batch_index * B;
+    j.part = m->hpart; j.words = (const int32_t*)ds.idx_dense_words + (size_t)batch_index * kHeavyMax;
+    j.nheavy = bx.dense_cnt; j.nblocks = j.extra; j.B = B;
+    return j;
+}
+
+static bool word_update_fusable(const sert_model* m, const DataSplit& ds, const BatchIndex& bx) {
+    const auto& c = m->cfg;
+    if (!m->fused_wg || !is_vs(m) || is_fs(m) || is_dp(m) || m->timing.enabled || c.keep_grads || c.word_dim % 4 != 0 ||
+        c.word_dim / 4 > 32 || !m->use_touched || adam_split_enabled() || !m->rw_last[0] || !m->lazy_skip || !m->rw_pred ||
+        !m->pt_big[0] || m->n_rw < ((size_t)1 << 22))
+        return false;
+    if (!ds.idx_recipe || !ds.idx_bit_prefix || !bx.recipe_ok || !m->wpart) return false;
+    if (bx.dense_cnt > 0 && (!heavy_stream_fused(m, ds, bx) || !m->hpart)) return false;
+    const float frac = (float)bx.num_distinct / (float)c.vocab_size;
+    const float lazy_max = m->lazy_next >= 0 ? m->lazy_max : std::min(m->lazy_max, 0.35f);
+    return frac <= lazy_max;
+}
+
+static int complete_word_grad(sert_model* m) {
+    if (m->wg_pending < 0) return 0;
+    const int64_t batch_index = m->wg_pending;
+    m->wg_pending = -1;
+    ++m->wg_completed_count;
+    const DataSplit& ds = m->split[SERT_SPLIT_TRAIN];
+    const BatchIndex& bx = ds.idx_batches[(size_t)batch_index];
+    const int d = m->cfg.word_dim;
+    const float* src = m->wg_src;
+    const float divisor = m->wg_divisor;
+    const int nfin = bx.nlevels >= 1 ? bx.item_cnt[0] - bx.l0_chunk_cnt : 0;
+    if (nfin > 0) {
+        PlusJob j = PlusJob();
+        j.slot_is_row = bx.slot_is_row ? 1 : 0;
+        hipLaunchKernelGGL(segsum_rows_plus, dim3(cdiv(nfin, 8), cdiv(d / 4, 32)), dim3(256), 0, m->stream, src,
+                           (const int32_t*)(ds.idx_rows + bx.rows_off), (const int4*)(ds.idx_items + bx.item_off[0] + bx.l0_chunk_cnt),
+                           nfin, m->g_rw, m->wpart, d, divisor, j);
+    }
+    PlusJob j = PlusJob();
+    if (bx.dense_cnt > 0) {
+        j = heavy_stream_job(m, ds, batch_index, bx, src);
+        j.kind = 2; j.extra = bx.dense_cnt; j.src = m->hpart;
+    }
+    const int n1 = bx.nlevels >= 2 ? bx.item_cnt[1] : 0;
+    if (n1 + j.extra > 0)
+        hipLaunchKernelGGL(segsum_rows_plus, dim3(j.extra + cdiv(n1, 8), cdiv(d / 4, 32)), dim3(256), 0, m->stream,
+                           (const float*)(m->wpart + (size_t)bx.part_off[0] * d), (const int32_t*)nullptr,
+                           (const int4*)(ds.idx_items + bx.item_off[1]), n1, m->g_rw, m->wpart + (size_t)bx.part_off[1] * d, d, divisor, j);
+    return 0;
+}
+
 static int word_grad_segsum(sert_model* m, const DataSplit& ds, int64_t batch_index,
-                            const float* src, float divisor) {
+                            const float* src, float divisor, bool allow_fused = false) {
     const int d = m->cfg.word_dim;
     if ((size_t)batch_index >= ds.idx_batches.size()) SERT_FAIL("batch has no word index");
     const BatchIndex& bx = ds.idx_batches[(size_t)batch_index];
+    m->wg_pending = -1;
+    if (allow_fused && word_update_fusable(m, ds, bx)) {
+        PlusJob j = PlusJob();
+        if (bx.dense_cnt > 0) j = heavy_stream_job(m, ds, batch_index, bx, src);
+        j.slot_is_row = bx.slot_is_row ? 1 : 0;
+        const int nch = bx.l0_chunk_cnt;
+        if (nch + j.extra > 0)
+            hipLaunchKernelGGL(segsum_rows_plus, dim3(j.extra + cdiv(nch, 8), cdiv(d / 4, 32)), dim3(256), 0, m->stream, src,
+                               (const int32_t*)(ds.idx_rows + bx.rows_off), (const int4*)(ds.idx_items + bx.item_off[0]), nch, m->g_rw,
+                               m->wpart + (size_t)bx.part_off[0] * d, d, divisor, j);
+        m->wg_pending = batch_index;
+        m->wg_src = src;
+        m->wg_divisor = divisor;
+        return 0;
+    }
     unsigned char* touched = nullptr;
     static const bool no_fused_upper = variant_knob("SERT_SEG_NO_FUSED_UPPER") != nullptr;
     const bool fused_upper = !no_fused_upper && bx.fused_upper_ok && ds.idx_heavy && d % 4 == 0 &&
diff --git a/sert_amd/csrc/host/optimizer_and_loss.inc b/sert_amd/csrc/host/optimizer_and_loss.inc
--- a/sert_amd/csrc/host/optimizer_and_loss.inc
+++ b/sert_amd/csrc/host/optimizer_and_loss.inc
@@ -67,6 +67,8 @@
     lz.next_bits = next_bits;
     lz.write_all = (next_bits == nullptr || m->step % kLazyK == 0) ? 1 : 0;
     const unsigned d4 = (unsigned)c.word_dim / 4;
+    const bool fused = m->wg_pending >= 0 && m->lazy_skip && m->rw_pred && d4 <= 32 && is_vs(m);
+    if (!fused) SERT_TRY(complete_word_grad(m));
     if (m->lazy_skip && m->rw_pred && d4 <= 256) {
         const int64_t u = m->step;
         const bool sparse = next_bits && m->rw_pred_ok && u < m->rw_pred_T;
@@ -88,14 +90,36 @@
         const int nb = std::max(1, std::min<int>(skip_blocks_knob > 0 ? std::min(skip_blocks_knob, 4 * kOptBlocks) : skip_grid(nb_dense, t.n),
                                                  (int)cdiv(nrows, 8u)));
         nb_skip = nb;
+        FusedGrad fg = FusedGrad();
+        if (fused) {
+            const DataSplit& ds = m->split[SERT_SPLIT_TRAIN];
+            const BatchIndex& bx = ds.idx_batches[(size_t)m->wg_pending];
+            const int64_t bi = m->wg_pending;
+            fg.recipe = ds.idx_recipe + bx.recipe_off;
+            fg.prefix = ds.idx_bit_prefix + (size_t)bi * ds.bit_words;
+            fg.rows = ds.idx_rows + bx.rows_off;
+            fg.src = m->wg_src;
+            fg.wpart = m->wpart + (size_t)bx.part_off[0] * c.word_dim;
+            fg.hpart = m->hpart;
+            fg.hwords = ds.idx_dense_words ? (const int32_t*)ds.idx_dense_words + (size_t)bi * kHeavyMax : nullptr;
+            fg.nheavy = bx.dense_cnt;
+            fg.nblocks = cdiv(c.batch_size, heavy_rows_fused(c.batch_size));
+            fg.divisor = m->wg_divisor;
+            m->wg_pending = -1;
+            ++m->wg_fused_count;
+        }
 #define SERT_SKIP_LAUNCH(ADAM, LPR, CPL)                                                                                   \
     hipLaunchKernelGGL((dense_update_skip<ADAM, LPR, CPL>), dim3(nb), dim3(256), 0, m->stream, t.p, (const float*)t.g, t.s0, \
-           t.s1, nrows, aa, da, sq, tf, (unsigned)c.word_dim, lz, sk)
+           t.s1, nrows, aa, da, sq, tf, (unsigned)c.word_dim, lz, sk, FusedGrad())
         static const int skip_32x3_knob = variant_knob("SERT_SKIP_32X3") ? atoi(variant_knob("SERT_SKIP_32X3")) : -1;
         const bool skip_32x3 = skip_32x3_knob >= 0 ? skip_32x3_knob != 0 : t.n < ((size_t)1 << 26);
 #define SERT_SKIP_SHAPE(ADAM)                                                                   \
     do {                                                                                        \
-        if (d4 <= 32) { SERT_SKIP_LAUNCH(ADAM, 32, 1); ++m->upd_counts[2]; }                    \
+        if (d4 <= 32 && fused) {                                                                \
+            hipLaunchKernelGGL((dense_update_skip<true, 32, 1, true>), dim3(nb), dim3(256), 0, m->stream, t.p,             \
+                               (const float*)nullptr, t.s0, t.s1, nrows, aa, da, sq, tf, (unsigned)c.word_dim, lz, sk, fg); \
+            ++m->upd_counts[2];                                                                 \
+        } else if (d4 <= 32) { SERT_SKIP_LAUNCH(ADAM, 32, 1); ++m->upd_counts[2]; }             \
         else if (d4 <= 64) { SERT_SKIP_LAUNCH(ADAM, 64, 1); ++m->upd_counts[3]; }               \
         else if (d4 <= 96 && skip_32x3) { SERT_SKIP_LAUNCH(ADAM, 32, 3); ++m->upd_counts[4]; }  \
         else if (d4 <= 128) { SERT_SKIP_LAUNCH(ADAM, 64, 2); ++m->upd_counts[5]; }              \
@@ -176,6 +200,7 @@
                 n_sq += launch_lazy_word_update(m, t, tf, next_bits, nb, aa, da, m->red_sq + n_sq);
                 continue;
             }
+            if (i == 0) SERT_TRY(complete_word_grad(m));
             if (i == 0) m->rw_pred_ok = false;
             if (i == 0) ++m->upd_counts[0];
             if (i == 0) SERT_TRY(ensure_rw_current(m, -1, m->step - 1));
diff --git a/sert_amd/csrc/host/step_vectorspace.inc b/sert_amd/csrc/host/step_vectorspace.inc
--- a/sert_amd/csrc/host/step_vectorspace.inc
+++ b/sert_amd/csrc/host/step_vectorspace.inc
@@ -375,7 +375,7 @@
     auto word_table_sum = [&]() -> int {
         {
             ScopedTimer t(m, TG_SCATTER);
-            SERT_TRY(word_grad_segsum(m, ds, batch_index, m->DH, (float)n));
+            SERT_TRY(word_grad_segsum(m, ds, batch_index, m->DH, (float)n, true));
         }
         return allreduce_word_grad(m);
     };
diff --git a/sert_amd/csrc/kernels_opt.h b/sert_amd/csrc/kernels_opt.h
--- a/sert_amd/csrc/kernels_opt.h
+++ b/sert_amd/csrc/kernels_opt.h
@@ -1,5 +1,6 @@
 #pragma once
 #include "common.h"
+#include "word_index.h"
 
 namespace sert {
 
@@ -316,6 +317,9 @@
 #ifndef SERT_SKIP_WAVES
 #define SERT_SKIP_WAVES(CPL) 1
 #endif
+#ifndef SERT_SKIP_FUSED_WAVES
+#define SERT_SKIP_FUSED_WAVES 5
+#endif
 struct SkipArgs {
     float* pred;
     unsigned stride;
@@ -323,6 +327,19 @@
     float a_fut[kLazyK];
 };
 
+struct FusedGrad {
+    const int2* recipe;
+    const int32_t* prefix;
+    const int32_t* rows;
+    const float* src;
+    const float* wpart;
+    const float* hpart;
+    const int32_t* hwords;
+    int nheavy;
+    int nblocks;
+    float divisor;
+};
+
 template <int LPR>
 __device__ __forceinline__ float lane_group_sum(float v, int lane) {
     v = row16_sum(v);
@@ -331,15 +348,18 @@
     return lane < 32 ? lo : hi;
 }
 
-template <bool ADAM, int LPR, int CPL>
-__global__ __launch_bounds__(256, SERT_SKIP_WAVES(CPL)) void dense_update_skip(float* __restrict__ p, const float* __restrict__ g,
+template <bool ADAM, int LPR, int CPL, bool FUSED = false>
+__global__ __launch_bounds__(256, FUSED ? SERT_SKIP_FUSED_WAVES : SERT_SKIP_WAVES(CPL)) void dense_update_skip(float* __restrict__ p, const float* __restrict__ g,
                                                          float* __restrict__ s0, float* __restrict__ s1, unsigned nrows,
                                                          AdamArgs a, AdadeltaArgs da, float* __restrict__ sumsq_partial,
                                                          const uint32_t* __restrict__ bits, unsigned row_len, const LazyArgs lz,
-                                                         const SkipArgs sk) {
+                                                         const SkipArgs sk, const FusedGrad fg) {
     constexpr int GPB = 256 / LPR;
     constexpr bool kSkipPrefetch = kSkipPrefetchAdam && ADAM;
+    static_assert(!FUSED || (ADAM && LPR == 32 && CPL == 1), "the fused gradient exists for the 32-lane, one-chunk Adam form");
     __shared__ float red[GPB];
+    __shared__ float4 hrow[FUSED ? kHeavyMax : 1][32];
+    __shared__ float4 hsc[FUSED ? 8 : 1][32];
     const int lane = threadIdx.x & 63, l = threadIdx.x & (LPR - 1), grp = threadIdx.x / LPR;
     const float omb1 = 1.0f - a.b1, omb2 = 1.0f - a.b2, omr = 1.0f - da.rho;
     const unsigned d4 = row_len >> 2;
@@ -350,6 +370,34 @@
     typedef float nt_f4 __attribute__((ext_vector_type(4)));
     float4* p4 = reinterpret_cast<float4*>(p);
     const float4* g4 = reinterpret_cast<const float4*>(g);
+    const float4* src4 = reinterpret_cast<const float4*>(fg.src);
+    const float4* wpart4 = reinterpret_cast<const float4*>(fg.wpart);
+    const int cf = (unsigned)l < d4 ? l : 0;
+    if (FUSED) {
+        for (int h = 0; h < fg.nheavy; ++h) {
+            const unsigned w = (unsigned)fg.hwords[h];
+            if (w < lo || w >= hi) continue;
+            const float4* h4 = reinterpret_cast<const float4*>(fg.hpart);
+            float4 ha = make_float4(0.f, 0.f, 0.f, 0.f);
+            if ((unsigned)l < d4) {
+#pragma unroll 8
+                for (int b = grp; b < fg.nblocks; b += 8) {
+                    const float4 v = h4[((size_t)b * kHeavyMax + h) * d4 + l];
+                    ha.x += v.x; ha.y += v.y; ha.z += v.z; ha.w += v.w;
+                }
+            }
+            hsc[grp][l] = ha;
+            __syncthreads();
+            if (grp == 0) {
+                ha = hsc[0][l];
+#pragma unroll
+                for (int q = 1; q < 8; ++q) { const float4 v = hsc[q][l]; ha.x += v.x; ha.y += v.y; ha.z += v.z; ha.w += v.w; }
+                ha.x /= fg.divisor; ha.y /= fg.divisor; ha.z /= fg.divisor; ha.w /= fg.divisor;
+                hrow[h][l] = ha;
+            }
+            __syncthreads();
+        }
+    }
     float acc = 0.f;
     const unsigned cnt = hi > lo + grp ? (hi - lo - grp + GPB - 1) / GPB : 0u;
     const unsigned cnt_w = (unsigned)__builtin_amdgcn_readfirstlane((int)cnt);
@@ -357,6 +405,7 @@
         const unsigned jm = j0 + l;
         const unsigned row_m = lo + grp + jm * GPB;
         int flags_m = 0, last_m = lz.t_prev;
+        int rcx_m = 0, rcy_m = 0;
         float pred_m = 0.f;
         if (jm < cnt) {
             last_m = lz.last_in ? lz.last_in[row_m] : lz.t_prev;
@@ -365,13 +414,25 @@
             lz.last_out[row_m] = need_m ? lz.t_prev + 1 : last_m;
             if (!need_m) pred_m = sk.pred[(size_t)slot_now * sk.stride + row_m];
             flags_m = 1 | (hit_m ? 2 : 0) | (need_m ? 4 : 0);
+            if (FUSED && hit_m) {
+                const unsigned wb = row_m >> 5;
+                const int2 rc = fg.recipe[fg.prefix[wb] + __popc(bits[wb] & ((1u << (row_m & 31u)) - 1u))];
+                rcx_m = rc.x;
+                rcy_m = rc.y;
+            }
         }
         const unsigned trips = cnt_w - j0 < (unsigned)LPR ? cnt_w - j0 : (unsigned)LPR;
-        struct RowRegs { float4 p[CPL], m[CPL], v[CPL], g[CPL]; };
+        struct RowRegs { float4 p[CPL], m[CPL], v[CPL], g[CPL]; int r0; };
         auto fetch = [&](unsigned jj, RowRegs& r) {
             const int flags = __shfl(flags_m, (int)jj, LPR);
             const bool hit = flags & 2, proc = (flags & 5) == 5;
             const unsigned row = lo + grp + (j0 + jj) * GPB;
+            if (FUSED) {
+                const int rx = __shfl(rcx_m, (int)jj, LPR), ry = __shfl(rcy_m, (int)jj, LPR);
+                const int kind = ry >> 24, len = ry & 0xffffff;
+                r.r0 = 0;
+                if (hit && kind == kRecipeEntries) r.r0 = fg.rows[rx + min(l, len - 1)];
+            }
 #pragma unroll
             for (int c = 0; c < CPL; ++c) {
                 r.p[c] = r.m[c] = r.v[c] = r.g[c] = make_float4(0.f, 0.f, 0.f, 0.f);
@@ -382,9 +443,49 @@
                     const nt_f4 vr = __builtin_nontemporal_load(reinterpret_cast<const nt_f4*>(s1) + i);
                     r.m[c] = make_float4(mr.x, mr.y, mr.z, mr.w);
                     r.v[c] = make_float4(vr.x, vr.y, vr.z, vr.w);
-                    if (hit) r.g[c] = g4[i];
+                    if (hit && !FUSED) r.g[c] = g4[i];
                 }
             }
+            if (FUSED) {
+                const int rx = __shfl(rcx_m, (int)jj, LPR), ry = __shfl(rcy_m, (int)jj, LPR);
+                if (hit && (ry >> 24) == kRecipeRow) r.g[0] = src4[(size_t)rx * d4 + cf];
+            }
+        };
+        auto form_grad = [&](unsigned jj, RowRegs& r) {
+            const int rx = __shfl(rcx_m, (int)jj, LPR), ry = __shfl(rcy_m, (int)jj, LPR);
+            const int kind = ry >> 24, len = ry & 0xffffff;
+            float4 ga = make_float4(0.f, 0.f, 0.f, 0.f);
+            if (kind == kRecipeHeavy) {
+                r.g[0] = hrow[rx][l];
+                return;
+            }
+            if (kind == kRecipeRow) {
+                ga.x += r.g[0].x; ga.y += r.g[0].y; ga.z += r.g[0].z; ga.w += r.g[0].w;
+            } else {
+                const bool ent = kind == kRecipeEntries;
+                for (int base = 0; base < len; base += LPR) {
+                    const int cnt = min(LPR, len - base);
+                    const int myr = base == 0 ? r.r0 : (ent ? fg.rows[rx + LPR + min(l, len - LPR - 1)] : 0);
+                    auto at = [&](int k) -> size_t {
+                        return ent ? (size_t)__shfl(myr, k, LPR) * d4 + cf : (size_t)(rx + base + k) * d4 + cf;
+                    };
+                    const float4* in = ent ? src4 : wpart4;
+                    int k = 0;
+                    for (; k + 4 <= cnt; k += 4) {
+                        float4 v[4];
+#pragma unroll
+                        for (int q = 0; q < 4; ++q) v[q] = in[at(k + q)];
+#pragma unroll
+                        for (int q = 0; q < 4; ++q) { ga.x += v[q].x; ga.y += v[q].y; ga.z += v[q].z; ga.w += v[q].w; }
+                    }
+                    for (; k < cnt; ++k) {
+                        const float4 v = in[at(k)];
+                        ga.x += v.x; ga.y += v.y; ga.z += v.z; ga.w += v.w;
+                    }
+                }
+            }
+            ga.x /= fg.divisor; ga.y /= fg.divisor; ga.z /= fg.divisor; ga.w /= fg.divisor;
+            r.g[0] = ga;
         };
         RowRegs nxt;
         if (kSkipPrefetch && trips > 0) fetch(0, nxt);
@@ -403,6 +504,7 @@
                 continue;
             }
             if (!kSkipPrefetch) fetch(jj, cur);
+            if (FUSED && (flags & 2)) form_grad(jj, cur);
             const unsigned row = lo + grp + (j0 + jj) * GPB;
             const int lag = proc ? lz.t_prev - last : 0;
             bool on[CPL];
diff --git a/sert_amd/csrc/model.h b/sert_amd/csrc/model.h
--- a/sert_amd/csrc/model.h
+++ b/sert_amd/csrc/model.h
@@ -33,6 +33,8 @@
     uint8_t* idx_tok_slot = nullptr;
     std::vector<int32_t> dense_cnt_of;
     int64_t bit_words = 0;
+    int2* idx_recipe = nullptr;
+    int32_t* idx_bit_prefix = nullptr;
     std::vector<BatchIndex> idx_batches;
 };
 
@@ -132,6 +134,11 @@
     int64_t rw_pred_T = 0;
     bool lazy_skip = true;
     float lazy_max = 0.5f;
+    bool fused_wg = true;
+    int64_t wg_pending = -1;
+    int64_t wg_fused_count = 0, wg_completed_count = 0;
+    const float* wg_src = nullptr;
+    float wg_divisor = 1.f;
     int64_t upd_counts[10] = {0, 0, 0, 0, 0, 0, 0, 0, 0, 0};
     int64_t projected_batch = -1;
     int64_t spec_fb_batch = -1;
diff --git a/sert_amd/csrc/sert_hip.hip b/sert_amd/csrc/sert_hip.hip
--- a/sert_amd/csrc/sert_hip.hip
+++ b/sert_amd/csrc/sert_hip.hip
@@ -225,6 +225,7 @@
         (void)hipStreamWaitEvent(m->stream, m->ev_join, 0);
     }
     m->spec_fb_batch = -1;
+    m->wg_pending = -1;
 }
 static int ensure_rw_current(sert_model* m, int64_t batch, int64_t t_applied = -1);
 static bool egrad_writes_every_row(const sert_model* m);
diff --git a/sert_amd/csrc/word_index.h b/sert_amd/csrc/word_index.h
--- a/sert_amd/csrc/word_index.h
+++ b/sert_amd/csrc/word_index.h
@@ -41,7 +41,12 @@
     int64_t bundle_off = 0;
     int32_t bundle_cnt = 0;
     bool slot_is_row = false;
+    int32_t l0_chunk_cnt = 0;
+    bool recipe_ok = false;
+    int64_t recipe_off = 0;
 };
+
+enum RecipeKind { kRecipeEntries = 0, kRecipeRow = 1, kRecipePartial = 2, kRecipeHeavy = 3 };
 
 struct WordIndex {
     std::vector<int32_t> rows;
@@ -59,14 +64,18 @@
     std::vector<uint8_t> dense_counts;
     bool any_dense = false;
     std::vector<uint8_t> dense_tok_slot;
+    std::vector<int32_t> recipe;
+    std::vector<int32_t> bit_prefix;
 };
 
 template <typename IdT>
 bool build_word_index(const IdT* ids, int64_t num_batches, int B, int n, int vocab,
                       bool row_is_pos, WordIndex& out, bool want_slots = false, bool dense_heavy = false,
-                      int row_groups = 1, bool sort_level0 = false) {
+                      int row_groups = 1, bool sort_level0 = false, bool want_recipe = false) {
     const int64_t T = (int64_t)B * n;
     if (want_slots || row_is_pos || row_groups < 1) row_groups = 1;
+    want_recipe = want_recipe && !want_slots && !row_is_pos && row_groups == 1;
+    if (want_recipe) out.bit_prefix.assign((size_t)(num_batches * ((((int64_t)vocab + 31) / 32) + 3) / 4 * 4), 0);
     const int rows_per_group = (B + row_groups - 1) / row_groups;
     const bool flag_only = want_slots;
     dense_heavy = dense_heavy && (want_slots || !row_is_pos) && n <= 255;
@@ -274,6 +283,48 @@
             std::stable_sort(l0, l0 + bx.item_cnt[0], [](const SegItem& a, const SegItem& b) { return a.end - a.begin > b.end - b.begin; });
             bx.slot_is_row = true;
         }
+        bx.l0_chunk_cnt = 0;
+        bx.recipe_ok = false;
+        bx.recipe_off = (int64_t)out.recipe.size() / 2;
+        if (want_recipe && level <= 2) {
+            SegItem* l0 = out.items.data() + bx.item_off[0];
+            const int32_t n0 = level >= 1 ? bx.item_cnt[0] : 0;
+            bx.l0_chunk_cnt = (int32_t)(std::stable_partition(l0, l0 + n0, [](const SegItem& it) { return it.dst < 0; }) - l0);
+            const size_t base = out.recipe.size();
+            out.recipe.resize(base + 2 * touched.size(), -1);
+            int32_t* rc = out.recipe.data() + base;
+            auto rank = [&](int32_t w) { return (size_t)(std::lower_bound(touched.begin(), touched.end(), w) - touched.begin()); };
+            for (int32_t k = bx.l0_chunk_cnt; k < n0; ++k) {
+                const SegItem& it = l0[k];
+                const size_t t = rank(it.dst);
+                const int32_t len = it.end - it.begin;
+                if (len == 1) { rc[2 * t] = rows[it.begin]; rc[2 * t + 1] = kRecipeRow << 24 | 1; }
+                else { rc[2 * t] = it.begin; rc[2 * t + 1] = kRecipeEntries << 24 | len; }
+            }
+            if (level == 2) {
+                const SegItem* l1 = out.items.data() + bx.item_off[1];
+                for (int32_t k = 0; k < bx.item_cnt[1]; ++k) {
+                    const size_t t = rank(l1[k].dst);
+                    rc[2 * t] = l1[k].begin;
+                    rc[2 * t + 1] = kRecipePartial << 24 | (l1[k].end - l1[k].begin);
+                }
+            }
+            for (int h = 0; h < bx.dense_cnt; ++h) {
+                const size_t t = rank(bx.dense_word[h]);
+                rc[2 * t] = h;
+                rc[2 * t + 1] = kRecipeHeavy << 24 | 0;
+            }
+            bool ok = true;
+            for (size_t t = 0; t < touched.size() && ok; ++t) ok = rc[2 * t + 1] >= 0;
+            bx.recipe_ok = ok;
+            if (!ok) { out.recipe.resize(base); bx.l0_chunk_cnt = 0; }
+            else {
+                const uint32_t* bits = out.touched_bits.data() + bi * out.bit_words;
+                int32_t* pre = out.bit_prefix.data() + bi * out.bit_words;
+                int32_t acc_p = 0;
+                for (int64_t w = 0; w < out.bit_words; ++w) { pre[w] = acc_p; acc_p += __builtin_popcount(bits[w]); }
+            }
+        }
         bx.heavy_off = (int64_t)out.heavy.size() / 4;
         bx.heavy_cnt = 0;
         bx.fused_upper_ok = false;
```

Result: no change. 297.7 million pairs/s, median of 6 (+1.0%).
